# krispy-kenay/WebDGS

Hardware: AMD Instinct MI355X
Metric: training iters/sec (fwd+bwd+Adam), 1M Gaussians @1080p SH3 (higher is better)
Workload: dtype f32

## Files before the change

### bindings/napi/webdgs_napi.cc

```cpp
#include <node_api.h>

#include <cstdint>
#include <cstring>
#include <string>

#include "../../include/webdgs.h"

#define NAPI_OK(call)                                                         \
    do {                                                                      \
        if ((call) != napi_ok) {                                              \
            napi_throw_error(env, nullptr, "N-API call failed: " #call);      \
            return nullptr;                                                   \
        }                                                                     \
    } while (0)

static napi_value throw_wdgs(napi_env env, int code) {
    std::string msg = "[wdgs " + std::to_string(code) + "] " + wdgs_last_error();
    napi_throw_error(env, code == WDGS_E_CAPACITY ? "WDGS_E_CAPACITY" : (code == WDGS_E_STATE ? "WDGS_E_STATE" : "WDGS_E"), msg.c_str());
    return nullptr;
}
#define WDGS_OK_OR_THROW(expr)                      \
    do {                                            \
        int _rc = (expr);                           \
        if (_rc != WDGS_OK) return throw_wdgs(env, _rc); \
// ... 62 lines not shown

static napi_value abiVersion(napi_env env, napi_callback_info) { return make_u32(env, (uint32_t)wdgs_abi_version()); }
static napi_value deviceCreate(napi_env env, napi_callback_info info) {
    ARGS(1);
    wdgs_device* d = nullptr;
    WDGS_OK_OR_THROW(wdgs_device_create((int)get_u32(env, argv[0]), nullptr, &d));
    return make_ptr(env, d);
}
static napi_value deviceDestroy(napi_env env, napi_callback_info info) { ARGS(1); wdgs_device_destroy((wdgs_device*)get_ptr(env, argv[0])); return js_undefined(env); }
static napi_value deviceSynchronize(napi_env env, napi_callback_info info) {
    ARGS(1);
    WDGS_OK_OR_THROW(wdgs_device_synchronize((wdgs_device*)get_ptr(env, argv[0])));
    return js_undefined(env);
}
static napi_value deviceMemoryInfo(napi_env env, napi_callback_info info) {
    ARGS(1);
    size_t f = 0, t = 0, c = 0;
    WDGS_OK_OR_THROW(wdgs_device_memory_info((wdgs_device*)get_ptr(env, argv[0]), &f, &t, &c));
    napi_value o, v; napi_create_object(env, &o);
    napi_create_double(env, (double)f, &v); set_prop(env, o, "free", v);
    napi_create_double(env, (double)t, &v); set_prop(env, o, "total", v);
    napi_create_double(env, (double)c, &v); set_prop(env, o, "cached", v);
    return o;
}
static napi_value bufferCreate(napi_env env, napi_callback_info info) {
    ARGS(2);
    wdgs_buffer* b = nullptr;
    WDGS_OK_OR_THROW(wdgs_buffer_create((wdgs_device*)get_ptr(env, argv[0]), (size_t)get_f64(env, argv[1]), &b));
    napi_value o; napi_create_object(env, &o);
    set_prop(env, o, "handle", make_ptr(env, b));
    set_prop(env, o, "ptr", make_ptr(env, wdgs_buffer_ptr(b)));
    napi_value sz; napi_create_double(env, (double)wdgs_buffer_size(b), &sz);
    set_prop(env, o, "size", sz);
    return o;
}
static napi_value bufferDestroy(napi_env env, napi_callback_info info) { ARGS(1); wdgs_buffer_destroy((wdgs_buffer*)get_ptr(env, argv[0])); return js_undefined(env); }
static napi_value copyToDevice(napi_env env, napi_callback_info info) {
    ARGS(3);
    void* data = nullptr; size_t len = 0; napi_typedarray_type tt; napi_value ab; size_t off;
    bool is_ta = false; napi_is_typedarray(env, argv[2], &is_ta);
    if (is_ta) { NAPI_OK(napi_get_typedarray_info(env, argv[2], &tt, &len, &data, &ab, &off)); size_t es[] = {1,1,1,2,2,4,4,4,8,8,8}; len *= es[tt]; }
    else NAPI_OK(napi_get_arraybuffer_info(env, argv[2], &data, &len));
    WDGS_OK_OR_THROW(wdgs_copy_to_device((wdgs_device*)get_ptr(env, argv[0]), get_ptr(env, argv[1]), data, len));
    return js_undefined(env);
}
static napi_value copyToHost(napi_env env, napi_callback_info info) {
    ARGS(3);
    size_t len = (size_t)get_f64(env, argv[2]);
    void* data = nullptr; napi_value ab;
    NAPI_OK(napi_create_arraybuffer(env, len, &data, &ab));
    WDGS_OK_OR_THROW(wdgs_copy_to_host((wdgs_device*)get_ptr(env, argv[0]), data, get_ptr(env, argv[1]), len));
    return ab;
}
static napi_value tiledForwardCreate(napi_env env, napi_callback_info info) {
    ARGS(2);
    wdgs_tiled_forward_config c; std::memset(&c, 0, sizeof(c));
    c.num_points = (uint32_t)prop_f64(env, argv[1], "numPoints", 0);
    c.sh_deg = (uint32_t)prop_f64(env, argv[1], "shDeg", 0);
    c.viewport_width = (uint32_t)prop_f64(env, argv[1], "viewportWidth", 1);
    c.viewport_height = (uint32_t)prop_f64(env, argv[1], "viewportHeight", 1);
    c.gaussian_scale = (float)prop_f64(env, argv[1], "gaussianScale", 1.0);
    c.point_size_px = (float)prop_f64(env, argv[1], "pointSizePx", 3.0);
    c.max_splat_radius_px = (float)prop_f64(env, argv[1], "maxSplatRadiusPx", 128.0);
    c.render_mode = (uint32_t)prop_f64(env, argv[1], "renderMode", 1);
    c.max_tile_entries = (uint32_t)prop_f64(env, argv[1], "maxTileEntries", 0);
    c.compat_caps = (uint32_t)prop_f64(env, argv[1], "compatCaps", 0);
    wdgs_tiled_forward* op = nullptr;
    WDGS_OK_OR_THROW(wdgs_tiled_forward_create((wdgs_device*)get_ptr(env, argv[0]), &c, &op));
    return make_ptr(env, op);
}
static napi_value tiledForwardEncode(napi_env env, napi_callback_info info) {
    ARGS(5);
    WDGS_OK_OR_THROW(wdgs_tiled_forward_encode((wdgs_tiled_forward*)get_ptr(env, argv[0]), get_ptr(env, argv[1]), get_ptr(env, argv[2]), get_ptr(env, argv[3]),
                                               (int)get_u32(env, argv[4])));
    return js_undefined(env);
}
static napi_value tiledForwardSetViewport(napi_env env, napi_callback_info info) {
    ARGS(3);
    WDGS_OK_OR_THROW(wdgs_tiled_forward_set_viewport((wdgs_tiled_forward*)get_ptr(env, argv[0]), get_u32(env, argv[1]), get_u32(env, argv[2])));
    return js_undefined(env);
}
static napi_value tiledForwardGetResources(napi_env env, napi_callback_info info) {
    ARGS(1);
    wdgs_tiled_forward_resources r;
    WDGS_OK_OR_THROW(wdgs_tiled_forward_get_resources((wdgs_tiled_forward*)get_ptr(env, argv[0]), &r));
    napi_value o; napi_create_object(env, &o);
    set_prop(env, o, "splatBuffer", make_ptr(env, r.splat_buffer));
    set_prop(env, o, "tileKeysBuffer", make_ptr(env, r.tile_keys_buffer));
    set_prop(env, o, "tileIndicesBuffer", make_ptr(env, r.tile_indices_buffer));
    set_prop(env, o, "tileOffsetsBuffer", make_ptr(env, r.tile_offsets_buffer));
    set_prop(env, o, "tileCountsBuffer", make_ptr(env, r.tile_counts_buffer));
    set_prop(env, o, "statsBuffer", make_ptr(env, r.stats_buffer));
    set_prop(env, o, "numTilesX", make_u32(env, r.num_tiles_x));
    set_prop(env, o, "numTilesY", make_u32(env, r.num_tiles_y));
    set_prop(env, o, "totalTiles", make_u32(env, r.total_tiles));
    set_prop(env, o, "maxTileEntries", make_u32(env, r.max_tile_entries));
    return o;
}
static napi_value tiledForwardDestroy(napi_env env, napi_callback_info info) { ARGS(1); wdgs_tiled_forward_destroy((wdgs_tiled_forward*)get_ptr(env, argv[0])); return js_undefined(env); }
static napi_value tiledRasterizerCreate(napi_env env, napi_callback_info info) {
    ARGS(2);
    wdgs_tiled_rasterizer* op = nullptr;
    WDGS_OK_OR_THROW(wdgs_tiled_rasterizer_create((wdgs_device*)get_ptr(env, argv[0]), (wdgs_tiled_forward*)get_ptr(env, argv[1]), 0, &op));
    return make_ptr(env, op);
}
static napi_value tiledRasterizerEncode(napi_env env, napi_callback_info info) {
    ARGS(3);
    WDGS_OK_OR_THROW(wdgs_tiled_rasterizer_encode((wdgs_tiled_rasterizer*)get_ptr(env, argv[0]), get_u32(env, argv[1]), get_u32(env, argv[2])));
    return js_undefined(env);
}
static napi_value tiledRasterizerGet(napi_env env, napi_callback_info info) {
    ARGS(2);
    void* p = nullptr;
    wdgs_tiled_rasterizer* op = (wdgs_tiled_rasterizer*)get_ptr(env, argv[0]);
    switch (get_u32(env, argv[1])) {
        case 0: WDGS_OK_OR_THROW(wdgs_tiled_rasterizer_get_output(op, &p)); break;
        case 1: WDGS_OK_OR_THROW(wdgs_tiled_rasterizer_get_alpha(op, &p)); break;
        case 2: WDGS_OK_OR_THROW(wdgs_tiled_rasterizer_get_n_contrib(op, &p)); break;
        default: WDGS_OK_OR_THROW(wdgs_tiled_rasterizer_get_tile_offsets(op, &p)); break;
    }
    return make_ptr(env, p);
}
static napi_value tiledRasterizerDestroy(napi_env env, napi_callback_info info) { ARGS(1); wdgs_tiled_rasterizer_destroy((wdgs_tiled_rasterizer*)get_ptr(env, argv[0])); return js_undefined(env); }
static napi_value tiledBackwardCreate(napi_env env, napi_callback_info info) {
    ARGS(2);
    wdgs_tiled_backward_config c; std::memset(&c, 0, sizeof(c));
    c.num_points = (uint32_t)prop_f64(env, argv[1], "numPoints", 0);
    c.sh_deg = (uint32_t)prop_f64(env, argv[1], "shDeg", 0);
    c.viewport_width = (uint32_t)prop_f64(env, argv[1], "viewportWidth", 1);
    c.viewport_height = (uint32_t)prop_f64(env, argv[1], "viewportHeight", 1);
    c.training.lambda_l1 = (float)prop_f64(env, argv[1], "lambda_l1", 0.8);
    c.training.lambda_l2 = (float)prop_f64(env, argv[1], "lambda_l2", 0.0);
    c.training.lambda_dssim = (float)prop_f64(env, argv[1], "lambda_dssim", 0.2);
    c.training.c1 = (float)prop_f64(env, argv[1], "c1", 0.0001);
    c.training.c2 = (float)prop_f64(env, argv[1], "c2", 0.0009);
    c.max_splat_radius_px = (float)prop_f64(env, argv[1], "maxSplatRadiusPx", 128.0);
    uint32_t mode = 0;
    if (!prop_dssim_mode(env, argv[1], &mode)) return nullptr;
    wdgs_tiled_backward* op = nullptr;
    WDGS_OK_OR_THROW(wdgs_tiled_backward_create((wdgs_device*)get_ptr(env, argv[0]), &c, &op));
    const int r = wdgs_tiled_backward_set_dssim_mode(op, mode);
    if (r != WDGS_OK) { wdgs_tiled_backward_destroy(op); WDGS_OK_OR_THROW(r); }
    return make_ptr(env, op);
}
static napi_value tiledBackwardEncode(napi_env env, napi_callback_info info) {
    ARGS(5);
    wdgs_tiled_backward_resources r;
    r.splat_buffer = prop_ptr(env, argv[3], "splatBuffer");
    r.tile_offsets_buffer = prop_ptr(env, argv[3], "tileOffsetsBuffer");
    r.tile_indices_buffer = prop_ptr(env, argv[3], "tileIndicesBuffer");
    r.camera_buffer = prop_ptr(env, argv[3], "cameraBuffer");
    r.alpha_texture = prop_ptr(env, argv[3], "alphaTexture");
    r.n_contrib_texture = prop_ptr(env, argv[3], "nContribTexture");
    WDGS_OK_OR_THROW(wdgs_tiled_backward_encode((wdgs_tiled_backward*)get_ptr(env, argv[0]), get_ptr(env, argv[1]), get_ptr(env, argv[2]), &r, get_ptr(env, argv[4])));
    return js_undefined(env);
}
static napi_value tiledBackwardGradients(napi_env env, napi_callback_info info) { ARGS(1); return make_ptr(env, wdgs_tiled_backward_gradients((wdgs_tiled_backward*)get_ptr(env, argv[0]))); }
static napi_value tiledBackwardDestroy(napi_env env, napi_callback_info info) { ARGS(1); wdgs_tiled_backward_destroy((wdgs_tiled_backward*)get_ptr(env, argv[0])); return js_undefined(env); }
static napi_value optimizerCreate(napi_env env, napi_callback_info info) {
    ARGS(4);
    wdgs_optimizer* op = nullptr;
    WDGS_OK_OR_THROW(wdgs_optimizer_create((wdgs_device*)get_ptr(env, argv[0]), get_u32(env, argv[1]), nullptr, get_ptr(env, argv[2]), get_ptr(env, argv[3]), nullptr, 1, 0, &op));
    return make_ptr(env, op);
}
static napi_value optimizerStep(napi_env env, napi_callback_info info) {
    ARGS(5);
    WDGS_OK_OR_THROW(wdgs_optimizer_step((wdgs_optimizer*)get_ptr(env, argv[0]), get_ptr(env, argv[1]), get_ptr(env, argv[2]), get_ptr(env, argv[3]), get_ptr(env, argv[4])));
    return js_undefined(env);
}
static napi_value optimizerGetIteration(napi_env env, napi_callback_info info) { ARGS(1); return make_u32(env, wdgs_optimizer_get_iteration((wdgs_optimizer*)get_ptr(env, argv[0]))); }
static napi_value optimizerDestroy(napi_env env, napi_callback_info info) { ARGS(1); wdgs_optimizer_destroy((wdgs_optimizer*)get_ptr(env, argv[0])); return js_undefined(env); }

static napi_value tiledForwardSet(napi_env env, napi_callback_info info) {
    ARGS(3);
    wdgs_tiled_forward* op = (wdgs_tiled_forward*)get_ptr(env, argv[0]);
    switch (get_u32(env, argv[1])) {
        case 0: WDGS_OK_OR_THROW(wdgs_tiled_forward_set_render_mode(op, get_u32(env, argv[2]))); break;
        case 1: WDGS_OK_OR_THROW(wdgs_tiled_forward_set_point_size(op, (float)get_f64(env, argv[2]))); break;
        default: WDGS_OK_OR_THROW(wdgs_tiled_forward_set_gaussian_scale(op, (float)get_f64(env, argv[2]))); break;
    }
    return js_undefined(env);
}
static napi_value tiledForwardCheck(napi_env env, napi_callback_info info) {
    ARGS(1);
    uint32_t st[4] = {0, 0, 0, 0};
    WDGS_OK_OR_THROW(wdgs_tiled_forward_check((wdgs_tiled_forward*)get_ptr(env, argv[0]), st));
    napi_value o; napi_create_object(env, &o);
    set_prop(env, o, "totalTileEntries", make_u32(env, st[0]));
    set_prop(env, o, "visibleCount", make_u32(env, st[1]));
    return o;
}
static napi_value tiledForwardSetLongLists(napi_env env, napi_callback_info info) {
    ARGS(4);
    WDGS_OK_OR_THROW(wdgs_tiled_forward_set_long_lists((wdgs_tiled_forward*)get_ptr(env, argv[0]), get_u32(env, argv[1]), get_u32(env, argv[2]), get_u32(env, argv[3])));
    return js_undefined(env);
}
static napi_value tiledForwardLongListStats(napi_env env, napi_callback_info info) {
    ARGS(1);
    uint32_t st[12] = {0};
    WDGS_OK_OR_THROW(wdgs_tiled_forward_long_list_stats((wdgs_tiled_forward*)get_ptr(env, argv[0]), st));
    static const char* const keys[12] = {"blocksWanted", "itemsWanted", "forwardQueue", "backwardQueue", "rowsUsed", "rowsWanted", "stalled", nullptr, "maxItems", "maxBlocks", "maxRows", "threshold"};
    napi_value o; napi_create_object(env, &o);
    for (int i = 0; i < 12; i++) if (keys[i]) set_prop(env, o, keys[i], make_u32(env, st[i]));
    return o;
}
static napi_value tiledRasterizerBlit(napi_env env, napi_callback_info info) {
    ARGS(4);
    WDGS_OK_OR_THROW(wdgs_tiled_rasterizer_blit((wdgs_tiled_rasterizer*)get_ptr(env, argv[0]), get_ptr(env, argv[1]), get_u32(env, argv[2]), get_u32(env, argv[3])));
    return js_undefined(env);
}
static napi_value tiledRasterizerEncodeDepth(napi_env env, napi_callback_info info) {
    ARGS(2);
    WDGS_OK_OR_THROW(wdgs_tiled_rasterizer_encode_depth((wdgs_tiled_rasterizer*)get_ptr(env, argv[0]), get_u32(env, argv[1])));
    return js_undefined(env);
}
static napi_value tiledRasterizerGetDepth(napi_env env, napi_callback_info info) {
    ARGS(2);
    void* p = nullptr;
    WDGS_OK_OR_THROW(wdgs_tiled_rasterizer_get_depth((wdgs_tiled_rasterizer*)get_ptr(env, argv[0]), get_u32(env, argv[1]), &p));
    return make_ptr(env, p);
}
static napi_value depthToRgba8(napi_env env, napi_callback_info info) {
    ARGS(7);
    WDGS_OK_OR_THROW(wdgs_depth_to_rgba8((wdgs_device*)get_ptr(env, argv[0]), get_ptr(env, argv[1]), get_u32(env, argv[2]), get_u32(env, argv[3]), (float)get_f64(env, argv[4]),
                                         (float)get_f64(env, argv[5]), get_ptr(env, argv[6])));
    return js_undefined(env);
}
static napi_value bufferClear(napi_env env, napi_callback_info info) {
    ARGS(3);
    WDGS_OK_OR_THROW(wdgs_memset((wdgs_device*)get_ptr(env, argv[0]), get_ptr(env, argv[1]), 0, (size_t)get_f64(env, argv[2])));
    return js_undefined(env);
}
static napi_value encoderBegin(napi_env env, napi_callback_info info) { ARGS(1); WDGS_OK_OR_THROW(wdgs_encoder_begin((wdgs_device*)get_ptr(env, argv[0]))); return js_undefined(env); }
static napi_value encoderFinish(napi_env env, napi_callback_info info) {
    ARGS(1);
    wdgs_command_buffer* c = nullptr;
    WDGS_OK_OR_THROW(wdgs_encoder_finish((wdgs_device*)get_ptr(env, argv[0]), &c));
    return make_ptr(env, c);
}
static napi_value queueSubmit(napi_env env, napi_callback_info info) {
    ARGS(2);
    WDGS_OK_OR_THROW(wdgs_queue_submit((wdgs_device*)get_ptr(env, argv[0]), (wdgs_command_buffer*)get_ptr(env, argv[1])));
    return js_undefined(env);
}
static napi_value commandBufferDestroy(napi_env env, napi_callback_info info) { ARGS(1); wdgs_command_buffer_destroy((wdgs_command_buffer*)get_ptr(env, argv[0])); return js_undefined(env); }

struct DoneCtx { napi_deferred deferred; napi_threadsafe_function tsfn; };
static void done_call_js(napi_env env, napi_value, void* context, void*) {
    DoneCtx* c = static_cast<DoneCtx*>(context);
    if (env) { napi_value u; napi_get_undefined(env, &u); napi_resolve_deferred(env, c->deferred, u); }
    napi_release_threadsafe_function(c->tsfn, napi_tsfn_release);
    delete c;
}
static void done_from_runtime_thread(void* user) {
    DoneCtx* c = static_cast<DoneCtx*>(user);
    napi_call_threadsafe_function(c->tsfn, nullptr, napi_tsfn_blocking);
}
static napi_value queueOnSubmittedWorkDone(napi_env env, napi_callback_info info) {
    ARGS(1);
    DoneCtx* c = new DoneCtx();
    napi_value promise, name;
    NAPI_OK(napi_create_promise(env, &c->deferred, &promise));
    napi_create_string_utf8(env, "wdgs onSubmittedWorkDone", NAPI_AUTO_LENGTH, &name);
    NAPI_OK(napi_create_threadsafe_function(env, nullptr, nullptr, name, 0, 1, nullptr, nullptr, c, done_call_js, &c->tsfn));
    int rc = wdgs_queue_on_done((wdgs_device*)get_ptr(env, argv[0]), done_from_runtime_thread, c);
    if (rc != WDGS_OK) { napi_release_threadsafe_function(c->tsfn, napi_tsfn_abort); delete c; return throw_wdgs(env, rc); }
    return promise;
}

static void read_backward_resources(napi_env env, napi_value o, wdgs_tiled_backward_resources* r) {
    r->splat_buffer = prop_ptr(env, o, "splatBuffer");
    r->tile_offsets_buffer = prop_ptr(env, o, "tileOffsetsBuffer");
    r->tile_indices_buffer = prop_ptr(env, o, "tileIndicesBuffer");
    r->camera_buffer = prop_ptr(env, o, "cameraBuffer");
    r->alpha_texture = prop_ptr(env, o, "alphaTexture");
    r->n_contrib_texture = prop_ptr(env, o, "nContribTexture");
}
static napi_value tiledBackwardMetric(napi_env env, napi_callback_info info) {
    ARGS(5);
    wdgs_tiled_backward* op = (wdgs_tiled_backward*)get_ptr(env, argv[0]);
    switch (get_u32(env, argv[1])) {
        case 0: WDGS_OK_OR_THROW(wdgs_tiled_backward_compute_loss_only(op, get_ptr(env, argv[2]), get_ptr(env, argv[3]))); break;
        case 1: WDGS_OK_OR_THROW(wdgs_tiled_backward_compute_metric_map(op, get_ptr(env, argv[2]), get_ptr(env, argv[3]), (float)get_f64(env, argv[4]))); break;
        case 2: {
            wdgs_tiled_backward_resources r;
            read_backward_resources(env, argv[2], &r);
            WDGS_OK_OR_THROW(wdgs_tiled_backward_compute_metric_counts(op, &r, get_u32(env, argv[3]), (int)get_u32(env, argv[4])));
            break;
        }
        case 3: WDGS_OK_OR_THROW(wdgs_tiled_backward_normalize_metric_counts(op, get_u32(env, argv[2]))); break;
        case 5: {
            uint32_t mode = 0;
            if (!prop_dssim_mode(env, argv[2], &mode)) return nullptr;
            wdgs_training_config t;
            t.lambda_l1 = (float)prop_f64(env, argv[2], "lambda_l1", 0.8);
            t.lambda_l2 = (float)prop_f64(env, argv[2], "lambda_l2", 0.0);
            t.lambda_dssim = (float)prop_f64(env, argv[2], "lambda_dssim", 0.2);
            t.c1 = (float)prop_f64(env, argv[2], "c1", 0.0001);
            t.c2 = (float)prop_f64(env, argv[2], "c2", 0.0009);
            WDGS_OK_OR_THROW(wdgs_tiled_backward_set_training_config(op, &t));
            WDGS_OK_OR_THROW(wdgs_tiled_backward_set_dssim_mode(op, mode));
            break;
        }
        default: WDGS_OK_OR_THROW(wdgs_tiled_backward_set_viewport(op, get_u32(env, argv[2]), get_u32(env, argv[3]))); break;
    }
    return js_undefined(env);
}
static napi_value tiledBackwardGet(napi_env env, napi_callback_info info) {
    ARGS(2);
    wdgs_tiled_backward* op = (wdgs_tiled_backward*)get_ptr(env, argv[0]);
    switch (get_u32(env, argv[1])) {
        case 0: return make_ptr(env, wdgs_tiled_backward_gradients(op));
        case 1: return make_ptr(env, wdgs_tiled_backward_metric_counts(op));
        case 2: return make_ptr(env, wdgs_tiled_backward_loss_image(op));
        default: return make_ptr(env, wdgs_tiled_backward_metric_map(op));
    }
}
static napi_value downsampleRGBA8(napi_env env, napi_callback_info info) {
    ARGS(7);
    WDGS_OK_OR_THROW(wdgs_downsample_rgba8((wdgs_device*)get_ptr(env, argv[0]), get_ptr(env, argv[1]), get_u32(env, argv[2]), get_u32(env, argv[3]),
                                           get_ptr(env, argv[4]), get_u32(env, argv[5]), get_u32(env, argv[6])));
    return js_undefined(env);
}
static napi_value imageSSE(napi_env env, napi_callback_info info) {
    ARGS(5);
    WDGS_OK_OR_THROW(wdgs_image_sse_rgb8((wdgs_device*)get_ptr(env, argv[0]), get_ptr(env, argv[1]), get_ptr(env, argv[2]), get_u32(env, argv[3]), get_ptr(env, argv[4])));
    return js_undefined(env);
}
static napi_value imageSSIM(napi_env env, napi_callback_info info) {
    ARGS(7);
    WDGS_OK_OR_THROW(wdgs_image_ssim_rgb8((wdgs_device*)get_ptr(env, argv[0]), get_ptr(env, argv[1]), get_ptr(env, argv[2]), get_u32(env, argv[3]), get_u32(env, argv[4]),
                                          get_ptr(env, argv[5]), get_ptr(env, argv[6])));
    return js_undefined(env);
}

static bool read_state(napi_env env, napi_value o, wdgs_optimizer_state* s) {
    napi_valuetype t; napi_typeof(env, o, &t);
    if (t != napi_object) return false;
    s->opt_pos = prop_ptr(env, o, "optPosBuffer"); s->opt_rot = prop_ptr(env, o, "optRotBuffer"); s->opt_scale = prop_ptr(env, o, "optScaleBuffer");
    s->opt_opacity = prop_ptr(env, o, "optOpacityBuffer"); s->param_sh = prop_ptr(env, o, "paramSH"); s->state_sh = prop_ptr(env, o, "stateSH");
    return true;
}
static napi_value make_state(napi_env env, const wdgs_optimizer_state& s) {
    napi_value o; napi_create_object(env, &o);
    set_prop(env, o, "optPosBuffer", make_ptr(env, s.opt_pos)); set_prop(env, o, "optRotBuffer", make_ptr(env, s.opt_rot));
    set_prop(env, o, "optScaleBuffer", make_ptr(env, s.opt_scale)); set_prop(env, o, "optOpacityBuffer", make_ptr(env, s.opt_opacity));
    set_prop(env, o, "paramSH", make_ptr(env, s.param_sh)); set_prop(env, o, "stateSH", make_ptr(env, s.state_sh));
    return o;
}
static napi_value optimizerStateSizes(napi_env env, napi_callback_info info) {
    ARGS(1);
    size_t sz[6];
    WDGS_OK_OR_THROW(wdgs_optimizer_state_sizes(get_u32(env, argv[0]), sz));
    napi_value arr; napi_create_array_with_length(env, 6, &arr);
    for (uint32_t i = 0; i < 6; i++) { napi_value v; napi_create_double(env, (double)sz[i], &v); napi_set_element(env, arr, i, v); }
    return arr;
}
static napi_value optimizerCreateWithState(napi_env env, napi_callback_info info) {
    ARGS(7);
    wdgs_optimizer_state st; std::memset(&st, 0, sizeof(st));
    const bool has = read_state(env, argv[4], &st);
    wdgs_optimizer* op = nullptr;
    WDGS_OK_OR_THROW(wdgs_optimizer_create((wdgs_device*)get_ptr(env, argv[0]), get_u32(env, argv[1]), nullptr, get_ptr(env, argv[2]), get_ptr(env, argv[3]),
                                           has ? &st : nullptr, (int)get_u32(env, argv[5]), get_u32(env, argv[6]), &op));
    return make_ptr(env, op);
}
static napi_value optimizerState(napi_env env, napi_callback_info info) {
    ARGS(2);
    wdgs_optimizer_state st;
    if (get_u32(env, argv[1])) WDGS_OK_OR_THROW(wdgs_optimizer_release_state((wdgs_optimizer*)get_ptr(env, argv[0]), &st));
    else WDGS_OK_OR_THROW(wdgs_optimizer_get_state((wdgs_optimizer*)get_ptr(env, argv[0]), &st));
    return make_state(env, st);
}
static napi_value optimizerHyperparameters(napi_env env, napi_callback_info info) {
    ARGS(2);
    wdgs_optimizer* op = (wdgs_optimizer*)get_ptr(env, argv[0]);
    wdgs_adam_hyperparameters h;
    WDGS_OK_OR_THROW(wdgs_optimizer_get_hyperparameters(op, &h));
    napi_valuetype t; napi_typeof(env, argv[1], &t);
    if (t == napi_object) {
        h.lr_pos = (float)prop_f64(env, argv[1], "lr_pos", h.lr_pos); h.lr_color = (float)prop_f64(env, argv[1], "lr_color", h.lr_color);
        h.lr_opacity = (float)prop_f64(env, argv[1], "lr_opacity", h.lr_opacity); h.lr_scale = (float)prop_f64(env, argv[1], "lr_scale", h.lr_scale);
        h.lr_rot = (float)prop_f64(env, argv[1], "lr_rot", h.lr_rot); h.beta1 = (float)prop_f64(env, argv[1], "beta1", h.beta1);
        h.beta2 = (float)prop_f64(env, argv[1], "beta2", h.beta2); h.epsilon = (float)prop_f64(env, argv[1], "epsilon", h.epsilon);
        WDGS_OK_OR_THROW(wdgs_optimizer_set_hyperparameters(op, &h));
    }
    napi_value o; napi_create_object(env, &o);
    const char* names[8] = {"lr_pos", "lr_color", "lr_opacity", "lr_scale", "lr_rot", "beta1", "beta2", "epsilon"};
    const float vals[8] = {h.lr_pos, h.lr_color, h.lr_opacity, h.lr_scale, h.lr_rot, h.beta1, h.beta2, h.epsilon};
    for (int i = 0; i < 8; i++) { napi_value v; napi_create_double(env, vals[i], &v); set_prop(env, o, names[i], v); }
    return o;
}
static napi_value optimizerAdvanceIteration(napi_env env, napi_callback_info info) {
    ARGS(2);
    WDGS_OK_OR_THROW(wdgs_optimizer_advance_iteration((wdgs_optimizer*)get_ptr(env, argv[0]), get_u32(env, argv[1])));
    return js_undefined(env);
}
static napi_value optimizerStepF32(napi_env env, napi_callback_info info) {
    ARGS(5);
    WDGS_OK_OR_THROW(wdgs_optimizer_step_f32((wdgs_optimizer*)get_ptr(env, argv[0]), get_ptr(env, argv[1]), get_ptr(env, argv[2]), get_ptr(env, argv[3]), get_ptr(env, argv[4])));
    return js_undefined(env);
}
static napi_value accumulateGradients(napi_env env, napi_callback_info info) {
    ARGS(6);
    WDGS_OK_OR_THROW(wdgs_accumulate_gradients((wdgs_device*)get_ptr(env, argv[0]), get_u32(env, argv[1]), get_ptr(env, argv[2]), get_ptr(env, argv[3]),
                                               get_ptr(env, argv[4]), get_ptr(env, argv[5])));
    return js_undefined(env);
}

static void read_densify_config(napi_env env, napi_value o, wdgs_densify_config* c) {
    c->num_views = (uint32_t)prop_f64(env, o, "numViews", 1);
    c->clone_threshold = (uint32_t)prop_f64(env, o, "cloneThreshold", 0);
    c->split_threshold = (float)prop_f64(env, o, "splitThreshold", 1e9);
    c->prune_threshold = (float)prop_f64(env, o, "pruneThreshold", 0.0);
    c->max_new_points_per_step = (uint32_t)prop_f64(env, o, "maxNewPointsPerStep", 0);
    c->max_buffer_bytes = (uint64_t)prop_f64(env, o, "maxBufferBytes", 128.0 * 1024 * 1024);
}
static napi_value densifyCreate(napi_env env, napi_callback_info info) {
    ARGS(2);
    wdgs_densify_config c; read_densify_config(env, argv[1], &c);
    wdgs_densify_prune* op = nullptr;
    WDGS_OK_OR_THROW(wdgs_densify_prune_create((wdgs_device*)get_ptr(env, argv[0]), &c, &op));
    return make_ptr(env, op);
}
static napi_value densifySetConfig(napi_env env, napi_callback_info info) {
    ARGS(2);
    wdgs_densify_config c; read_densify_config(env, argv[1], &c);
    WDGS_OK_OR_THROW(wdgs_densify_prune_set_config((wdgs_densify_prune*)get_ptr(env, argv[0]), &c));
    return js_undefined(env);
// ... 370 lines not shown
```

### include/webdgs.h

```cpp
#ifndef WEBDGS_H
#define WEBDGS_H

#include <stddef.h>
#include <stdint.h>

#ifdef __cplusplus
extern "C" {
#endif

#define WDGS_OK 0
#define WDGS_E_INVALID (-1)
#define WDGS_E_HIP (-2)
#define WDGS_E_CAPACITY (-3)
#define WDGS_E_STATE (-4)

typedef struct wdgs_device wdgs_device;
typedef struct wdgs_buffer wdgs_buffer;
typedef struct wdgs_prefix_scanner wdgs_prefix_scanner;
typedef struct wdgs_sorter wdgs_sorter;
typedef struct wdgs_tiled_forward wdgs_tiled_forward;
typedef struct wdgs_tiled_rasterizer wdgs_tiled_rasterizer;
typedef struct wdgs_tiled_backward wdgs_tiled_backward;
typedef struct wdgs_optimizer wdgs_optimizer;
typedef struct wdgs_densify_prune wdgs_densify_prune;
typedef struct wdgs_command_buffer wdgs_command_buffer;

const char* wdgs_last_error(void);
int wdgs_abi_version(void);

int wdgs_device_create(int hip_ordinal, void* external_hip_stream, wdgs_device** out);
int wdgs_device_destroy(wdgs_device* dev);
int wdgs_device_synchronize(wdgs_device* dev);
int wdgs_device_memory_info(wdgs_device* dev, size_t* free_bytes, size_t* total_bytes, size_t* cached_bytes);
int wdgs_device_set_profiling(wdgs_device* dev, int enabled);
typedef struct wdgs_kernel_time {
    char name[48];
    uint32_t launches;
    float total_ms;
} wdgs_kernel_time;
int wdgs_device_get_kernel_times(wdgs_device* dev, wdgs_kernel_time* out, uint32_t cap, uint32_t* count);
int wdgs_device_reset_kernel_times(wdgs_device* dev);
#define WDGS_MAX_LANES 4
#define WDGS_MAX_BATCH_VIEWS 16
int wdgs_device_select_lane(wdgs_device* dev, int lane);
int wdgs_device_lane_order(wdgs_device* dev, int waiter_lane, int signal_lane);
int wdgs_device_lane_mark(wdgs_device* dev, int lane, int mark);
int wdgs_device_lane_wait_mark(wdgs_device* dev, int lane, int mark);

int wdgs_encoder_begin(wdgs_device* dev);
int wdgs_encoder_finish(wdgs_device* dev, wdgs_command_buffer** out);
int wdgs_encoder_abort(wdgs_device* dev);
int wdgs_queue_submit(wdgs_device* dev, wdgs_command_buffer* cmd);
int wdgs_command_buffer_destroy(wdgs_command_buffer* cmd);
typedef void (*wdgs_done_callback)(void* user);
int wdgs_queue_on_done(wdgs_device* dev, wdgs_done_callback fn, void* user);
#define WDGS_TICKET_RING 8
int wdgs_queue_mark(wdgs_device* dev, uint64_t* ticket);
int wdgs_queue_wait(wdgs_device* dev, uint64_t ticket);

int wdgs_copy_to_host(wdgs_device* dev, void* dst_host, const void* src_dev, size_t bytes);
int wdgs_copy_to_device(wdgs_device* dev, void* dst_dev, const void* src_host, size_t bytes);
int wdgs_memset(wdgs_device* dev, void* dst_dev, int value, size_t bytes);
int wdgs_copy_buffer_to_buffer(wdgs_device* dev, void* dst_dev, const void* src_dev, size_t bytes);

int wdgs_buffer_create(wdgs_device* dev, size_t bytes, wdgs_buffer** out);
int wdgs_buffer_destroy(wdgs_buffer* buf);
void* wdgs_buffer_ptr(const wdgs_buffer* buf);
size_t wdgs_buffer_size(const wdgs_buffer* buf);
int wdgs_buffer_write(wdgs_device* dev, wdgs_buffer* buf, size_t offset, const void* src_host, size_t bytes);
int wdgs_buffer_read(wdgs_device* dev, const wdgs_buffer* buf, size_t offset, void* dst_host, size_t bytes);
int wdgs_buffer_read_async(wdgs_device* dev, const wdgs_buffer* buf, size_t offset, void* dst_host, size_t bytes);
int wdgs_host_alloc(size_t bytes, void** out_host);
int wdgs_host_free(void* host);

int wdgs_prefix_scanner_create(wdgs_device* dev, uint32_t max_elements, wdgs_prefix_scanner** out);
int wdgs_prefix_scanner_destroy(wdgs_prefix_scanner* s);
void* wdgs_prefix_scanner_input(wdgs_prefix_scanner* s);
void* wdgs_prefix_scanner_output(wdgs_prefix_scanner* s);
int wdgs_prefix_scanner_set_count(wdgs_prefix_scanner* s, uint32_t count);
int wdgs_prefix_scanner_scan(wdgs_prefix_scanner* s);
int wdgs_prefix_scanner_scan_ptr(wdgs_prefix_scanner* s, const void* in_dev, void* out_dev, uint32_t count);

int wdgs_sorter_create(wdgs_device* dev, uint32_t max_capacity, const void* stats_dev, wdgs_sorter** out);
int wdgs_sorter_destroy(wdgs_sorter* s);
void* wdgs_sorter_keys(wdgs_sorter* s, int ping_pong_index);
void* wdgs_sorter_values(wdgs_sorter* s, int ping_pong_index);
int wdgs_sorter_sort(wdgs_sorter* s, uint32_t key_bits);
int wdgs_sorter_final_out_index(wdgs_sorter* s);
uint32_t wdgs_sorter_capacity(wdgs_sorter* s);

typedef struct wdgs_tiled_forward_config {
    uint32_t num_points;
    uint32_t sh_deg;
    uint32_t viewport_width;
    uint32_t viewport_height;
    float gaussian_scale;
    float point_size_px;
    float max_splat_radius_px;
    uint32_t render_mode;
    uint32_t max_tile_entries;
    uint32_t compat_caps;
} wdgs_tiled_forward_config;

typedef struct wdgs_tiled_forward_resources {
    void* splat_buffer;
    void* depths_buffer;
    void* tile_keys_buffer;
    void* tile_indices_buffer;
    void* tile_offsets_buffer;
    void* tile_counts_buffer;
    void* stats_buffer;
    uint32_t num_tiles_x, num_tiles_y, total_tiles, max_tile_entries;
    float settings[7];
} wdgs_tiled_forward_resources;

int wdgs_tiled_forward_create(wdgs_device* dev, const wdgs_tiled_forward_config* cfg, wdgs_tiled_forward** out);
int wdgs_tiled_forward_destroy(wdgs_tiled_forward* op);
int wdgs_tiled_forward_resize(wdgs_tiled_forward* op, uint32_t num_points);
int wdgs_tiled_forward_encode(wdgs_tiled_forward* op, const void* gaussians_dev, const void* sh_dev, const void* camera_dev, int skip_sort);
int wdgs_tiled_forward_set_viewport(wdgs_tiled_forward* op, uint32_t width, uint32_t height);
int wdgs_tiled_forward_set_render_mode(wdgs_tiled_forward* op, uint32_t render_mode);
int wdgs_tiled_forward_set_point_size(wdgs_tiled_forward* op, float point_size_px);
int wdgs_tiled_forward_set_gaussian_scale(wdgs_tiled_forward* op, float scale);
int wdgs_tiled_forward_get_resources(wdgs_tiled_forward* op, wdgs_tiled_forward_resources* out);
int wdgs_tiled_forward_check(wdgs_tiled_forward* op, uint32_t* stats_out);
int wdgs_tiled_forward_set_long_lists(wdgs_tiled_forward* op, uint32_t threshold, uint32_t max_items, uint32_t max_rows);
int wdgs_tiled_forward_long_list_stats(wdgs_tiled_forward* op, uint32_t stats_out[12]);

int wdgs_tiled_rasterizer_create(wdgs_device* dev, wdgs_tiled_forward* forward, uint32_t compat_caps, wdgs_tiled_rasterizer** out);
int wdgs_tiled_rasterizer_destroy(wdgs_tiled_rasterizer* op);
int wdgs_tiled_rasterizer_encode(wdgs_tiled_rasterizer* op, uint32_t width, uint32_t height);
int wdgs_tiled_rasterizer_get_output(wdgs_tiled_rasterizer* op, void** rgba8_dev);
int wdgs_tiled_rasterizer_get_alpha(wdgs_tiled_rasterizer* op, void** final_t_dev);
int wdgs_tiled_rasterizer_get_n_contrib(wdgs_tiled_rasterizer* op, void** n_contrib_dev);
int wdgs_tiled_rasterizer_get_tile_offsets(wdgs_tiled_rasterizer* op, void** ranges_dev);
int wdgs_tiled_rasterizer_blit(wdgs_tiled_rasterizer* op, void* target_rgba8_dev, uint32_t target_width, uint32_t target_height);

#define WDGS_DEPTH_EXPECTED   1u
#define WDGS_DEPTH_MEDIAN     2u
#define WDGS_DEPTH_WEIGHT_SUM 4u
int wdgs_tiled_rasterizer_encode_depth(wdgs_tiled_rasterizer* op, uint32_t kinds);
int wdgs_tiled_rasterizer_get_depth(wdgs_tiled_rasterizer* op, uint32_t kind, void** f32_dev);
int wdgs_depth_to_rgba8(wdgs_device* dev, const void* depth_f32_dev, uint32_t width, uint32_t height, float near_z, float far_z, void* rgba8_dev);

typedef struct wdgs_training_config {
    float lambda_l1, lambda_l2, lambda_dssim, c1, c2;
} wdgs_training_config;
typedef struct wdgs_tiled_backward_config {
    uint32_t num_points;
    uint32_t sh_deg;
    uint32_t viewport_width, viewport_height;
    wdgs_training_config training;
    float gaussian_scale, point_size_px, max_splat_radius_px;
} wdgs_tiled_backward_config;
typedef struct wdgs_tiled_backward_resources {
    const void* splat_buffer;
    const void* tile_offsets_buffer;
    const void* tile_indices_buffer;
    const void* camera_buffer;
    const void* alpha_texture;
    const void* n_contrib_texture;
} wdgs_tiled_backward_resources;

int wdgs_tiled_backward_create(wdgs_device* dev, const wdgs_tiled_backward_config* cfg, wdgs_tiled_backward** out);
int wdgs_tiled_backward_resize(wdgs_tiled_backward* op, uint32_t num_points);
int wdgs_tiled_backward_destroy(wdgs_tiled_backward* op);
int wdgs_tiled_backward_encode(wdgs_tiled_backward* op, const void* predicted_rgba8_dev, const void* target_rgba8_dev,
                               const wdgs_tiled_backward_resources* res, const void* gaussians_dev);
typedef struct wdgs_view_accumulate {
    void* sums;
    void* visible;
    const void* tile_counts;
    void* guard;
    const void* overflow_word;
    int first;
} wdgs_view_accumulate;
int wdgs_tiled_backward_encode_raster(wdgs_tiled_backward* op, const void* predicted_rgba8_dev, const void* target_rgba8_dev,
                                      const wdgs_tiled_backward_resources* res);
int wdgs_tiled_backward_encode_geometry(wdgs_tiled_backward* op, const void* camera_dev, const void* gaussians_dev, const wdgs_view_accumulate* into);
int wdgs_tiled_backward_compute_loss_only(wdgs_tiled_backward* op, const void* predicted_rgba8_dev, const void* target_rgba8_dev);
int wdgs_tiled_backward_compute_metric_map(wdgs_tiled_backward* op, const void* predicted_rgba8_dev, const void* target_rgba8_dev, float threshold);
int wdgs_tiled_backward_compute_metric_counts(wdgs_tiled_backward* op, const wdgs_tiled_backward_resources* res, uint32_t num_instances, int clear);
int wdgs_tiled_backward_normalize_metric_counts(wdgs_tiled_backward* op, uint32_t divisor);
int wdgs_tiled_backward_set_viewport(wdgs_tiled_backward* op, uint32_t width, uint32_t height);
int wdgs_tiled_backward_set_training_config(wdgs_tiled_backward* op, const wdgs_training_config* cfg);
#define WDGS_DSSIM_REFERENCE 0
#define WDGS_DSSIM_GAUSSIAN 1
int wdgs_tiled_backward_set_dssim_mode(wdgs_tiled_backward* op, uint32_t mode);
int wdgs_tiled_backward_get_dssim_mode(const wdgs_tiled_backward* op, uint32_t* out);
void* wdgs_tiled_backward_gradients(wdgs_tiled_backward* op);
void* wdgs_tiled_backward_metric_counts(wdgs_tiled_backward* op);
int wdgs_tiled_backward_set_metric_counts_target(wdgs_tiled_backward* op, void* counts_dev);
void* wdgs_tiled_backward_loss_image(wdgs_tiled_backward* op);
void* wdgs_tiled_backward_metric_map(wdgs_tiled_backward* op);
int wdgs_tiled_backward_set_gradient_output(wdgs_tiled_backward* op, int enabled);
void* wdgs_tiled_backward_accumulators(wdgs_tiled_backward* op);
void* wdgs_tiled_backward_metric_minmax(wdgs_tiled_backward* op);
int wdgs_downsample_rgba8(wdgs_device* dev, const void* src_dev, uint32_t src_w, uint32_t src_h, void* dst_dev, uint32_t dst_w, uint32_t dst_h);

int wdgs_image_sse_rgb8(wdgs_device* dev, const void* a_rgba8_dev, const void* b_rgba8_dev, uint32_t num_pixels, void* out_u64_dev);

int wdgs_image_ssim_rgb8(wdgs_device* dev, const void* a_rgba8_dev, const void* b_rgba8_dev, uint32_t width, uint32_t height, void* out_f64_dev,
                         void* map_f32_dev);

int wdgs_debug_eval_math(wdgs_device* dev, uint32_t which, uint32_t count, const void* in_u32_dev, void* out_u32_dev);

typedef struct wdgs_adam_hyperparameters {
    float lr_pos, lr_color, lr_opacity, lr_scale, lr_rot, beta1, beta2, epsilon;
} wdgs_adam_hyperparameters;
typedef struct wdgs_optimizer_state {
    void* opt_pos;
    void* opt_rot;
    void* opt_scale;
    void* opt_opacity;
    void* param_sh;
    void* state_sh;
} wdgs_optimizer_state;
int wdgs_optimizer_state_sizes(uint32_t num_points, size_t sizes_out[6]);
int wdgs_optimizer_create(wdgs_device* dev, uint32_t num_points, const wdgs_adam_hyperparameters* params,
                          const void* gaussians_dev, const void* sh_dev,
                          const wdgs_optimizer_state* initial_state, int owns_state, uint32_t initial_iteration, wdgs_optimizer** out);
int wdgs_optimizer_destroy(wdgs_optimizer* op);
int wdgs_optimizer_init_from_point_cloud(wdgs_optimizer* op, const void* gaussians_dev, const void* sh_dev);
int wdgs_optimizer_step(wdgs_optimizer* op, void* gaussians_dev, void* sh_dev, const void* gradients_dev, const void* tile_counts_dev);
int wdgs_optimizer_step_with_geometry(wdgs_optimizer* op, wdgs_tiled_backward* bwd, const void* camera_dev, void* gaussians_dev, void* sh_dev,
                                      const void* tile_counts_dev);
int wdgs_optimizer_step_f32(wdgs_optimizer* op, void* gaussians_dev, void* sh_dev, const void* grad_f32_dev, const void* visible_counts_dev);
int wdgs_accumulate_gradients(wdgs_device* dev, uint32_t num_points, const void* gradients_dev, const void* tile_counts_dev,
                              void* acc_f32_dev, void* visible_counts_dev);
int wdgs_store_gradients(wdgs_device* dev, uint32_t num_points, const void* gradients_dev, const void* tile_counts_dev,
                         void* acc_f32_dev, void* visible_counts_dev);
int wdgs_optimizer_step_f32_range(wdgs_optimizer* op, void* gaussians_dev, void* sh_dev, const void* grad_f32_dev, const void* visible_counts_dev,
                                  uint32_t first, uint32_t count, void* rows_out_dev);
int wdgs_apply_repacked_rows(wdgs_device* dev, uint32_t num_points, const void* rows_dev, uint32_t skip_first, uint32_t skip_count,
                             const void* guard_dev, void* gaussians_dev, void* sh_dev);
int wdgs_optimizer_set_guard(wdgs_optimizer* op, const void* flag_u32_dev);
int wdgs_optimizer_set_deferred_sh(wdgs_optimizer* op, void* sh_dev, int enabled);
void* wdgs_optimizer_dc_words(wdgs_optimizer* op);
int wdgs_optimizer_flush_sh(wdgs_optimizer* op, void* sh_dev);
int wdgs_optimizer_apply_repacked_rows(wdgs_optimizer* op, const void* rows_dev, uint32_t skip_first, uint32_t skip_count, const void* guard_u32_dev,
                                       void* gaussians_dev, void* sh_dev);
int wdgs_tiled_forward_set_dc_source(wdgs_tiled_forward* op, const void* dc_words_dev);

int wdgs_tiled_forward_project_views(wdgs_tiled_forward* const* ops, const void* const* cameras_dev, uint32_t count, const void* gaussians_dev, const void* sh_dev);
int wdgs_tiled_forward_encode_projected(wdgs_tiled_forward* op);
int wdgs_tiled_forward_is_projected(const wdgs_tiled_forward* op);
int wdgs_tiled_backward_encode_geometry_views(wdgs_tiled_backward* const* ops, const void* const* cameras_dev, const void* const* tile_counts_dev,
                                              const void* const* overflow_words_dev, uint32_t count, const void* gaussians_dev, void* sums_f32_dev,
                                              void* visible_dev, void* guard_u32_dev, int write_gradients, int continues);
int wdgs_guard_accumulate(wdgs_device* dev, void* flag_u32_dev, const void* src_u32_dev, int overwrite);
int wdgs_optimizer_state_changed(wdgs_optimizer* op);
uint32_t wdgs_optimizer_get_iteration(const wdgs_optimizer* op);
int wdgs_optimizer_advance_iteration(wdgs_optimizer* op, uint32_t count);
int wdgs_optimizer_get_hyperparameters(const wdgs_optimizer* op, wdgs_adam_hyperparameters* out);
int wdgs_optimizer_set_hyperparameters(wdgs_optimizer* op, const wdgs_adam_hyperparameters* params);
int wdgs_optimizer_get_state(wdgs_optimizer* op, wdgs_optimizer_state* out);
int wdgs_optimizer_release_state(wdgs_optimizer* op, wdgs_optimizer_state* out);

typedef struct wdgs_densify_config {
    uint32_t num_views;
    uint32_t clone_threshold;
    float split_threshold;
    float prune_threshold;
    uint32_t max_new_points_per_step;
    uint64_t max_buffer_bytes;
} wdgs_densify_config;
typedef struct wdgs_densify_prepared {
    void* action_buffer;
    void* out_count_buffer;
    void* out_offset_buffer;
    void* out_total_buffer;
    uint32_t max_out_points;
} wdgs_densify_prepared;

int wdgs_densify_prune_create(wdgs_device* dev, const wdgs_densify_config* cfg, wdgs_densify_prune** out);
int wdgs_densify_prune_destroy(wdgs_densify_prune* op);
int wdgs_densify_prune_set_config(wdgs_densify_prune* op, const wdgs_densify_config* cfg);
int wdgs_densify_prune_ensure_size(wdgs_densify_prune* op, uint32_t num_points);
int wdgs_densify_prune_encode_prepare(wdgs_densify_prune* op, uint32_t num_points, const void* gaussians_dev,
                                      const void* metric_counts_dev, wdgs_densify_prepared* out);
int wdgs_densify_prune_encode_decision(wdgs_densify_prune* op, uint32_t num_points, const void* gaussians_dev, const void* metric_counts_dev);
int wdgs_densify_prune_encode_prefix_sum(wdgs_densify_prune* op, uint32_t num_points);
int wdgs_densify_prune_encode_cap_to_max(wdgs_densify_prune* op, uint32_t num_points, uint32_t max_out_points);
int wdgs_densify_prune_encode_total_out(wdgs_densify_prune* op, uint32_t num_points);
int wdgs_densify_prune_compute_max_out_points(wdgs_densify_prune* op, uint32_t num_points, uint32_t* max_out_points);
int wdgs_densify_prune_get_buffers(wdgs_densify_prune* op, wdgs_densify_prepared* out);
int wdgs_densify_prune_read_total(wdgs_densify_prune* op, uint32_t* total_out);
int wdgs_densify_prune_encode_scatter(wdgs_densify_prune* op, uint32_t in_points, const void* in_gaussians_dev, const void* in_sh_dev,
                                      const wdgs_optimizer_state* in_state, uint32_t out_num_points, int reset_new_optimizer_state,
                                      void* out_gaussians_dev, void* out_sh_dev, const wdgs_optimizer_state* out_state);

#define WDGS_COMM_ID_BYTES 128
typedef struct wdgs_comm wdgs_comm;
int wdgs_comm_get_unique_id(uint8_t id_out[WDGS_COMM_ID_BYTES]);
int wdgs_comm_create(wdgs_device* dev, const uint8_t id[WDGS_COMM_ID_BYTES], int world_size, int rank, wdgs_comm** out);
int wdgs_comm_destroy(wdgs_comm* comm);
int wdgs_comm_world_size(const wdgs_comm* comm);
int wdgs_comm_rank(const wdgs_comm* comm);
int wdgs_comm_allreduce_gradients(wdgs_comm* comm, void* grad_f32_dev, void* visible_counts_dev, uint32_t num_points);
int wdgs_comm_allreduce_counts(wdgs_comm* comm, void* counts_u32_dev, uint32_t count);
int wdgs_comm_exchange_gradients(wdgs_comm* comm, void* grad_f32_dev, void* visible_counts_dev, void* flag_u32_dev, uint32_t slice_points);
int wdgs_comm_allgather_rows(wdgs_comm* comm, void* rows_dev, uint32_t slice_points);
int wdgs_comm_broadcast(wdgs_comm* comm, void* ptr_dev, size_t bytes, int root);
int wdgs_comm_group_start(void);
int wdgs_comm_group_end(void);

#ifdef __cplusplus
}
#endif
#endif
```

### webdgs_amd/_lib.py

```python
from __future__ import annotations

import ctypes as C
import os

_HERE = os.path.dirname(os.path.abspath(__file__))
LIB_PATH = os.environ.get("WDGS_LIB_PATH") or os.path.join(_HERE, "lib", "libwebdgs_hip.so")

WDGS_OK, WDGS_E_INVALID, WDGS_E_HIP, WDGS_E_CAPACITY, WDGS_E_STATE = 0, -1, -2, -3, -4


class WdgsError(RuntimeError):

    def __init__(self, code: int, message: str):
        super().__init__(f"[wdgs {code}] {message}")
        self.code = code


class CapacityError(WdgsError):
    pass


class StateError(WdgsError):
    pass


class KernelTime(C.Structure):
    _fields_ = [("name", C.c_char * 48), ("launches", C.c_uint32), ("total_ms", C.c_float)]


class TiledForwardConfig(C.Structure):
    _fields_ = [("num_points", C.c_uint32), ("sh_deg", C.c_uint32), ("viewport_width", C.c_uint32), ("viewport_height", C.c_uint32),
                ("gaussian_scale", C.c_float), ("point_size_px", C.c_float), ("max_splat_radius_px", C.c_float), ("render_mode", C.c_uint32),
                ("max_tile_entries", C.c_uint32), ("compat_caps", C.c_uint32)]


class TiledForwardResources(C.Structure):
    _fields_ = [("splat_buffer", C.c_void_p), ("depths_buffer", C.c_void_p), ("tile_keys_buffer", C.c_void_p), ("tile_indices_buffer", C.c_void_p),
                ("tile_offsets_buffer", C.c_void_p), ("tile_counts_buffer", C.c_void_p), ("stats_buffer", C.c_void_p),
                ("num_tiles_x", C.c_uint32), ("num_tiles_y", C.c_uint32), ("total_tiles", C.c_uint32), ("max_tile_entries", C.c_uint32),
                ("settings", C.c_float * 7)]


class TrainingConfig(C.Structure):
    _fields_ = [("lambda_l1", C.c_float), ("lambda_l2", C.c_float), ("lambda_dssim", C.c_float), ("c1", C.c_float), ("c2", C.c_float)]


class TiledBackwardConfig(C.Structure):
    _fields_ = [("num_points", C.c_uint32), ("sh_deg", C.c_uint32), ("viewport_width", C.c_uint32), ("viewport_height", C.c_uint32),
                ("training", TrainingConfig), ("gaussian_scale", C.c_float), ("point_size_px", C.c_float), ("max_splat_radius_px", C.c_float)]


class TiledBackwardResources(C.Structure):
    _fields_ = [("splat_buffer", C.c_void_p), ("tile_offsets_buffer", C.c_void_p), ("tile_indices_buffer", C.c_void_p), ("camera_buffer", C.c_void_p),
                ("alpha_texture", C.c_void_p), ("n_contrib_texture", C.c_void_p)]


class ViewAccumulate(C.Structure):
    _fields_ = [("sums", C.c_void_p), ("visible", C.c_void_p), ("tile_counts", C.c_void_p), ("guard", C.c_void_p), ("overflow_word", C.c_void_p),
                ("first", C.c_int)]


class AdamHyperparameters(C.Structure):
    _fields_ = [("lr_pos", C.c_float), ("lr_color", C.c_float), ("lr_opacity", C.c_float), ("lr_scale", C.c_float), ("lr_rot", C.c_float),
                ("beta1", C.c_float), ("beta2", C.c_float), ("epsilon", C.c_float)]


class OptimizerState(C.Structure):
    _fields_ = [("opt_pos", C.c_void_p), ("opt_rot", C.c_void_p), ("opt_scale", C.c_void_p), ("opt_opacity", C.c_void_p), ("param_sh", C.c_void_p),
                ("state_sh", C.c_void_p)]


class DensifyConfig(C.Structure):
    _fields_ = [("num_views", C.c_uint32), ("clone_threshold", C.c_uint32), ("split_threshold", C.c_float), ("prune_threshold", C.c_float),
                ("max_new_points_per_step", C.c_uint32), ("max_buffer_bytes", C.c_uint64)]


class DensifyPrepared(C.Structure):
    _fields_ = [("action_buffer", C.c_void_p), ("out_count_buffer", C.c_void_p), ("out_offset_buffer", C.c_void_p), ("out_total_buffer", C.c_void_p),
                ("max_out_points", C.c_uint32)]


_P = C.c_void_p
_U = C.c_uint32
_I = C.c_int
_F = C.c_float
_Z = C.c_size_t
DoneCallback = C.CFUNCTYPE(None, C.c_void_p)

SIGNATURES = {
    "wdgs_last_error": (C.c_char_p, []),
    "wdgs_abi_version": (_I, []),
    "wdgs_device_create": (_I, [_I, _P, C.POINTER(_P)]),
    "wdgs_device_destroy": (_I, [_P]),
    "wdgs_device_synchronize": (_I, [_P]),
    "wdgs_device_memory_info": (_I, [_P, C.POINTER(C.c_size_t), C.POINTER(C.c_size_t), C.POINTER(C.c_size_t)]),
    "wdgs_device_set_profiling": (_I, [_P, _I]),
    "wdgs_device_get_kernel_times": (_I, [_P, C.POINTER(KernelTime), _U, C.POINTER(_U)]),
    "wdgs_device_reset_kernel_times": (_I, [_P]),
    "wdgs_queue_mark": (_I, [_P, C.POINTER(C.c_uint64)]),
    "wdgs_queue_wait": (_I, [_P, C.c_uint64]),
    "wdgs_device_select_lane": (_I, [_P, _I]),
    "wdgs_device_lane_order": (_I, [_P, _I, _I]),
    "wdgs_device_lane_mark": (_I, [_P, _I, _I]),
    "wdgs_device_lane_wait_mark": (_I, [_P, _I, _I]),
    "wdgs_encoder_begin": (_I, [_P]),
    "wdgs_encoder_finish": (_I, [_P, C.POINTER(_P)]),
    "wdgs_encoder_abort": (_I, [_P]),
    "wdgs_queue_submit": (_I, [_P, _P]),
    "wdgs_command_buffer_destroy": (_I, [_P]),
    "wdgs_queue_on_done": (_I, [_P, DoneCallback, _P]),
    "wdgs_buffer_read_async": (_I, [_P, _P, _Z, _P, _Z]),
    "wdgs_host_alloc": (_I, [_Z, C.POINTER(_P)]),
    "wdgs_host_free": (_I, [_P]),
    "wdgs_tiled_rasterizer_blit": (_I, [_P, _P, _U, _U]),
    "wdgs_densify_prune_encode_decision": (_I, [_P, _U, _P, _P]),
    "wdgs_densify_prune_encode_prefix_sum": (_I, [_P, _U]),
    "wdgs_densify_prune_encode_cap_to_max": (_I, [_P, _U, _U]),
    "wdgs_densify_prune_encode_total_out": (_I, [_P, _U]),
    "wdgs_densify_prune_compute_max_out_points": (_I, [_P, _U, C.POINTER(_U)]),
    "wdgs_densify_prune_get_buffers": (_I, [_P, C.POINTER(DensifyPrepared)]),
    "wdgs_debug_eval_math": (_I, [_P, _U, _U, _P, _P]),
    "wdgs_comm_get_unique_id": (_I, [C.POINTER(C.c_uint8)]),
    "wdgs_comm_create": (_I, [_P, C.POINTER(C.c_uint8), _I, _I, C.POINTER(_P)]),
    "wdgs_comm_destroy": (_I, [_P]),
    "wdgs_comm_world_size": (_I, [_P]),
    "wdgs_comm_rank": (_I, [_P]),
    "wdgs_comm_allreduce_gradients": (_I, [_P, _P, _P, _U]),
    "wdgs_comm_allreduce_counts": (_I, [_P, _P, _U]),
    "wdgs_comm_exchange_gradients": (_I, [_P, _P, _P, _P, _U]),
    "wdgs_comm_allgather_rows": (_I, [_P, _P, _U]),
    "wdgs_comm_broadcast": (_I, [_P, _P, _Z, _I]),
    "wdgs_comm_group_start": (_I, []),
    "wdgs_comm_group_end": (_I, []),
    "wdgs_optimizer_step_f32_range": (_I, [_P, _P, _P, _P, _P, _U, _U, _P]),
    "wdgs_apply_repacked_rows": (_I, [_P, _U, _P, _U, _U, _P, _P, _P]),
    "wdgs_optimizer_set_guard": (_I, [_P, _P]),
    "wdgs_optimizer_set_deferred_sh": (_I, [_P, _P, _I]),
    "wdgs_optimizer_dc_words": (_P, [_P]),
    "wdgs_optimizer_flush_sh": (_I, [_P, _P]),
    "wdgs_optimizer_apply_repacked_rows": (_I, [_P, _P, _U, _U, _P, _P, _P]),
    "wdgs_tiled_forward_set_dc_source": (_I, [_P, _P]),
    "wdgs_tiled_forward_project_views": (_I, [_P, _P, _U, _P, _P]),
    "wdgs_tiled_forward_encode_projected": (_I, [_P]),
    "wdgs_tiled_forward_is_projected": (_I, [_P]),
    "wdgs_tiled_backward_encode_geometry_views": (_I, [_P, _P, _P, _P, _U, _P, _P, _P, _P, _I, _I]),
    "wdgs_guard_accumulate": (_I, [_P, _P, _P, _I]),
    "wdgs_optimizer_state_changed": (_I, [_P]),
    "wdgs_copy_to_host": (_I, [_P, _P, _P, _Z]),
    "wdgs_copy_to_device": (_I, [_P, _P, _P, _Z]),
    "wdgs_memset": (_I, [_P, _P, _I, _Z]),
    "wdgs_copy_buffer_to_buffer": (_I, [_P, _P, _P, _Z]),
    "wdgs_buffer_create": (_I, [_P, _Z, C.POINTER(_P)]),
    "wdgs_buffer_destroy": (_I, [_P]),
    "wdgs_buffer_ptr": (_P, [_P]),
    "wdgs_buffer_size": (_Z, [_P]),
    "wdgs_buffer_write": (_I, [_P, _P, _Z, _P, _Z]),
    "wdgs_buffer_read": (_I, [_P, _P, _Z, _P, _Z]),
    "wdgs_prefix_scanner_create": (_I, [_P, _U, C.POINTER(_P)]),
    "wdgs_prefix_scanner_destroy": (_I, [_P]),
    "wdgs_prefix_scanner_input": (_P, [_P]),
    "wdgs_prefix_scanner_output": (_P, [_P]),
    "wdgs_prefix_scanner_set_count": (_I, [_P, _U]),
    "wdgs_prefix_scanner_scan": (_I, [_P]),
    "wdgs_prefix_scanner_scan_ptr": (_I, [_P, _P, _P, _U]),
    "wdgs_sorter_create": (_I, [_P, _U, _P, C.POINTER(_P)]),
    "wdgs_sorter_destroy": (_I, [_P]),
    "wdgs_sorter_keys": (_P, [_P, _I]),
    "wdgs_sorter_values": (_P, [_P, _I]),
    "wdgs_sorter_sort": (_I, [_P, _U]),
    "wdgs_sorter_final_out_index": (_I, [_P]),
    "wdgs_sorter_capacity": (_U, [_P]),
    "wdgs_tiled_forward_create": (_I, [_P, C.POINTER(TiledForwardConfig), C.POINTER(_P)]),
    "wdgs_tiled_forward_destroy": (_I, [_P]),
    "wdgs_tiled_forward_resize": (_I, [_P, _U]),
    "wdgs_tiled_forward_encode": (_I, [_P, _P, _P, _P, _I]),
    "wdgs_tiled_forward_set_viewport": (_I, [_P, _U, _U]),
    "wdgs_tiled_forward_set_render_mode": (_I, [_P, _U]),
    "wdgs_tiled_forward_set_point_size": (_I, [_P, _F]),
    "wdgs_tiled_forward_set_gaussian_scale": (_I, [_P, _F]),
    "wdgs_tiled_forward_get_resources": (_I, [_P, C.POINTER(TiledForwardResources)]),
    "wdgs_tiled_forward_check": (_I, [_P, C.POINTER(_U)]),
    "wdgs_tiled_forward_set_long_lists": (_I, [_P, _U, _U, _U]),
    "wdgs_tiled_forward_long_list_stats": (_I, [_P, C.POINTER(_U)]),
    "wdgs_tiled_rasterizer_create": (_I, [_P, _P, _U, C.POINTER(_P)]),
    "wdgs_tiled_rasterizer_destroy": (_I, [_P]),
    "wdgs_tiled_rasterizer_encode": (_I, [_P, _U, _U]),
    "wdgs_tiled_rasterizer_get_output": (_I, [_P, C.POINTER(_P)]),
    "wdgs_tiled_rasterizer_get_alpha": (_I, [_P, C.POINTER(_P)]),
    "wdgs_tiled_rasterizer_get_n_contrib": (_I, [_P, C.POINTER(_P)]),
    "wdgs_tiled_rasterizer_get_tile_offsets": (_I, [_P, C.POINTER(_P)]),
    "wdgs_tiled_rasterizer_encode_depth": (_I, [_P, _U]),
    "wdgs_tiled_rasterizer_get_depth": (_I, [_P, _U, C.POINTER(_P)]),
    "wdgs_depth_to_rgba8": (_I, [_P, _P, _U, _U, _F, _F, _P]),
    "wdgs_tiled_backward_create": (_I, [_P, C.POINTER(TiledBackwardConfig), C.POINTER(_P)]),
    "wdgs_tiled_backward_resize": (_I, [_P, _U]),
    "wdgs_tiled_backward_destroy": (_I, [_P]),
    "wdgs_tiled_backward_encode": (_I, [_P, _P, _P, C.POINTER(TiledBackwardResources), _P]),
    "wdgs_tiled_backward_encode_raster": (_I, [_P, _P, _P, C.POINTER(TiledBackwardResources)]),
    "wdgs_tiled_backward_encode_geometry": (_I, [_P, _P, _P, C.POINTER(ViewAccumulate)]),
    "wdgs_tiled_backward_compute_loss_only": (_I, [_P, _P, _P]),
    "wdgs_tiled_backward_compute_metric_map": (_I, [_P, _P, _P, _F]),
    "wdgs_tiled_backward_compute_metric_counts": (_I, [_P, C.POINTER(TiledBackwardResources), _U, _I]),
    "wdgs_tiled_backward_normalize_metric_counts": (_I, [_P, _U]),
    "wdgs_tiled_backward_set_viewport": (_I, [_P, _U, _U]),
    "wdgs_tiled_backward_set_training_config": (_I, [_P, C.POINTER(TrainingConfig)]),
    "wdgs_tiled_backward_set_dssim_mode": (_I, [_P, _U]),
    "wdgs_tiled_backward_get_dssim_mode": (_I, [_P, C.POINTER(_U)]),
    "wdgs_tiled_backward_gradients": (_P, [_P]),
    "wdgs_tiled_backward_metric_counts": (_P, [_P]),
    "wdgs_tiled_backward_set_metric_counts_target": (_I, [_P, _P]),
    "wdgs_tiled_backward_loss_image": (_P, [_P]),
    "wdgs_tiled_backward_metric_map": (_P, [_P]),
    "wdgs_tiled_backward_accumulators": (_P, [_P]),
    "wdgs_tiled_backward_set_gradient_output": (_I, [_P, _I]),
    "wdgs_tiled_backward_metric_minmax": (_P, [_P]),
    "wdgs_downsample_rgba8": (_I, [_P, _P, _U, _U, _P, _U, _U]),
    "wdgs_image_sse_rgb8": (_I, [_P, _P, _P, _U, _P]),
    "wdgs_image_ssim_rgb8": (_I, [_P, _P, _P, _U, _U, _P, _P]),
    "wdgs_optimizer_state_sizes": (_I, [_U, C.POINTER(_Z * 6)]),
    "wdgs_optimizer_create": (_I, [_P, _U, C.POINTER(AdamHyperparameters), _P, _P, C.POINTER(OptimizerState), _I, _U, C.POINTER(_P)]),
    "wdgs_optimizer_destroy": (_I, [_P]),
    "wdgs_optimizer_init_from_point_cloud": (_I, [_P, _P, _P]),
    "wdgs_optimizer_step": (_I, [_P, _P, _P, _P, _P]),
    "wdgs_optimizer_step_with_geometry": (_I, [_P, _P, _P, _P, _P, _P]),
    "wdgs_optimizer_step_f32": (_I, [_P, _P, _P, _P, _P]),
    "wdgs_accumulate_gradients": (_I, [_P, _U, _P, _P, _P, _P]),
    "wdgs_store_gradients": (_I, [_P, _U, _P, _P, _P, _P]),
    "wdgs_optimizer_get_iteration": (_U, [_P]),
    "wdgs_optimizer_advance_iteration": (_I, [_P, _U]),
    "wdgs_optimizer_get_hyperparameters": (_I, [_P, C.POINTER(AdamHyperparameters)]),
    "wdgs_optimizer_set_hyperparameters": (_I, [_P, C.POINTER(AdamHyperparameters)]),
    "wdgs_optimizer_get_state": (_I, [_P, C.POINTER(OptimizerState)]),
    "wdgs_optimizer_release_state": (_I, [_P, C.POINTER(OptimizerState)]),
    "wdgs_densify_prune_create": (_I, [_P, C.POINTER(DensifyConfig), C.POINTER(_P)]),
    "wdgs_densify_prune_destroy": (_I, [_P]),
    "wdgs_densify_prune_set_config": (_I, [_P, C.POINTER(DensifyConfig)]),
    "wdgs_densify_prune_ensure_size": (_I, [_P, _U]),
    "wdgs_densify_prune_encode_prepare": (_I, [_P, _U, _P, _P, C.POINTER(DensifyPrepared)]),
    "wdgs_densify_prune_read_total": (_I, [_P, C.POINTER(_U)]),
    "wdgs_densify_prune_encode_scatter": (_I, [_P, _U, _P, _P, C.POINTER(OptimizerState), _U, _I, _P, _P, C.POINTER(OptimizerState)]),
}

_lib = None


def load() -> C.CDLL:
    global _lib
    if _lib is not None:
        return _lib
    if not os.path.exists(LIB_PATH):
        raise ImportError(f"{LIB_PATH} is missing: build it with `python -c 'import __graft_entry__ as g; g.build()'` "
                          "or `make -C webdgs_amd/csrc` (hipcc --offload-arch=gfx950). There is no CPU fallback.")
    lib = C.CDLL(LIB_PATH)
    for name, (res, args) in SIGNATURES.items():
        fn = getattr(lib, name)
        fn.restype = res
        fn.argtypes = args
    _lib = lib
    return lib


def check(code: int) -> None:
    if code == WDGS_OK:
        return
    msg = load().wdgs_last_error().decode("utf-8", "replace")
    if code == WDGS_E_CAPACITY:
        raise CapacityError(code, msg)
    if code == WDGS_E_STATE:
        raise StateError(code, msg)
    raise WdgsError(code, msg)
```

### webdgs_amd/csrc/api.hip

```cpp
#include <cstdarg>
#include <cstdio>
#include <cstdlib>
#include <cstring>
#include <algorithm>
#include <mutex>
#include <map>
#include <set>
#include <unordered_map>
#include <vector>

#include "common.h"
#include "alloc_cache.h"
#include "longlist.h"

int launch_project_count(wdgs_device*, u32, const void*, const void*, const void*, const RenderSettings&, const TileInfo&, void*, void*, void*, void*, void*, void*,
                         const void*, void*, const void*);
int launch_emit_scatter(wdgs_device*, u32, const void*, const void*, const void*, void*, const void*, const RenderSettings&, const TileInfo&, const void*, const void*, void*, void*, u32);
int sorter_sort_rows(wdgs_sorter* s, u32 num_tiles_x, u32 num_tiles_y, u32* ranges, const LongWork* lw);
extern "C" void sorter_set_final_out_index(wdgs_sorter* s, int i);
int launch_update_stats(wdgs_device*, u32, const void*, const void*, u32, void*, void*, void*);
int launch_emit(wdgs_device*, u32, const void*, const void*, const void*, void*, const void*, const RenderSettings&, const TileInfo&, void*, void*, u32);
int launch_tile_ranges(wdgs_device*, const void*, const void*, u32, void*);
int launch_depth_composite(wdgs_device*, const RenderSettings&, const TileInfo&, const void*, u32, const void*, const void*, const void*, const void*, const void*, u32,
                           void*, void*, void*, const void*, const void*);
int launch_rasterize(wdgs_device*, const RenderSettings&, const TileInfo&, const void*, u32, const void*, const void*, const void*, const void*, u32, void*,
                     void*, void*, const void*, const void*, const LongWork*);
int launch_loss_grad(wdgs_device*, u32, u32, const void*, const void*, const wdgs_training_config&, void*, void*, u32, const void*);
int launch_dssim_grad(wdgs_device*, u32, u32, const void*, const void*, const wdgs_training_config&, void*, void*, u32, const void*);
int launch_backward_rasterize(wdgs_device*, const RenderSettings&, u32, u32, const void*, const void*, const void*, const void*, const void*, const void*,
                              void*, void*, const LongWork*);
int launch_acc_clear_if_dirty(wdgs_device*, void*, u32, void*);
int launch_geometry_backward_views(wdgs_device*, u32, u32, const void* const*, const RenderSettings&, const void*, void* const*, void* const*, const void* const*,
                                   const void* const*, void* const*, void*, void*, void*, u32);
int launch_project_count_views(wdgs_device*, u32, u32, const void*, const void*, const void* const*, const RenderSettings&, const TileInfo&, void* const*, void* const*,
                               void* const*, void* const*, void* const*, void* const*, const void*, void* const*, const void* const*);
int launch_geometry_backward(wdgs_device*, u32, const void*, const RenderSettings&, const void*, void*, void*);
int launch_geometry_backward_adam(wdgs_device*, u32, const void*, const RenderSettings&, void*, void*, void*, void*, const wdgs_adam_hyperparameters&, const void*,
                                  const wdgs_optimizer_state&, const CsView&, void*, const void*, void*);
int launch_geometry_backward_accumulate(wdgs_device*, u32, const void*, const RenderSettings&, const void*, void*, void*, void*, void*, void*, const void*, void*,
                                        const void*, u32);
int launch_adam_repack(wdgs_device*, u32, const wdgs_adam_hyperparameters&, const void*, const void*, const wdgs_optimizer_state&, const CsView&, void*, void*,
                       const void*, void*);
int launch_adam_repack_f32(wdgs_device*, u32, u32, const wdgs_adam_hyperparameters&, const void*, const void*, const wdgs_optimizer_state&, const CsView&, void*,
                           void*, const void*, void*, void*, void*);
int launch_apply_rows(wdgs_device*, u32, const void*, u32, u32, const void*, void*, void*, void*, void*);
int launch_dc_words_load(wdgs_device*, u32, const void*, void*);
int launch_dc_words_flush(wdgs_device*, u32, const void*, void*);
int launch_guard_accumulate(wdgs_device*, void*, const void*, u32);
int launch_cs_load(wdgs_device*, u32, const wdgs_optimizer_state&, const CsView&);
int launch_cs_flush(wdgs_device*, u32, const CsView&, const wdgs_optimizer_state&);
int launch_accumulate_gradients(wdgs_device*, u32, const void*, const void*, void*, void*);
int launch_store_gradients(wdgs_device*, u32, const void*, const void*, void*, void*);
int launch_unpack(wdgs_device*, u32, const void*, const void*, const wdgs_optimizer_state&);
int launch_metric_map(wdgs_device*, u32, u32, const void*, const void*, float, float, void*, void*, void*, void*);
int launch_metric_count(wdgs_device*, const RenderSettings&, u32, u32, const void*, const void*, u32, const void*, u32, const void*, const void*, void*, u32);
int launch_metric_normalize(wdgs_device*, u32, u32, void*);
int launch_downsample(wdgs_device*, const void*, u32, u32, void*, u32, u32);

int sorter_sort_segmented(wdgs_sorter* s, u32 segment_bits, u32 num_segments, u32* ranges, const LongWork* lw);
extern "C" int wdgs_sorter_final_out_index(wdgs_sorter* s);
extern "C" uint32_t wdgs_sorter_capacity(wdgs_sorter* s);

static thread_local char g_last_error[512] = "";

static std::mutex g_live_mutex;
static std::set<const wdgs_device*> g_live_devices;
bool wdgs_device_alive(const wdgs_device* d) {
    std::lock_guard<std::mutex> lock(g_live_mutex);
    return d && g_live_devices.count(d) != 0;
}
static void sync_if_alive(wdgs_device* d) {
    if (wdgs_device_alive(d) && !d->capturing) (void)wdgs_sync_lanes(d);
}

void wdgs_set_error(const char* fmt, ...) {
    va_list ap;
    va_start(ap, fmt);
    vsnprintf(g_last_error, sizeof(g_last_error), fmt, ap);
    va_end(ap);
}

namespace {
struct HipBackend {
    void* malloc(int device, size_t bytes) {
        int cur = 0;
        if (hipGetDevice(&cur) != hipSuccess) return nullptr;
        if (cur != device && hipSetDevice(device) != hipSuccess) return nullptr;
        void* p = nullptr;
        const hipError_t e = hipMalloc(&p, bytes);
        if (cur != device) (void)hipSetDevice(cur);
        if (e != hipSuccess) { (void)hipGetLastError(); return nullptr; }
        return p;
    }
    void free(void* p) { (void)hipFree(p); }
    bool sync(int device) {
        int cur = 0;
        if (hipGetDevice(&cur) != hipSuccess) return false;
        if (cur != device && hipSetDevice(device) != hipSuccess) return false;
        const hipError_t e = hipDeviceSynchronize();
        if (cur != device) (void)hipSetDevice(cur);
        return e == hipSuccess;
    }
};
wdgs::AllocCache<HipBackend> g_alloc_cache;
size_t g_cache_limit = 0;
std::mutex g_cache_limit_mutex;
bool alloc_cache_enabled() {
    static const bool on = !(std::getenv("WDGS_ALLOC_CACHE") && std::getenv("WDGS_ALLOC_CACHE")[0] == '0');
    return on;
}
}

int wdgs_alloc(void** p, size_t bytes, bool zero, hipStream_t stream) {
    *p = nullptr;
    if (bytes == 0) bytes = 16;
    if (!alloc_cache_enabled()) {
        WDGS_CHECK_HIP(hipMalloc(p, bytes));
    } else {
        int device = 0;
        WDGS_CHECK_HIP(hipGetDevice(&device));
        hipStreamCaptureStatus capture = hipStreamCaptureStatusNone;
        const bool recording = stream && hipStreamIsCapturing(stream, &capture) == hipSuccess && capture != hipStreamCaptureStatusNone;
        *p = g_alloc_cache.alloc(device, bytes, !recording);
        WDGS_REQUIRE(*p, WDGS_E_HIP, "device allocation of %zu bytes failed (device %d)", bytes, device);
    }
    if (zero) WDGS_CHECK_HIP(hipMemsetAsync(*p, 0, bytes, stream));
    return WDGS_OK;
}

void wdgs_free(void* p) {
    if (!p) return;
    if (alloc_cache_enabled()) {
        size_t limit;
        {
            std::lock_guard<std::mutex> lock(g_cache_limit_mutex);
            if (g_cache_limit == 0) {
                size_t free_b = 0, total_b = 0;
                g_cache_limit = (hipMemGetInfo(&free_b, &total_b) == hipSuccess && total_b) ? total_b / 4 : ((size_t)8 << 30);
            }
            limit = g_cache_limit;
        }
        if (g_alloc_cache.free(p, limit)) return;
    }
    (void)hipFree(p);
}
static void free_dev(void* p) { wdgs_free(p); }

struct wdgs_buffer {
    void* ptr;
    size_t size;
};

struct wdgs_prefix_scanner {
    wdgs_device* dev;
    u32 max_elements, count;
    u32 *input, *output;
    ScanScratch scratch;
};

struct wdgs_tiled_forward {
    wdgs_device* dev;
    wdgs_tiled_forward_config cfg;
    RenderSettings settings;
    TileInfo tile_info;
    u32* stats;
    u32* nf_stamp;
    u32 nf_capacity;
    LongWork long_lists;
    u32 long_flags_capacity;
    u32* host_stats;
    u32* splats;
    u32* depths;
    u32* block_counts;
    u32* column_counts;
    u32* column_totals;
    const void* dc_source;
    u32 points_capacity;
    wdgs_prefix_scanner* scanner;
    wdgs_sorter* sorter;
    u32* ranges;
// ... 929 lines not shown
            WDGS_TRY(wdgs_alloc((void**)&op->ranges, sizeof(u32) * (size_t)(ti.total_tiles + 1), true, d->stream));
            op->ranges_capacity = ti.total_tiles + 1;
        }
        WDGS_TRY(launch_tile_ranges(d, keys, f->stats, ti.total_tiles, op->ranges));
        op->ranges_used = op->ranges;
    }
    WDGS_TRY(launch_rasterize(d, f->settings, ti, f->splats, f->cfg.num_points, op->ranges_used, keys, vals, f->stats, op->compat_caps ? 32u : 0u, op->rgba8,
                              op->alpha, op->n_contrib, f->nf_stamp, f->stats + FRAME_WORD,
                              (f->ranges_valid && f->long_lists.hdr && !op->compat_caps) ? &f->long_lists : nullptr));
    op->encoded = true;
    return WDGS_OK;
}

int wdgs_tiled_rasterizer_encode_depth(wdgs_tiled_rasterizer* op, uint32_t kinds) {
    WDGS_REQUIRE(op, WDGS_E_INVALID, "wdgs_tiled_rasterizer_encode_depth: null op");
    constexpr uint32_t all = WDGS_DEPTH_EXPECTED | WDGS_DEPTH_MEDIAN | WDGS_DEPTH_WEIGHT_SUM;
    WDGS_REQUIRE(kinds != 0u && (kinds & ~all) == 0u, WDGS_E_INVALID, "wdgs_tiled_rasterizer_encode_depth: kinds 0x%x is not a non-empty set of WDGS_DEPTH_* bits", kinds);
    wdgs_tiled_forward* f = op->fwd;
    WDGS_REQUIRE(op->encoded && f->encoded && op->ranges_used, WDGS_E_STATE, "TiledRasterizer.encodeDepth before encode: depth is composited from the frame encode rasterized");
    WDGS_REQUIRE(op->width == f->cfg.viewport_width && op->height == f->cfg.viewport_height, WDGS_E_STATE,
                 "TiledRasterizer.encodeDepth: the forward pass viewport changed to %ux%u since the last encode (%ux%u)", f->cfg.viewport_width, f->cfg.viewport_height,
                 op->width, op->height);
    WDGS_REQUIRE(f->settings.gaussian_mode >= 0.5f, WDGS_E_STATE, "TiledRasterizer.encodeDepth: the forward pass is in point-cloud render mode, which has no weights");
    wdgs_device* d = op->dev;
    if (op->depth_width != op->width || op->depth_height != op->height) {
        bool any = false;
        for (float* img : op->depth) any = any || img != nullptr;
        if (any) {
            WDGS_REQUIRE(!d->capturing, WDGS_E_STATE, "TiledRasterizer.encodeDepth re-allocates its images after a size change: run one eager encodeDepth before recording");
            (void)wdgs_sync_lanes(d);
            for (float*& img : op->depth) { free_dev(img); img = nullptr; }
        }
        op->depth_width = op->width;
        op->depth_height = op->height;
    }
    for (u32 k = 0; k < 3u; k++) {
        if (!((kinds >> k) & 1u) || op->depth[k]) continue;
        WDGS_REQUIRE(!d->capturing, WDGS_E_STATE, "TiledRasterizer.encodeDepth allocates a depth image on first use of its kind: run one eager encodeDepth before recording");
        WDGS_TRY(wdgs_alloc((void**)&op->depth[k], (size_t)op->width * op->height * 4, true, d->stream));
    }
    const int fo = wdgs_sorter_final_out_index(f->sorter);
    WDGS_TRY(launch_depth_composite(d, f->settings, f->tile_info, f->splats, f->cfg.num_points, f->depths, op->ranges_used, wdgs_sorter_keys(f->sorter, fo),
                                    wdgs_sorter_values(f->sorter, fo), f->stats, op->compat_caps ? 32u : 0u, (kinds & WDGS_DEPTH_WEIGHT_SUM) ? op->depth[2] : nullptr,
                                    (kinds & WDGS_DEPTH_EXPECTED) ? op->depth[0] : nullptr, (kinds & WDGS_DEPTH_MEDIAN) ? op->depth[1] : nullptr, f->nf_stamp,
                                    f->stats + FRAME_WORD));
    op->depth_encoded = kinds;
    return WDGS_OK;
}
int wdgs_tiled_rasterizer_get_depth(wdgs_tiled_rasterizer* op, uint32_t kind, void** out) {
    WDGS_REQUIRE(op && out, WDGS_E_INVALID, "wdgs_tiled_rasterizer_get_depth: null argument");
    WDGS_REQUIRE(kind == WDGS_DEPTH_EXPECTED || kind == WDGS_DEPTH_MEDIAN || kind == WDGS_DEPTH_WEIGHT_SUM, WDGS_E_INVALID,
                 "wdgs_tiled_rasterizer_get_depth: kind 0x%x is not one WDGS_DEPTH_* bit", kind);
    const u32 k = kind == WDGS_DEPTH_EXPECTED ? 0u : kind == WDGS_DEPTH_MEDIAN ? 1u : 2u;
    WDGS_REQUIRE((op->depth_encoded & kind) && op->depth[k], WDGS_E_STATE, "TiledRasterizer: depth image of this kind not encoded yet (call encodeDepth with it first)");
    *out = op->depth[k];
    return WDGS_OK;
}
#define RASTER_GETTER(fn, field, what)                                                                            \
    int fn(wdgs_tiled_rasterizer* op, void** out) {                                                               \
        WDGS_REQUIRE(op && out, WDGS_E_INVALID, #fn ": null argument");                                           \
        WDGS_REQUIRE(op->encoded && op->field, WDGS_E_STATE, "TiledRasterizer: " what " not created yet (call encode first)"); \
        *out = op->field;                                                                                         \
        return WDGS_OK;                                                                                           \
    }
RASTER_GETTER(wdgs_tiled_rasterizer_get_output, rgba8, "output texture")
RASTER_GETTER(wdgs_tiled_rasterizer_get_alpha, alpha, "alpha texture")
RASTER_GETTER(wdgs_tiled_rasterizer_get_n_contrib, n_contrib, "n_contrib texture")
RASTER_GETTER(wdgs_tiled_rasterizer_get_tile_offsets, ranges_used, "tile offsets")
#undef RASTER_GETTER

int wdgs_tiled_rasterizer_blit(wdgs_tiled_rasterizer* op, void* target, uint32_t tw, uint32_t th) {
    WDGS_REQUIRE(op && target, WDGS_E_INVALID, "wdgs_tiled_rasterizer_blit: null argument");
    WDGS_REQUIRE(op->encoded && op->rgba8, WDGS_E_STATE, "TiledRasterizer: no output texture to blit from. Call encode() first.");
    WDGS_REQUIRE(tw > 0 && th > 0, WDGS_E_INVALID, "wdgs_tiled_rasterizer_blit: empty target %ux%u", tw, th);
    return launch_downsample(op->dev, op->rgba8, op->width, op->height, target, tw, th);
}

static int backward_alloc_images(wdgs_tiled_backward* op, u32 w, u32 h) {
    const u32 px = w * h;
    if (px <= op->img_capacity) return WDGS_OK;
    (void)wdgs_sync_lanes(op->dev);
    free_dev(op->loss_image); free_dev(op->metric_err); free_dev(op->metric_flags);
    op->loss_image = nullptr; op->metric_err = nullptr; op->metric_flags = nullptr;
    WDGS_TRY(wdgs_alloc((void**)&op->loss_image, (size_t)px * 16, true, op->dev->stream));
    WDGS_TRY(wdgs_alloc((void**)&op->metric_err, (size_t)px * 4, true, op->dev->stream));
    WDGS_TRY(wdgs_alloc((void**)&op->metric_flags, (size_t)px * 4, true, op->dev->stream));
    op->img_capacity = px;
    return WDGS_OK;
}

static int backward_alloc_per_point(wdgs_tiled_backward* op, u32 capacity) {
    wdgs_device* d = op->dev;
    int r = wdgs_alloc((void**)&op->acc, (size_t)capacity * 48 + 16, true, d->stream);
    if (r == WDGS_OK) op->acc_dirty = reinterpret_cast<u32*>(reinterpret_cast<char*>(op->acc) + (size_t)capacity * 48);
    if (r == WDGS_OK) r = wdgs_alloc((void**)&op->gradients, (size_t)capacity * 32, true, d->stream);
    if (r == WDGS_OK) r = wdgs_alloc((void**)&op->metric_counts, (size_t)capacity * 4, true, d->stream);
    if (r == WDGS_OK) op->points_capacity = capacity;
    return r;
}
int wdgs_tiled_backward_resize(wdgs_tiled_backward* op, uint32_t n) {
    WDGS_REQUIRE(op, WDGS_E_INVALID, "wdgs_tiled_backward_resize: null op");
    wdgs_device* d = op->dev;
    WDGS_REQUIRE(!d->capturing, WDGS_E_STATE, "wdgs_tiled_backward_resize while recording a command buffer");
    WDGS_CHECK_HIP(hipSetDevice(d->ordinal));
    WDGS_CHECK_HIP(wdgs_sync_lanes(d));
    const u32 need = std::max(n, 1u);
    if (need > op->points_capacity) {
        free_dev(op->acc); free_dev(op->gradients); free_dev(op->metric_counts);
        op->acc = nullptr; op->gradients = nullptr; op->metric_counts = nullptr;
        op->points_capacity = 0;
        WDGS_TRY(backward_alloc_per_point(op, (u32)std::min<uint64_t>((uint64_t)need + need / 4, 0xFFFFFFFFull)));
    } else {
        WDGS_CHECK_HIP(hipMemsetAsync(op->acc, 0, (size_t)need * 48, d->stream));
        WDGS_CHECK_HIP(hipMemsetAsync(op->acc_dirty, 0, 16, d->stream));
        WDGS_CHECK_HIP(hipMemsetAsync(op->gradients, 0, (size_t)need * 32, d->stream));
        WDGS_CHECK_HIP(hipMemsetAsync(op->metric_counts, 0, (size_t)need * 4, d->stream));
    }
    op->cfg.num_points = n;
    return WDGS_OK;
}
int wdgs_tiled_backward_create(wdgs_device* d, const wdgs_tiled_backward_config* cfg, wdgs_tiled_backward** out) {
    WDGS_REQUIRE(d && cfg && out, WDGS_E_INVALID, "wdgs_tiled_backward_create: null argument");
    WDGS_REQUIRE(cfg->viewport_width > 0 && cfg->viewport_height > 0, WDGS_E_INVALID, "viewport must be non-empty");
    wdgs_tiled_backward* op = new wdgs_tiled_backward();
    std::memset(op, 0, sizeof(*op));
    op->dev = d;
    op->cfg = *cfg;
    op->gradient_output = true;
    if (op->cfg.training.c1 == 0.f) op->cfg.training.c1 = 0.01f * 0.01f;
    if (op->cfg.training.c2 == 0.f) op->cfg.training.c2 = 0.03f * 0.03f;
    op->settings = RenderSettings{cfg->gaussian_scale != 0.f ? cfg->gaussian_scale : 1.0f, (float)cfg->sh_deg, (float)cfg->viewport_width,
                                  (float)cfg->viewport_height, cfg->point_size_px != 0.f ? cfg->point_size_px : 3.0f, 0.0f,
                                  cfg->max_splat_radius_px != 0.f ? cfg->max_splat_radius_px : 128.0f};
    int r = backward_alloc_per_point(op, std::max(cfg->num_points, 1u));
    if (r == WDGS_OK) r = wdgs_alloc((void**)&op->metric_minmax, 4096, true, d->stream);
    if (r == WDGS_OK) r = backward_alloc_images(op, cfg->viewport_width, cfg->viewport_height);
    if (r != WDGS_OK) { wdgs_tiled_backward_destroy(op); return r; }
    *out = op;
    return WDGS_OK;
}
int wdgs_tiled_backward_destroy(wdgs_tiled_backward* op) {
    if (!op) return WDGS_OK;
    sync_if_alive(op->dev);
    free_dev(op->acc); free_dev(op->gradients); free_dev(op->loss_image); free_dev(op->metric_counts);
    free_dev(op->metric_err); free_dev(op->metric_flags); free_dev(op->metric_minmax);
    delete op;
    return WDGS_OK;
}
int wdgs_tiled_backward_set_gradient_output(wdgs_tiled_backward* op, int enabled) {
    WDGS_REQUIRE(op, WDGS_E_INVALID, "wdgs_tiled_backward_set_gradient_output: null op");
    op->gradient_output = enabled != 0;
    return WDGS_OK;
}
static int backward_loss(wdgs_tiled_backward* op, const void* pred, const void* targ, void* acc, u32 acc_rows, const void* acc_dirty) {
    const u32 w = op->cfg.viewport_width, h = op->cfg.viewport_height;
    if (op->dssim_mode == WDGS_DSSIM_GAUSSIAN) return launch_dssim_grad(op->dev, w, h, pred, targ, op->cfg.training, op->loss_image, acc, acc_rows, acc_dirty);
    return launch_loss_grad(op->dev, w, h, pred, targ, op->cfg.training, op->loss_image, acc, acc_rows, acc_dirty);
}
int wdgs_tiled_backward_compute_loss_only(wdgs_tiled_backward* op, const void* pred, const void* targ) {
    WDGS_REQUIRE(op && pred && targ, WDGS_E_INVALID, "wdgs_tiled_backward_compute_loss_only: null argument");
    return backward_loss(op, pred, targ, nullptr, 0u, nullptr);
}
static int backward_encode_raster(wdgs_tiled_backward* op, const void* pred, const void* targ, const wdgs_tiled_backward_resources* res) {
    wdgs_device* d = op->dev;
    const u32 w = op->cfg.viewport_width, h = op->cfg.viewport_height, n = op->cfg.num_points;
    if (w > 0 && h > 0) WDGS_TRY(backward_loss(op, pred, targ, op->acc, std::max(n, 1u), op->acc_dirty));
    else WDGS_TRY(launch_acc_clear_if_dirty(d, op->acc, n, op->acc_dirty));
    const LongWork* lw = nullptr;
    auto owner = d->range_tables.find(res->tile_offsets_buffer);
    if (owner != d->range_tables.end() && owner->second->ranges_valid && owner->second->long_lists.hdr) lw = &owner->second->long_lists;
    return launch_backward_rasterize(d, op->settings, ceil_div(w, 16), ceil_div(h, 16), res->tile_offsets_buffer, res->tile_indices_buffer, res->splat_buffer,
                                     res->alpha_texture, res->n_contrib_texture, op->loss_image, op->acc, op->acc_dirty, lw);
}
int wdgs_tiled_backward_encode(wdgs_tiled_backward* op, const void* pred, const void* targ, const wdgs_tiled_backward_resources* res,
                               const void* gaussians) {
    WDGS_REQUIRE(op && pred && targ && res && gaussians, WDGS_E_INVALID, "wdgs_tiled_backward_encode: null argument");
    WDGS_REQUIRE(res->splat_buffer && res->tile_offsets_buffer && res->tile_indices_buffer && res->camera_buffer && res->alpha_texture && res->n_contrib_texture,
                 WDGS_E_INVALID, "wdgs_tiled_backward_encode: incomplete resources");
    WDGS_TRY(backward_encode_raster(op, pred, targ, res));
    return launch_geometry_backward(op->dev, op->cfg.num_points, res->camera_buffer, op->settings, gaussians, op->acc, op->gradients);
}
int wdgs_tiled_backward_encode_raster(wdgs_tiled_backward* op, const void* pred, const void* targ, const wdgs_tiled_backward_resources* res) {
    WDGS_REQUIRE(op && pred && targ && res, WDGS_E_INVALID, "wdgs_tiled_backward_encode_raster: null argument");
    WDGS_REQUIRE(res->splat_buffer && res->tile_offsets_buffer && res->tile_indices_buffer && res->alpha_texture && res->n_contrib_texture, WDGS_E_INVALID,
                 "wdgs_tiled_backward_encode_raster: incomplete resources");
    return backward_encode_raster(op, pred, targ, res);
}
int wdgs_tiled_backward_encode_geometry(wdgs_tiled_backward* op, const void* camera, const void* gaussians, const wdgs_view_accumulate* into) {
    WDGS_REQUIRE(op && camera && gaussians, WDGS_E_INVALID, "wdgs_tiled_backward_encode_geometry: null argument");
    if (!into) return launch_geometry_backward(op->dev, op->cfg.num_points, camera, op->settings, gaussians, op->acc, op->gradients);
    WDGS_REQUIRE(into->sums && into->visible && into->tile_counts && into->guard && into->overflow_word, WDGS_E_INVALID,
                 "wdgs_tiled_backward_encode_geometry: incomplete accumulate target");
    return launch_geometry_backward_accumulate(op->dev, op->cfg.num_points, camera, op->settings, gaussians, op->acc, op->acc_dirty, op->gradients, into->sums, into->visible,
                                               into->tile_counts, into->guard, into->overflow_word, into->first ? 1u : 2u);
}
int wdgs_tiled_backward_encode_geometry_views(wdgs_tiled_backward* const* ops, const void* const* cameras, const void* const* tile_counts, const void* const* overflow_words,
                                              uint32_t count, const void* gaussians, void* sums, void* visible, void* guard, int write_gradients, int continues) {
    WDGS_REQUIRE(ops && cameras && tile_counts && overflow_words && gaussians && sums && visible && guard && count > 0 && count <= WDGS_MAX_BATCH_VIEWS, WDGS_E_INVALID,
                 "wdgs_tiled_backward_encode_geometry_views: invalid argument");
    wdgs_tiled_backward* b0 = ops[0];
    WDGS_REQUIRE(b0, WDGS_E_INVALID, "wdgs_tiled_backward_encode_geometry_views: null pass");
    void *accs[WDGS_MAX_BATCH_VIEWS], *dirty[WDGS_MAX_BATCH_VIEWS], *grads[WDGS_MAX_BATCH_VIEWS];
    for (u32 v = 0; v < count; v++) {
        wdgs_tiled_backward* b = ops[v];
        WDGS_REQUIRE(b && cameras[v] && tile_counts[v] && overflow_words[v], WDGS_E_INVALID, "wdgs_tiled_backward_encode_geometry_views: null argument for view %u", v);
        for (u32 u = 0; u < v; u++) WDGS_REQUIRE(ops[u] != b, WDGS_E_INVALID, "wdgs_tiled_backward_encode_geometry_views: pass %u is given twice (every view has accumulators of its own)", v);
        WDGS_REQUIRE(b->dev == b0->dev && b->cfg.num_points == b0->cfg.num_points && std::memcmp(&b->settings, &b0->settings, sizeof(RenderSettings)) == 0, WDGS_E_STATE,
                     "wdgs_tiled_backward_encode_geometry_views: pass %u differs from pass 0 (cloud size, viewport or settings)", v);
        accs[v] = b->acc; dirty[v] = b->acc_dirty; grads[v] = b->gradients;
    }
    return launch_geometry_backward_views(b0->dev, b0->cfg.num_points, count, cameras, b0->settings, gaussians, accs, dirty, tile_counts, overflow_words,
                                          write_gradients ? grads : nullptr, sums, visible, guard, continues ? 1u : 0u);
}
int wdgs_tiled_backward_compute_metric_map(wdgs_tiled_backward* op, const void* pred, const void* targ, float threshold) {
    WDGS_REQUIRE(op && pred && targ, WDGS_E_INVALID, "wdgs_tiled_backward_compute_metric_map: null argument");
    return launch_metric_map(op->dev, op->cfg.viewport_width, op->cfg.viewport_height, pred, targ, 1000000.0f, threshold, op->metric_err, op->metric_minmax,
                             op->metric_minmax + 2, op->metric_flags);
}
int wdgs_tiled_backward_compute_metric_counts(wdgs_tiled_backward* op, const wdgs_tiled_backward_resources* res, uint32_t num_instances, int clear) {
    WDGS_REQUIRE(op && res && res->splat_buffer && res->tile_offsets_buffer && res->tile_indices_buffer && res->n_contrib_texture, WDGS_E_INVALID,
                 "wdgs_tiled_backward_compute_metric_counts: incomplete resources");
    const u32 n = op->cfg.num_points;
    u32* const counts = op->metric_counts_into ? op->metric_counts_into : op->metric_counts;
    if (clear) WDGS_CHECK_HIP(hipMemsetAsync(counts, 0, (size_t)std::max(n, 1u) * 4, op->dev->stream));
    return launch_metric_count(op->dev, op->settings, ceil_div(op->cfg.viewport_width, 16), ceil_div(op->cfg.viewport_height, 16), res->tile_offsets_buffer,
                               res->tile_indices_buffer, num_instances, res->splat_buffer, n, op->metric_flags, res->n_contrib_texture, counts, n);
}
int wdgs_tiled_backward_normalize_metric_counts(wdgs_tiled_backward* op, uint32_t divisor) {
    WDGS_REQUIRE(op, WDGS_E_INVALID, "null op");
    return launch_metric_normalize(op->dev, op->cfg.num_points, divisor, op->metric_counts);
}
int wdgs_tiled_backward_set_viewport(wdgs_tiled_backward* op, uint32_t w, uint32_t h) {
    WDGS_REQUIRE(op && w > 0 && h > 0, WDGS_E_INVALID, "wdgs_tiled_backward_set_viewport: invalid argument");
    op->cfg.viewport_width = w;
    op->cfg.viewport_height = h;
    op->settings.viewport_x = (float)w;
    op->settings.viewport_y = (float)h;
    return backward_alloc_images(op, w, h);
}
int wdgs_tiled_backward_set_training_config(wdgs_tiled_backward* op, const wdgs_training_config* cfg) {
    WDGS_REQUIRE(op && cfg, WDGS_E_INVALID, "null argument");
    op->cfg.training = *cfg;
    if (op->cfg.training.c1 == 0.f) op->cfg.training.c1 = 0.01f * 0.01f;
    if (op->cfg.training.c2 == 0.f) op->cfg.training.c2 = 0.03f * 0.03f;
    return WDGS_OK;
}
int wdgs_tiled_backward_set_dssim_mode(wdgs_tiled_backward* op, uint32_t mode) {
    WDGS_REQUIRE(op, WDGS_E_INVALID, "wdgs_tiled_backward_set_dssim_mode: null op");
    WDGS_REQUIRE(mode == WDGS_DSSIM_REFERENCE || mode == WDGS_DSSIM_GAUSSIAN, WDGS_E_INVALID, "wdgs_tiled_backward_set_dssim_mode: unknown mode %u", mode);
    op->dssim_mode = mode;
    return WDGS_OK;
}
int wdgs_tiled_backward_get_dssim_mode(const wdgs_tiled_backward* op, uint32_t* out) {
    WDGS_REQUIRE(op && out, WDGS_E_INVALID, "wdgs_tiled_backward_get_dssim_mode: null argument");
    *out = op->dssim_mode;
    return WDGS_OK;
}
void* wdgs_tiled_backward_gradients(wdgs_tiled_backward* op) { return op ? op->gradients : nullptr; }
void* wdgs_tiled_backward_metric_counts(wdgs_tiled_backward* op) { return op ? op->metric_counts : nullptr; }
int wdgs_tiled_backward_set_metric_counts_target(wdgs_tiled_backward* op, void* counts_dev) {
    WDGS_REQUIRE(op, WDGS_E_INVALID, "wdgs_tiled_backward_set_metric_counts_target: null op");
    op->metric_counts_into = (u32*)counts_dev;
    return WDGS_OK;
}
void* wdgs_tiled_backward_loss_image(wdgs_tiled_backward* op) { return op ? op->loss_image : nullptr; }
void* wdgs_tiled_backward_metric_map(wdgs_tiled_backward* op) { return op ? op->metric_flags : nullptr; }
void* wdgs_tiled_backward_accumulators(wdgs_tiled_backward* op) { return op ? op->acc : nullptr; }
void* wdgs_tiled_backward_metric_minmax(wdgs_tiled_backward* op) { return op ? op->metric_minmax : nullptr; }

int wdgs_downsample_rgba8(wdgs_device* d, const void* src, uint32_t sw, uint32_t sh, void* dst, uint32_t dw, uint32_t dh) {
    WDGS_REQUIRE(d && src && dst && sw && sh && dw && dh, WDGS_E_INVALID, "wdgs_downsample_rgba8: invalid argument");
    return launch_downsample(d, src, sw, sh, dst, dw, dh);
}

int wdgs_optimizer_state_sizes(uint32_t n, size_t sizes[6]) {
    WDGS_REQUIRE(sizes, WDGS_E_INVALID, "null argument");
    const size_t N = std::max(n, 1u);
    sizes[0] = sizes[1] = sizes[2] = N * 48;
    sizes[3] = N * 12;
    sizes[4] = N * 48 * 4;
    sizes[5] = N * 48 * 2 * 4;
    return WDGS_OK;
}

static void optimizer_free_state(wdgs_optimizer* op) {
    free_dev(op->state.opt_pos); free_dev(op->state.opt_rot); free_dev(op->state.opt_scale);
    free_dev(op->state.opt_opacity); free_dev(op->state.param_sh); free_dev(op->state.state_sh);
    std::memset(&op->state, 0, sizeof(op->state));
}

int wdgs_optimizer_create(wdgs_device* d, uint32_t n, const wdgs_adam_hyperparameters* params, const void* gaussians, const void* sh,
                          const wdgs_optimizer_state* initial, int owns_state, uint32_t initial_iteration, wdgs_optimizer** out) {
    WDGS_REQUIRE(d && out, WDGS_E_INVALID, "wdgs_optimizer_create: null argument");
    wdgs_optimizer* op = new wdgs_optimizer();
    std::memset(op, 0, sizeof(*op));
    op->dev = d;
    op->num_points = n;
    const wdgs_adam_hyperparameters defaults = {0.00016f, 0.0025f, 0.05f, 0.005f, 0.001f, 0.9f, 0.999f, 1e-8f};
    op->params = params ? *params : defaults;
    if (initial) {
        WDGS_REQUIRE(initial->opt_pos && initial->opt_rot && initial->opt_scale && initial->opt_opacity && initial->param_sh && initial->state_sh,
                     WDGS_E_INVALID, "wdgs_optimizer_create: incomplete initial state");
        op->state = *initial;
        op->owns_state = owns_state != 0;
        op->iteration = initial_iteration;
    } else {
        if (!(gaussians && sh)) { delete op; wdgs_set_error("wdgs_optimizer_create: point cloud required when no initial state is given"); return WDGS_E_INVALID; }
        size_t sz[6];
        wdgs_optimizer_state_sizes(n, sz);
        void** fields[6] = {&op->state.opt_pos, &op->state.opt_rot, &op->state.opt_scale, &op->state.opt_opacity, &op->state.param_sh, &op->state.state_sh};
        op->owns_state = true;
        for (int i = 0; i < 6; i++) {
            int r = wdgs_alloc(fields[i], sz[i], true, d->stream);
            if (r != WDGS_OK) { optimizer_free_state(op); delete op; return r; }
        }
        int r = launch_unpack(d, n, gaussians, sh, op->state);
        if (r != WDGS_OK) { optimizer_free_state(op); delete op; return r; }
        op->iteration = 0;
    }
// ... 155 lines not shown
```

### webdgs_amd/csrc/dssim.hip

```cpp
#include "common.h"
#include "dmath.h"

namespace {

WD_DEV float sgn(float v) { return v > 0.0f ? 1.0f : (v < 0.0f ? -1.0f : 0.0f); }

constexpr u32 DT = 32;
constexpr u32 DR = 5;
constexpr u32 DK = SSIM_TAPS;
constexpr u32 ME = DT + 2u * DR;
constexpr u32 IE = ME + 2u * DR;
constexpr u32 IN_WORDS = IE * IE;
constexpr u32 IN_PER_THREAD = (IN_WORDS + 255u) / 256u;
constexpr u32 MP = ME + 1u;
constexpr u32 NP = DT + 1u;
constexpr u32 P_FLOATS = 3u * ME * MP > 2u * IN_WORDS ? 3u * ME * MP : 2u * IN_WORDS;
constexpr u32 H_FLOATS = 5u * IE * ME;
static_assert(3u * ME * NP <= H_FLOATS, "dssim LDS layout");

constexpr u32 H1_OUT = 3;
constexpr u32 H1_SEGS = ME / H1_OUT;
constexpr u32 V1_OUT = 7;
constexpr u32 V1_ITEMS = ME * (ME / V1_OUT);
constexpr u32 H2_OUT = 4;
// ... 41 lines not shown
        const bool in = t < IN_WORDS && gx >= 0 && gx < (int)W && gy >= 0 && gy < (int)H;
        const size_t p = in ? (size_t)gy * W + (size_t)gx : 0;
        ra[i] = in ? pred[p] : 0u;
        rb[i] = in ? targ[p] : 0u;
    }
    const u32 lx = threadIdx.x & (DT - 1u), ly0 = (threadIdx.x / DT) * V2_OUT;
    const u32 ox = (u32)bx + lx;
    u32 pa[V2_OUT], pb[V2_OUT];
#pragma unroll
    for (u32 k = 0; k < V2_OUT; k++) {
        const u32 oy = (u32)by + ly0 + k;
        const bool in = ox < W && oy < H;
        const size_t p = in ? (size_t)oy * W + ox : 0;
        pa[k] = in ? pred[p] : 0u;
        pb[k] = in ? targ[p] : 0u;
    }
    const u32 cx = min((u32)bx + DT / 2u, W - 1u), cy = min((u32)by + DT / 2u, H - 1u);
    const u32 a0 = pred[(size_t)cy * W + cx], b0 = targ[(size_t)cy * W + cx];
    float g[3][V2_OUT];
    __syncthreads();

#pragma unroll 1
    for (u32 c = 0; c < 3u; c++) {
        const u32 sh = 8u * c;
        const float s = (s_lut[(a0 >> sh) & 0xFFu] + s_lut[(b0 >> sh) & 0xFFu]) * 0.5f;
#pragma unroll
        for (u32 i = 0; i < IN_PER_THREAD; i++) {
            const u32 t = threadIdx.x + 256u * i;
            if (t < IN_WORDS) {
                s_x[t] = s_lut[(ra[i] >> sh) & 0xFFu] - s;
                s_y[t] = s_lut[(rb[i] >> sh) & 0xFFu] - s;
            }
        }
        __syncthreads();
        for (u32 it = threadIdx.x; it < IE * H1_SEGS; it += 256u) {
            const u32 r = it / H1_SEGS, c0 = (it % H1_SEGS) * H1_OUT;
            float xs[H1_OUT + DK - 1u], ys[H1_OUT + DK - 1u];
#pragma unroll
            for (u32 j = 0; j < H1_OUT + DK - 1u; j++) { xs[j] = s_x[r * IE + c0 + j]; ys[j] = s_y[r * IE + c0 + j]; }
#pragma unroll
            for (u32 o = 0; o < H1_OUT; o++) {
                float mx = 0.f, my = 0.f, xx = 0.f, yy = 0.f, xy = 0.f;
#pragma unroll
                for (u32 k = 0; k < DK; k++) {
                    const float x = xs[o + k], y = ys[o + k], w = win.g[k];
                    mx = __builtin_fmaf(w, x, mx);
                    my = __builtin_fmaf(w, y, my);
                    xx = __builtin_fmaf(w, x * x, xx);
                    yy = __builtin_fmaf(w, y * y, yy);
                    xy = __builtin_fmaf(w, x * y, xy);
                }
                const u32 h = r * ME + c0 + o;
                s_h[0u * IE * ME + h] = mx; s_h[1u * IE * ME + h] = my; s_h[2u * IE * ME + h] = xx; s_h[3u * IE * ME + h] = yy; s_h[4u * IE * ME + h] = xy;
            }
        }
        __syncthreads();
        if (threadIdx.x < V1_ITEMS) {
            const u32 col = threadIdx.x % ME, r0 = (threadIdx.x / ME) * V1_OUT;
            float v[V1_OUT][5];
#pragma unroll
            for (u32 o = 0; o < V1_OUT; o++)
#pragma unroll
                for (u32 q = 0; q < 5u; q++) v[o][q] = 0.f;
#pragma unroll
            for (u32 j = 0; j < V1_OUT + DK - 1u; j++) {
                float hq[5];
#pragma unroll
                for (u32 q = 0; q < 5u; q++) hq[q] = s_h[q * IE * ME + (r0 + j) * ME + col];
#pragma unroll
                for (u32 o = 0; o < V1_OUT; o++)
                    if (j >= o && j - o < DK) {
#pragma unroll
                        for (u32 q = 0; q < 5u; q++) v[o][q] = __builtin_fmaf(win.g[j - o], hq[q], v[o][q]);
                    }
            }
            const int gx = bx - (int)DR + (int)col;
#pragma unroll
            for (u32 o = 0; o < V1_OUT; o++) {
                const int gy = by - (int)DR + (int)(r0 + o);
                float ma = 0.f, md = 0.f, mg = 0.f;
                if (gx >= 0 && gx < (int)W && gy >= 0 && gy < (int)H) dssim_maps(v[o], s, cfg.c1, cfg.c2, ma, md, mg);
                const u32 m = (r0 + o) * MP + col;
                s_p[0u * ME * MP + m] = ma; s_p[1u * ME * MP + m] = md; s_p[2u * ME * MP + m] = mg;
            }
        }
        __syncthreads();
        for (u32 it = threadIdx.x; it < ME * (DT / H2_OUT); it += 256u) {
            const u32 r = it % ME, c0 = (it / ME) * H2_OUT;
            float n[3][H2_OUT];
#pragma unroll
            for (u32 m = 0; m < 3u; m++)
#pragma unroll
                for (u32 o = 0; o < H2_OUT; o++) n[m][o] = 0.f;
#pragma unroll
            for (u32 j = 0; j < H2_OUT + DK - 1u; j++) {
                float t[3];
#pragma unroll
                for (u32 m = 0; m < 3u; m++) t[m] = s_p[m * ME * MP + r * MP + c0 + j];
#pragma unroll
                for (u32 o = 0; o < H2_OUT; o++)
                    if (j >= o && j - o < DK) {
#pragma unroll
                        for (u32 m = 0; m < 3u; m++) n[m][o] = __builtin_fmaf(win.g[j - o], t[m], n[m][o]);
                    }
            }
#pragma unroll
            for (u32 m = 0; m < 3u; m++)
#pragma unroll
                for (u32 o = 0; o < H2_OUT; o++) s_h[m * ME * NP + r * NP + c0 + o] = n[m][o];
        }
        __syncthreads();
        {
            float n[3][V2_OUT];
#pragma unroll
            for (u32 m = 0; m < 3u; m++)
#pragma unroll
                for (u32 o = 0; o < V2_OUT; o++) n[m][o] = 0.f;
#pragma unroll
            for (u32 j = 0; j < V2_OUT + DK - 1u; j++) {
                float t[3];
#pragma unroll
                for (u32 m = 0; m < 3u; m++) t[m] = s_h[m * ME * NP + (ly0 + j) * NP + lx];
#pragma unroll
                for (u32 o = 0; o < V2_OUT; o++)
                    if (j >= o && j - o < DK) {
#pragma unroll
                        for (u32 m = 0; m < 3u; m++) n[m][o] = __builtin_fmaf(win.g[j - o], t[m], n[m][o]);
                    }
            }
#pragma unroll
            for (u32 o = 0; o < V2_OUT; o++) {
                const float xp = s_lut[(pa[o] >> sh) & 0xFFu] - s, yp = s_lut[(pb[o] >> sh) & 0xFFu] - s;
                g[c][o] = (n[0][o] + xp * n[1][o]) + (yp - xp) * n[2][o];
            }
        }
    }
#pragma unroll
    for (u32 o = 0; o < V2_OUT; o++) {
        const u32 oy = (u32)by + ly0 + o;
        if (ox >= W || oy >= H) continue;
        const float d[3] = {s_lut[pa[o] & 0xFFu] - s_lut[pb[o] & 0xFFu], s_lut[(pa[o] >> 8) & 0xFFu] - s_lut[(pb[o] >> 8) & 0xFFu],
                            s_lut[(pa[o] >> 16) & 0xFFu] - s_lut[(pb[o] >> 16) & 0xFFu]};
        float4 r;
        r.x = cfg.lambda_l1 * sgn(d[0]) + cfg.lambda_l2 * d[0] - cfg.lambda_dssim * g[0][o];
        r.y = cfg.lambda_l1 * sgn(d[1]) + cfg.lambda_l2 * d[1] - cfg.lambda_dssim * g[1][o];
        r.z = cfg.lambda_l1 * sgn(d[2]) + cfg.lambda_l2 * d[2] - cfg.lambda_dssim * g[2][o];
        r.w = 1.0f;
        out[(size_t)oy * W + ox] = r;
    }
}

}

int launch_loss_grad(wdgs_device*, u32, u32, const void*, const void*, const wdgs_training_config&, void*, void*, u32, const void*);

int launch_dssim_grad(wdgs_device* dev, u32 W, u32 H, const void* pred, const void* targ, const wdgs_training_config& cfg, void* out, void* acc, u32 acc_rows,
                      const void* acc_dirty) {
    if (W == 0 || H == 0) return WDGS_OK;
    if (cfg.lambda_dssim == 0.0f) return launch_loss_grad(dev, W, H, pred, targ, cfg, out, acc, acc_rows, acc_dirty);
    WDGS_LAUNCH(dev, "dssim_grad", dssim_grad_kernel, dim3(ceil_div(W, DT), ceil_div(H, DT)), dim3(256), 0, W, H, (const u32*)pred, (const u32*)targ, cfg,
                ssim_window(), (float4*)out, (int4*)acc, acc_rows * 3u , (const u32*)acc_dirty);
    WDGS_CHECK_HIP(hipGetLastError());
    return WDGS_OK;
}
```

### webdgs_amd/csrc/loss.hip

```cpp
#include "common.h"
#include "dmath.h"

namespace {

typedef wd_pair f2;

WD_DEV float sgn(float v) { return v > 0.0f ? 1.0f : (v < 0.0f ? -1.0f : 0.0f); }

constexpr u32 LT = 32;
constexpr u32 LH = LT + 4;

template <u32 PPT>
__global__ __launch_bounds__(256) void loss_grad_kernel(u32 W, u32 H, const u32* __restrict__ pred, const u32* __restrict__ targ,
                                                         wdgs_training_config cfg, float4* __restrict__ out, int4* __restrict__ acc, u32 acc_quads,
                                                         const u32* __restrict__ acc_dirty) {
    if (acc && *acc_dirty != 0u) {
        const int4 z = make_int4(0, 0, 0, 0);
        const u32 nblk = gridDim.x * gridDim.y, blk = blockIdx.y * gridDim.x + blockIdx.x;
        for (u32 i = blk * 256u + threadIdx.x; i < acc_quads; i += nblk * 256u) acc[i] = z;
    }
    __shared__ float s_lut[256];
    constexpr u32 TH = 8u * PPT, HH = TH + 4u;
    __shared__ float4 sp[HH][LH];
    __shared__ float2 st[HH][LH];
    s_lut[threadIdx.x] = wd_div((float)threadIdx.x, 255.0f);
    __syncthreads();
    const int bx = blockIdx.x * LT, by = blockIdx.y * TH;
    for (u32 t = threadIdx.x; t < HH * LH; t += 256u) {
        const int hy = (int)(t / LH), hx = (int)(t % LH);
        int gx = bx + hx - 2, gy = by + hy - 2;
        gx = gx < 0 ? 0 : (gx > (int)W - 1 ? (int)W - 1 : gx);
        gy = gy < 0 ? 0 : (gy > (int)H - 1 ? (int)H - 1 : gy);
        const u32 a = pred[(size_t)gy * W + gx], b = targ[(size_t)gy * W + gx];
        sp[hy][hx] = make_float4(s_lut[a & 0xFFu], s_lut[(a >> 8) & 0xFFu], s_lut[(a >> 16) & 0xFFu], s_lut[b & 0xFFu]);
        st[hy][hx] = make_float2(s_lut[(b >> 8) & 0xFFu], s_lut[(b >> 16) & 0xFFu]);
    }
    __syncthreads();
    const u32 lx = threadIdx.x & (LT - 1u), ly0 = (threadIdx.x / LT) * PPT;
    const u32 x = bx + lx, y0 = by + ly0;
    if (x >= W || y0 >= H) return;

    const bool dssim = cfg.lambda_dssim > 0.0f;
    const float n = 25.0f;
    float mx[PPT][3], my[PPT][3], sx2[PPT][3], sy2[PPT][3], sxy[PPT][3];
    if (dssim) {
        f2 mxa[PPT], mxb[PPT], mya[PPT], myb[PPT];
#pragma unroll
        for (u32 k = 0; k < PPT; k++) mxa[k] = mxb[k] = mya[k] = myb[k] = f2{0.f, 0.f};
#pragma unroll
        for (u32 r = 0; r < PPT + 4u; r++) {
#pragma unroll
            for (u32 c = 0; c < 5u; c++) {
                const float4 a = sp[ly0 + r][lx + c];
                const float2 b = st[ly0 + r][lx + c];
#pragma unroll
                for (u32 k = 0; k < PPT; k++)
                    if (r >= k && r <= k + 4u) {
                        mxa[k] += f2{a.x, a.y}; mxb[k].x += a.z;
                        mya[k] += f2{a.w, b.x}; myb[k].x += b.y;
                    }
            }
#pragma unroll
            for (u32 k = 0; k < PPT; k++)
                asm volatile("" : "+v"(mxa[k].x), "+v"(mxa[k].y), "+v"(mxb[k].x), "+v"(mya[k].x), "+v"(mya[k].y), "+v"(myb[k].x));
        }
        f2 sx2a[PPT], sx2b[PPT], sy2a[PPT], sy2b[PPT], sxya[PPT], sxyb[PPT], ma[PPT], mb[PPT], na[PPT], nb[PPT];
#pragma unroll
        for (u32 k = 0; k < PPT; k++) {
            mx[k][0] = wd_div_inrange(mxa[k].x, n); mx[k][1] = wd_div_inrange(mxa[k].y, n); mx[k][2] = wd_div_inrange(mxb[k].x, n);
            my[k][0] = wd_div_inrange(mya[k].x, n); my[k][1] = wd_div_inrange(mya[k].y, n); my[k][2] = wd_div_inrange(myb[k].x, n);
            ma[k] = f2{mx[k][0], mx[k][1]}; mb[k] = f2{mx[k][2], 0.f};
            na[k] = f2{my[k][0], my[k][1]}; nb[k] = f2{my[k][2], 0.f};
            sx2a[k] = sx2b[k] = sy2a[k] = sy2b[k] = sxya[k] = sxyb[k] = f2{0.f, 0.f};
        }
#pragma unroll
        for (u32 r = 0; r < PPT + 4u; r++) {
#pragma unroll
            for (u32 c = 0; c < 5u; c++) {
                const float4 a = sp[ly0 + r][lx + c];
                const float2 b = st[ly0 + r][lx + c];
#pragma unroll
                for (u32 k = 0; k < PPT; k++)
                    if (r >= k && r <= k + 4u) {
                        const f2 daa = f2{a.x, a.y} - ma[k];
                        const float dab = a.z - mb[k].x;
                        const f2 dba = f2{a.w, b.x} - na[k];
                        const float dbb = b.y - nb[k].x;
                        sx2a[k].x = __builtin_fmaf(daa.x, daa.x, sx2a[k].x); sx2a[k].y = __builtin_fmaf(daa.y, daa.y, sx2a[k].y);
                        sx2b[k].x = __builtin_fmaf(dab, dab, sx2b[k].x);
                        sy2a[k].x = __builtin_fmaf(dba.x, dba.x, sy2a[k].x); sy2a[k].y = __builtin_fmaf(dba.y, dba.y, sy2a[k].y);
                        sy2b[k].x = __builtin_fmaf(dbb, dbb, sy2b[k].x);
                        sxya[k].x = __builtin_fmaf(daa.x, dba.x, sxya[k].x); sxya[k].y = __builtin_fmaf(daa.y, dba.y, sxya[k].y);
                        sxyb[k].x = __builtin_fmaf(dab, dbb, sxyb[k].x);
                    }
            }
#pragma unroll
            for (u32 k = 0; k < PPT; k++)
                asm volatile("" : "+v"(sx2a[k].x), "+v"(sx2a[k].y), "+v"(sx2b[k].x), "+v"(sy2a[k].x), "+v"(sy2a[k].y), "+v"(sy2b[k].x), "+v"(sxya[k].x),
                             "+v"(sxya[k].y), "+v"(sxyb[k].x));
        }
#pragma unroll
        for (u32 k = 0; k < PPT; k++) {
            sx2[k][0] = sx2a[k].x; sx2[k][1] = sx2a[k].y; sx2[k][2] = sx2b[k].x;
            sy2[k][0] = sy2a[k].x; sy2[k][1] = sy2a[k].y; sy2[k][2] = sy2b[k].x;
            sxy[k][0] = sxya[k].x; sxy[k][1] = sxya[k].y; sxy[k][2] = sxyb[k].x;
        }
    }
#pragma unroll
    for (u32 k = 0; k < PPT; k++) {
        const u32 y = y0 + k;
        if (y >= H) break;
        const float4 p = sp[ly0 + k + 2u][lx + 2u];
        const float2 t = st[ly0 + k + 2u][lx + 2u];
        const float d[3] = {p.x - p.w, p.y - t.x, p.z - t.y};
        float g[3] = {0.0f, 0.0f, 0.0f};
        if (dssim) {
#pragma unroll
            for (int c = 0; c < 3; c++) {
                const float vx = wd_div_inrange(sx2[k][c], n), vy = wd_div_inrange(sy2[k][c], n), vxy = wd_div_inrange(sxy[k][c], n);
                const float num1 = 2.0f * mx[k][c] * my[k][c] + cfg.c1;
                const float num2 = 2.0f * vxy + cfg.c2;
                const float den1 = mx[k][c] * mx[k][c] + my[k][c] * my[k][c] + cfg.c1;
                const float den2 = vx + vy + cfg.c2;
                const float den = den1 * den2;
                const float ssim = (cfg.c1 > 0.0f && cfg.c2 > 0.0f) ? wd_div_inrange(num1 * num2, den) : wd_div(num1 * num2, den);
                g[c] = ((1.0f - ssim) * 0.5f) * d[c];
            }
        }
        float4 o;
        o.x = cfg.lambda_l1 * sgn(d[0]) + cfg.lambda_l2 * d[0] + cfg.lambda_dssim * g[0];
        o.y = cfg.lambda_l1 * sgn(d[1]) + cfg.lambda_l2 * d[1] + cfg.lambda_dssim * g[1];
        o.z = cfg.lambda_l1 * sgn(d[2]) + cfg.lambda_l2 * d[2] + cfg.lambda_dssim * g[2];
        o.w = 1.0f;
        out[(size_t)y * W + x] = o;
    }
}

}

int launch_loss_grad(wdgs_device* dev, u32 W, u32 H, const void* pred, const void* targ, const wdgs_training_config& cfg, void* out, void* acc, u32 acc_rows,
                     const void* acc_dirty) {
    if (W == 0 || H == 0) return WDGS_OK;
#define WDGS_LOSS_LAUNCH(PPT_)                                                                                                                                       \
    WDGS_LAUNCH(dev, "loss_grad", loss_grad_kernel<PPT_>, dim3(ceil_div(W, LT), ceil_div(H, 8u * PPT_)), dim3(256), 0, W, H, (const u32*)pred, (const u32*)targ, cfg, \
                (float4*)out, (int4*)acc, acc_rows * 3u , (const u32*)acc_dirty)
    if ((size_t)W * H <= 640u * 480u) { WDGS_LOSS_LAUNCH(1u); } else { WDGS_LOSS_LAUNCH(2u); }
#undef WDGS_LOSS_LAUNCH
    WDGS_CHECK_HIP(hipGetLastError());
    return WDGS_OK;
}
```

### webdgs_amd/ops.py

```python
from __future__ import annotations

import ctypes as C
import dataclasses
import re
from typing import Optional

import numpy as np
import torch

from . import _lib
from ._lib import CapacityError, StateError, WdgsError, check


MAX_LANES = 4
MAX_BATCH_VIEWS = 16


class HipBuffer:

    def __init__(self, device: "HipDevice", ptr: int, size: int, owner: Optional[torch.Tensor] = None, label: str = ""):
        self.device, self.ptr, self.size, self._owner, self.label = device, int(ptr or 0), int(size), owner, label
        self.destroyed = False
        self.before_read = None

# ... 359 lines not shown
        check(self.device.lib.wdgs_tiled_forward_get_resources(self.handle, C.byref(r)))
        return r

    def getResources(self) -> dict:
        r, d, n = self._res(), self.device, max(1, self.pointCloud.num_points)
        return dict(splatBuffer=d.view(r.splat_buffer, 24 * n), depthsBuffer=d.view(r.depths_buffer, 4 * n),
                    tileKeysBuffer=d.view(r.tile_keys_buffer, 4 * r.max_tile_entries), tileIndicesBuffer=d.view(r.tile_indices_buffer, 4 * r.max_tile_entries),
                    tileOffsetsBuffer=d.view(r.tile_offsets_buffer, 4 * n), tileCountsBuffer=d.view(r.tile_counts_buffer, 4 * n),
                    statsBuffer=d.view(r.stats_buffer, 16), numTilesX=r.num_tiles_x, numTilesY=r.num_tiles_y, totalTiles=r.total_tiles,
                    maxTileEntries=r.max_tile_entries, settings=np.array(list(r.settings), np.float32))

    def getSortedIndicesBuffer(self) -> HipBuffer:
        return self.getResources()["tileIndicesBuffer"]

    def getSortedKeysBuffer(self) -> HipBuffer:
        return self.getResources()["tileKeysBuffer"]

    def getTileOffsetsBuffer(self) -> HipBuffer:
        return self.getResources()["tileOffsetsBuffer"]

    def getStatsBuffer(self) -> HipBuffer:
        return self.getResources()["statsBuffer"]

    def check(self) -> np.ndarray:
        st = (C.c_uint32 * 4)()
        check(self.device.lib.wdgs_tiled_forward_check(self.handle, st))
        return np.array(list(st), np.uint32)

    def setLongLists(self, threshold: int, maxItems: int = 0, maxRows: int = 0) -> None:
        check(self.device.lib.wdgs_tiled_forward_set_long_lists(self.handle, int(threshold), int(maxItems), int(maxRows)))

    def longListStats(self) -> dict:
        st = (C.c_uint32 * 12)()
        check(self.device.lib.wdgs_tiled_forward_long_list_stats(self.handle, st))
        keys = ("blocksWanted", "itemsWanted", "forwardQueue", "backwardQueue", "rowsUsed", "rowsWanted", "stalled", "_", "maxItems", "maxBlocks", "maxRows", "threshold")
        return {k: int(v) for k, v in zip(keys, st) if k != "_"}

    def destroy(self) -> None:
        if self.destroyed:
            return
        self.destroyed = True
        self.device.lib.wdgs_tiled_forward_destroy(self.handle)
        self.handle = None


DEPTH_KINDS = {"expected": 1, "median": 2, "weight_sum": 4}


def _depth_mask(kinds) -> int:
    mask = 0
    for k in ((kinds,) if isinstance(kinds, str) else kinds):
        if k not in DEPTH_KINDS:
            raise ValueError(f"unknown depth kind {k!r}: one of {sorted(DEPTH_KINDS)}")
        mask |= DEPTH_KINDS[k]
    return mask


class TiledRasterizer:

    def __init__(self, config: dict):
        self.device: HipDevice = config["device"]
        self.forwardPass: TiledForwardPass = config["forwardPass"]
        self.destroyed = False
        self.width = self.height = 0
        h = C.c_void_p()
        check(self.device.lib.wdgs_tiled_rasterizer_create(self.device.handle, self.forwardPass.handle, 1 if config.get("compatCaps") else 0, C.byref(h)))
        self.handle = h

    def encode(self, encoder: Optional[HipEncoder], width: int, height: int) -> None:
        check(self.device.lib.wdgs_tiled_rasterizer_encode(self.handle, int(width), int(height)))
        self.width, self.height = int(width), int(height)

    def _get(self, fn, nbytes: int) -> HipBuffer:
        p = C.c_void_p()
        check(fn(self.handle, C.byref(p)))
        return self.device.view(p.value, nbytes)

    def getOutputTextureView(self) -> HipBuffer:
        return self._get(self.device.lib.wdgs_tiled_rasterizer_get_output, 4 * self.width * self.height)

    def getAlphaTextureView(self) -> HipBuffer:
        return self._get(self.device.lib.wdgs_tiled_rasterizer_get_alpha, 4 * self.width * self.height)

    def getNContribTextureView(self) -> HipBuffer:
        return self._get(self.device.lib.wdgs_tiled_rasterizer_get_n_contrib, 4 * self.width * self.height)

    def getTileOffsetsBuffer(self) -> HipBuffer:
        tiles = ((self.width + 15) // 16) * ((self.height + 15) // 16)
        return self._get(self.device.lib.wdgs_tiled_rasterizer_get_tile_offsets, 4 * (tiles + 1))

    def encodeDepth(self, encoder: Optional[HipEncoder], kinds=("expected",)) -> None:
        mask = int(kinds) if isinstance(kinds, (int, np.integer)) else _depth_mask(kinds)
        check(self.device.lib.wdgs_tiled_rasterizer_encode_depth(self.handle, mask))

    def getDepthTextureView(self, kind: str = "expected") -> HipBuffer:
        p = C.c_void_p()
        check(self.device.lib.wdgs_tiled_rasterizer_get_depth(self.handle, _depth_mask((kind,)), C.byref(p)))
        return self.device.view(p.value, 4 * self.width * self.height)

    def blitToTexture(self, encoder: Optional[HipEncoder], target: HipBuffer, width: Optional[int] = None, height: Optional[int] = None) -> None:
        w, h = int(width or self.width), int(height or self.height)
        if self.handle is not None and w * h * 4 > target.size:
            raise _lib.WdgsError(_lib.WDGS_E_INVALID, f"blitToTexture: target of {target.size} bytes is smaller than {w}x{h} rgba8")
        check(self.device.lib.wdgs_tiled_rasterizer_blit(self.handle, target.ptr, max(w, 0), max(h, 0)))

    def destroy(self) -> None:
        if self.destroyed:
            return
        self.destroyed = True
        self.device.lib.wdgs_tiled_rasterizer_destroy(self.handle)
        self.handle = None


def _training_config(tc: Optional[dict]) -> _lib.TrainingConfig:
    tc = tc or {}
    return _lib.TrainingConfig(float(tc.get("lambda_l1", 0.8)), float(tc.get("lambda_l2", 0.0)), float(tc.get("lambda_dssim", 0.2)),
                               float(tc.get("c1", 0.01 * 0.01)), float(tc.get("c2", 0.03 * 0.03)))


DSSIM_MODES = {"reference": 0, "gaussian": 1}


def dssim_mode(tc: Optional[dict]) -> int:
    mode = (tc or {}).get("dssim_mode")
    mode = "reference" if mode is None else mode
    if not isinstance(mode, str) or mode not in DSSIM_MODES:
        raise ValueError(f"dssim_mode must be one of {sorted(DSSIM_MODES)}, not {mode!r}")
    return DSSIM_MODES[mode]


class TiledBackwardPass:

    def __init__(self, device: HipDevice, pointCloud: PointCloud, config: dict):
        mode = dssim_mode(config.get("trainingConfig"))
        self.device, self.pointCloud = device, pointCloud
        self.destroyed = False
        self.viewportWidth, self.viewportHeight = int(config["viewportWidth"]), int(config["viewportHeight"])
        self.trainingConfig = dict(config.get("trainingConfig") or {})
        cfg = _lib.TiledBackwardConfig(pointCloud.num_points, pointCloud.sh_deg, self.viewportWidth, self.viewportHeight, _training_config(self.trainingConfig),
                                       float(config.get("gaussianScale", 1.0)), float(config.get("pointSizePx", 3.0)),
                                       float(config.get("maxSplatRadiusPx", 128.0)))
        h = C.c_void_p()
        check(device.lib.wdgs_tiled_backward_create(device.handle, C.byref(cfg), C.byref(h)))
        self.handle = h
        if mode:
            check(device.lib.wdgs_tiled_backward_set_dssim_mode(h, mode))

    @staticmethod
    def _resources(res: dict) -> _lib.TiledBackwardResources:
        def p(k):
            b = res.get(k)
            return b.ptr if b is not None else None
        return _lib.TiledBackwardResources(p("splatBuffer"), p("tileOffsetsBuffer"), p("tileIndicesBuffer"), p("cameraBuffer"), p("alphaTexture"),
                                           p("nContribTexture"))

    def setPointCloud(self, pointCloud: PointCloud) -> bool:
        if pointCloud.sh_deg != self.pointCloud.sh_deg:
            return False
        check(self.device.lib.wdgs_tiled_backward_resize(self.handle, pointCloud.num_points))
        self.pointCloud = pointCloud
        return True

    def encode(self, encoder: Optional[HipEncoder], predictedTexture: HipBuffer, targetTexture: HipBuffer, forwardResources: dict, options=None) -> None:
        r = self._resources(forwardResources)
        check(self.device.lib.wdgs_tiled_backward_encode(self.handle, predictedTexture.ptr, targetTexture.ptr, C.byref(r), self.pointCloud.gaussian_3d_buffer.ptr))

    def encodeRaster(self, encoder: Optional[HipEncoder], predictedTexture: HipBuffer, targetTexture: HipBuffer, forwardResources: dict) -> None:
        r = self._resources(forwardResources)
        check(self.device.lib.wdgs_tiled_backward_encode_raster(self.handle, predictedTexture.ptr, targetTexture.ptr, C.byref(r)))

    def encodeGeometry(self, encoder: Optional[HipEncoder], cameraBuffer: HipBuffer, accumulate: Optional[dict] = None) -> None:
        into = None
        if accumulate is not None:
            a = accumulate
            into = C.byref(_lib.ViewAccumulate(a["sums"].ptr, a["visible"].ptr, a["tileCounts"].ptr, a["guard"].ptr, a["stats"].ptr + 8, 1 if a["first"] else 0))
        check(self.device.lib.wdgs_tiled_backward_encode_geometry(self.handle, cameraBuffer.ptr, self.pointCloud.gaussian_3d_buffer.ptr, into))

    def computeLossOnly(self, encoder, predictedTexture: HipBuffer, targetTexture: HipBuffer) -> None:
        check(self.device.lib.wdgs_tiled_backward_compute_loss_only(self.handle, predictedTexture.ptr, targetTexture.ptr))

    def computeMetricMap(self, encoder, predictedTexture: HipBuffer, targetTexture: HipBuffer, options: Optional[dict] = None) -> None:
        thr = float((options or {}).get("threshold", 0.5))
        check(self.device.lib.wdgs_tiled_backward_compute_metric_map(self.handle, predictedTexture.ptr, targetTexture.ptr, thr))

    def computeMetricCounts(self, encoder, resources: dict, options: Optional[dict] = None) -> None:
        r = self._resources(resources)
        clear = 1 if (options or {}).get("clear", True) else 0
        n_inst = resources["tileIndicesBuffer"].size // 4
        check(self.device.lib.wdgs_tiled_backward_compute_metric_counts(self.handle, C.byref(r), n_inst, clear))

    def normalizeMetricCounts(self, encoder, options: dict) -> None:
        check(self.device.lib.wdgs_tiled_backward_normalize_metric_counts(self.handle, max(1, int(options["divisor"]))))

    def setViewport(self, width: int, height: int) -> None:
        check(self.device.lib.wdgs_tiled_backward_set_viewport(self.handle, int(width), int(height)))
        self.viewportWidth, self.viewportHeight = int(width), int(height)

    def setTrainingConfig(self, next_cfg: dict) -> None:
        merged = dict(self.trainingConfig, **{k: v for k, v in next_cfg.items() if v is not None})
        mode = dssim_mode(merged)
        self.trainingConfig = merged
        tc = _training_config(self.trainingConfig)
        check(self.device.lib.wdgs_tiled_backward_set_training_config(self.handle, C.byref(tc)))
        check(self.device.lib.wdgs_tiled_backward_set_dssim_mode(self.handle, mode))

    def setGradientOutput(self, enabled: bool) -> None:
        check(self.device.lib.wdgs_tiled_backward_set_gradient_output(self.handle, 1 if enabled else 0))

    def getGradientsBuffer(self) -> HipBuffer:
        return self.device.view(self.device.lib.wdgs_tiled_backward_gradients(self.handle), 32 * max(1, self.pointCloud.num_points))

    def setMetricCountsTarget(self, counts: Optional[HipBuffer]) -> None:
        self._metric_target = counts
        check(self.device.lib.wdgs_tiled_backward_set_metric_counts_target(self.handle, counts.ptr if counts is not None else None))

    def getMetricCountsBuffer(self) -> HipBuffer:
        return self.device.view(self.device.lib.wdgs_tiled_backward_metric_counts(self.handle), 4 * max(1, self.pointCloud.num_points))

    def getLossTextureView(self) -> HipBuffer:
        return self.device.view(self.device.lib.wdgs_tiled_backward_loss_image(self.handle), 16 * self.viewportWidth * self.viewportHeight)

    def getMetricMapTextureView(self) -> HipBuffer:
        return self.device.view(self.device.lib.wdgs_tiled_backward_metric_map(self.handle), 4 * self.viewportWidth * self.viewportHeight)

    def getMetricMapTexture(self) -> HipBuffer:
        return self.getMetricMapTextureView()

    def getAccumulatorsBuffer(self) -> HipBuffer:
        return self.device.view(self.device.lib.wdgs_tiled_backward_accumulators(self.handle), 48 * max(1, self.pointCloud.num_points))

    def getMetricMinMaxBuffer(self) -> HipBuffer:
        return self.device.view(self.device.lib.wdgs_tiled_backward_metric_minmax(self.handle), 8)

    def destroy(self) -> None:
        if self.destroyed:
            return
        self.destroyed = True
        self.device.lib.wdgs_tiled_backward_destroy(self.handle)
        self.handle = None


def downsampleRGBA8(device: HipDevice, src: HipBuffer, src_w: int, src_h: int, dst: HipBuffer, dst_w: int, dst_h: int) -> None:
    check(device.lib.wdgs_downsample_rgba8(device.handle, src.ptr, src_w, src_h, dst.ptr, dst_w, dst_h))


def depthToRGBA8(device: HipDevice, depth: HipBuffer, width: int, height: int, near: float, far: float, target: HipBuffer) -> None:
    n = int(width) * int(height)
    if depth.size < 4 * n or target.size < 4 * n:
        raise ValueError(f"depthToRGBA8: buffers too small for {width}x{height}")
    check(device.lib.wdgs_depth_to_rgba8(device.handle, depth.ptr, int(width), int(height), float(near), float(far), target.ptr))


def encodeImageSSE(device: HipDevice, a: HipBuffer, b: HipBuffer, num_pixels: int, out: HipBuffer) -> None:
    check(device.lib.wdgs_image_sse_rgb8(device.handle, a.ptr, b.ptr, int(num_pixels), out.ptr))


def imageSSE(device: HipDevice, a: HipBuffer, b: HipBuffer, num_pixels: int) -> int:
    out = device.createBuffer(8, "sse")
    check(device.lib.wdgs_image_sse_rgb8(device.handle, a.ptr, b.ptr, int(num_pixels), out.ptr))
    return int(out.read(np.uint64, count=1)[0])


def imagePSNR(device: HipDevice, a: HipBuffer, b: HipBuffer, num_pixels: int) -> float:
    sse = imageSSE(device, a, b, num_pixels)
    return float("inf") if sse == 0 else 10.0 * float(np.log10(255.0 * 255.0 * 3.0 * num_pixels / sse))


def psnrFromSSE(sse: int, num_pixels: int) -> float:
    return float("inf") if int(sse) == 0 else 10.0 * float(np.log10(255.0 * 255.0 * 3.0 * num_pixels / int(sse)))


def encodeImageSSIM(device: HipDevice, a: HipBuffer, b: HipBuffer, width: int, height: int, out: HipBuffer, map: Optional[HipBuffer] = None) -> None:
    n = int(width) * int(height)
    if a.size < 4 * n or b.size < 4 * n or out.size < 8 or (map is not None and map.size < 12 * n):
        raise ValueError(f"encodeImageSSIM: buffers too small for {width}x{height}")
    check(device.lib.wdgs_image_ssim_rgb8(device.handle, a.ptr, b.ptr, int(width), int(height), out.ptr, map.ptr if map is not None else None))


def imageSSIM(device: HipDevice, a: HipBuffer, b: HipBuffer, width: int, height: int, map: Optional[HipBuffer] = None) -> float:
    out = device.createBuffer(8, "ssim")
    encodeImageSSIM(device, a, b, width, height, out, map)
    return float(out.read(np.float64, count=1)[0])


DEFAULT_ADAM_HYPERPARAMETERS = dict(lr_pos=0.00016, lr_color=0.0025, lr_opacity=0.05, lr_scale=0.005, lr_rot=0.001, beta1=0.9, beta2=0.999, epsilon=1e-8)
_STATE_FIELDS = ("optPosBuffer", "optRotBuffer", "optScaleBuffer", "optOpacityBuffer", "paramSH", "stateSH")


def allocateOptimizerStateBuffers(device: HipDevice, numPoints: int) -> dict:
    sizes = (C.c_size_t * 6)()
    check(device.lib.wdgs_optimizer_state_sizes(int(numPoints), C.byref(sizes)))
    return {k: device.createBuffer(sizes[i], k) for i, k in enumerate(_STATE_FIELDS)}


def _state_struct(buffers: dict) -> _lib.OptimizerState:
    return _lib.OptimizerState(*[buffers[k].ptr for k in _STATE_FIELDS])


class Optimizer:

    def __init__(self, device: HipDevice, pointCloud: PointCloud, params: Optional[dict] = None, initialState: Optional[dict] = None):
        self.device, self.numPoints = device, pointCloud.num_points
        self.params = {**DEFAULT_ADAM_HYPERPARAMETERS, **(params or {})}
        self.destroyed = False
        hp = _lib.AdamHyperparameters(*[float(self.params[k]) for k in DEFAULT_ADAM_HYPERPARAMETERS])
        if initialState and initialState.get("buffers"):
            self.buffers = initialState["buffers"]
            it = int(initialState.get("iteration") or 0)
            fresh = False
        else:
            self.buffers = allocateOptimizerStateBuffers(device, self.numPoints)
            it, fresh = 0, True
        st = _state_struct(self.buffers)
        h = C.c_void_p()
        check(device.lib.wdgs_optimizer_create(device.handle, self.numPoints, C.byref(hp), None, None, C.byref(st), 0, it, C.byref(h)))
        self.handle = h
        self._deferred_cloud: Optional[PointCloud] = None
        if fresh:
            check(device.lib.wdgs_optimizer_init_from_point_cloud(h, pointCloud.gaussian_3d_buffer.ptr, pointCloud.sh_buffer.ptr))

    def getIteration(self) -> int:
        return int(self.device.lib.wdgs_optimizer_get_iteration(self.handle))

    def getHyperparameters(self) -> dict:
        return dict(self.params)

    def setHyperparameters(self, next_params: dict) -> None:
        self.params.update(next_params)
        hp = _lib.AdamHyperparameters(*[float(self.params[k]) for k in DEFAULT_ADAM_HYPERPARAMETERS])
        check(self.device.lib.wdgs_optimizer_set_hyperparameters(self.handle, C.byref(hp)))

    def getStateBuffers(self) -> dict:
        st = _lib.OptimizerState()
        check(self.device.lib.wdgs_optimizer_get_state(self.handle, C.byref(st)))
        for b in self.buffers.values():
            if b.before_read is None:
                b.before_read = self._flush_state
        return self.buffers

    def _flush_state(self) -> None:
        if not self.destroyed and self.handle:
            st = _lib.OptimizerState()
            check(self.device.lib.wdgs_optimizer_get_state(self.handle, C.byref(st)))

    def setDeferredSH(self, pointCloud: PointCloud, enabled: bool = True) -> Optional[HipBuffer]:
        check(self.device.lib.wdgs_optimizer_set_deferred_sh(self.handle, pointCloud.sh_buffer.ptr, 1 if enabled else 0))
        self._deferred_cloud = pointCloud if enabled else None
        pointCloud.sh_buffer.before_read = (lambda: self.flushSH(pointCloud)) if enabled else None
        ptr = self.device.lib.wdgs_optimizer_dc_words(self.handle)
        words = self.device.view(ptr, 8 * max(1, self.numPoints), "sh-dc words") if (enabled and ptr) else None
        pointCloud.dc_words = words
        return words

    def flushSH(self, pointCloud: PointCloud) -> None:
        if not self.destroyed and self.handle:
            check(self.device.lib.wdgs_optimizer_flush_sh(self.handle, pointCloud.sh_buffer.ptr))

    def applyRepackedRows(self, rows: HipBuffer, skipFirst: int, skipCount: int, guard: Optional[HipBuffer], pointCloud: PointCloud) -> None:
        check(self.device.lib.wdgs_optimizer_apply_repacked_rows(self.handle, rows.ptr, int(skipFirst), int(skipCount), guard.ptr if guard is not None else None,
                                                                 pointCloud.gaussian_3d_buffer.ptr, pointCloud.sh_buffer.ptr))

    def advanceIteration(self, count: int = 1) -> None:
        check(self.device.lib.wdgs_optimizer_advance_iteration(self.handle, int(count)))

    def step(self, encoder, coefficients: PointCloud, gradientsBuffer: HipBuffer, tileCountsBuffer: HipBuffer) -> None:
        check(self.device.lib.wdgs_optimizer_step(self.handle, coefficients.gaussian_3d_buffer.ptr, coefficients.sh_buffer.ptr, gradientsBuffer.ptr, tileCountsBuffer.ptr))

    def stepWithGeometry(self, encoder, coefficients: PointCloud, backwardPass: "TiledBackwardPass", cameraBuffer: HipBuffer, tileCountsBuffer: HipBuffer) -> None:
        check(self.device.lib.wdgs_optimizer_step_with_geometry(self.handle, backwardPass.handle, cameraBuffer.ptr, coefficients.gaussian_3d_buffer.ptr,
                                                                coefficients.sh_buffer.ptr, tileCountsBuffer.ptr))

    def stepF32(self, encoder, coefficients: PointCloud, gradF32: HipBuffer, visibleCounts: HipBuffer) -> None:
        check(self.device.lib.wdgs_optimizer_step_f32(self.handle, coefficients.gaussian_3d_buffer.ptr, coefficients.sh_buffer.ptr, gradF32.ptr, visibleCounts.ptr))

    def stepF32Range(self, encoder, coefficients: PointCloud, gradF32: HipBuffer, visibleCounts: HipBuffer, first: int, count: int,
                     rowsOut: Optional[HipBuffer] = None) -> None:
        check(self.device.lib.wdgs_optimizer_step_f32_range(self.handle, coefficients.gaussian_3d_buffer.ptr, coefficients.sh_buffer.ptr, gradF32.ptr,
                                                            visibleCounts.ptr, int(first), int(count), rowsOut.ptr if rowsOut is not None else None))

    def setGuard(self, flagBuffer: Optional[HipBuffer], offset: int = 0) -> None:
        check(self.device.lib.wdgs_optimizer_set_guard(self.handle, (flagBuffer.ptr + offset) if flagBuffer is not None else None))

    def stateChanged(self) -> None:
        check(self.device.lib.wdgs_optimizer_state_changed(self.handle))

    def destroy(self) -> None:
        if self.destroyed:
            return
        pc = self._deferred_cloud
        if pc is not None and self.device.handle and not pc.sh_buffer.destroyed:
            try:
                self.setDeferredSH(pc, False)
            except _lib.WdgsError:
                pc.sh_buffer.before_read = None
        self.destroyed = True
        self.device.lib.wdgs_optimizer_destroy(self.handle)
# ... 151 lines not shown
```

### webdgs_amd/trainer.py

```python
from __future__ import annotations

import math
import os
import random
import time
from typing import Optional

import numpy as np
import torch

from . import loaders, ops, parallel


class Trainer:
    def __init__(self, device: ops.HipDevice, trainingConfig: Optional[dict] = None, seed: int = 0, world_size: int = 1, rank: int = 0,
                 views_per_rank: int = 1, maxTileEntries: int = 0, use_command_buffers: bool = True, exchange: Optional[parallel.Exchange] = None,
                 overlap_views: Optional[bool] = None, pipeline_depth: int = 1, batch_views: Optional[bool] = None):
        ops.dssim_mode(trainingConfig)
        self.device = device
        self.trainingConfig = dict(trainingConfig or dict(lambda_l1=0.8, lambda_l2=0.0, lambda_dssim=0.2))
        self.optimizerHyperparameters = dict(ops.DEFAULT_ADAM_HYPERPARAMETERS)
        self.world_size, self.rank, self.views_per_rank = int(world_size), int(rank), max(1, int(views_per_rank))
        self.maxTileEntries = int(maxTileEntries)
        self._grown_tile_entries = 0
        self._foreign_overflow_warned = False
        self.exchange = exchange if exchange is not None else (parallel.default_exchange(device, self.world_size) if self.world_size > 1 else parallel.Exchange())
        self._sliced = self.world_size > 1 or bool(getattr(self.exchange, "force", False))
        if self.world_size > 1 and (self.exchange.world_size, self.exchange.rank) != (self.world_size, self.rank):
            raise ValueError(f"exchange is rank {self.exchange.rank} of {self.exchange.world_size}, trainer is rank {self.rank} of {self.world_size}")
        self.use_command_buffers = bool(use_command_buffers)
        self._cmd_cache: dict = {}
        self._eager_steps = 0
        if overlap_views is None:
            overlap_views = int(os.environ.get("WDGS_LANES", self.DEFAULT_LANES))
        elif isinstance(overlap_views, bool):
            overlap_views = self.DEFAULT_LANES if overlap_views else 1
        self._lanes = max(1, min(int(overlap_views), self.views_per_rank, ops.MAX_LANES))
        self.batch_views = self.views_per_rank > 1 and (os.environ.get("WDGS_BATCH_VIEWS", "1") != "0" if batch_views is None else bool(batch_views))
        self._op_sets = min(self.views_per_rank, ops.MAX_BATCH_VIEWS) if self.batch_views else self._lanes
        self.view_group = int(os.environ.get("WDGS_VIEW_GROUP", "0"))
        self._camera_buffers: list = []
        self._rng = random.Random(seed)

        self.forwardPass = self.rasterizer = self.backwardPass = self.optimizer = None
        self.pipeline_depth = max(1, min(int(pipeline_depth), 4))
        self.reuse_passes = True
        self.fuse_geometry_adam = True
        self.keep_gradients = os.environ.get("WDGS_KEEP_GRADIENTS", "0") == "1"
        self.deferred_sh = os.environ.get("WDGS_DEFERRED_SH", "1") != "0"
        self._dc_words: Optional[ops.HipBuffer] = None
        self._gradient_output_applied: Optional[bool] = None
        self._tickets: list = []
        self._more_op_sets: list = []
        self.metricsForwardPass = self.metricsRasterizer = self.metricsPass = None
        self.metricsViewportWidth = self.metricsViewportHeight = 0
        self.metricsTarget: Optional[ops.HipBuffer] = None
        self.metric_lanes = max(1, min(int(os.environ.get("WDGS_METRIC_LANES", self.DEFAULT_LANES)), ops.MAX_LANES))
        self._more_metric_sets: list = []
        self.pointCloud: Optional[ops.PointCloud] = None
        self.cameraBuffer = device.createBuffer(272, "camera uniform")
        self.metricsCameraBuffer = device.createBuffer(272, "metrics camera uniform")

        self.isTraining = False
        self.iteration = 0
        self.maxIterations = 10_000
        self.stepItersPerSec = 0.0
        self.stepMs = 0.0
        self.lastDensifyPruneIteration: Optional[int] = None
        self.lastViewportWidth = self.lastViewportHeight = 1
        self.pendingPointCloudSwap: Optional[dict] = None
        self.trainCameras: list = []
        self.images: list = []
        self.evalCameras: list = []
        self.evalImages: list = []
        self._eval_camera_buffers: list = []
        self._eval_sets: dict = {}
        self.evalMaxTileEntries = 0
        self._eval_tile_entries = 0
        self._eval_long_lists: Optional[dict] = None

        self.densifyPruneConfig = dict(
            schedule=dict(enabled=True, warmupIterations=500, interval=100, stopIterations=15_000),
            metricViews=10, metricDownscale=2, metricThreshold=0.5, maxBufferBytes=128 * 1024 * 1024, maxNewPointsPerStep=5000,
            pruneOpacity=0.01, cloneThresholdCount=500, splitScaleThreshold=1.0)
        self.densifyPrune = ops.DensifyPrunePass(device, self._densify_op_config())
        self._dp_grad: Optional[ops.HipBuffer] = None
        self._dp_visible: Optional[ops.HipBuffer] = None
        self._dp_rows: Optional[ops.HipBuffer] = None
        self._dp_flag: Optional[ops.HipBuffer] = None
        self._agree_word: Optional[ops.HipBuffer] = None
        self.longLists: Optional[dict] = None
        self._state_sliced = False
        self.exchange_timing = False
        self._exchange_events: list = []

    DEFAULT_LANES = 3
    _OP_NAMES = ("forwardPass", "rasterizer", "backwardPass", "metricsForwardPass", "metricsRasterizer", "metricsPass", "optimizer")

    def _destroy_more_metric_sets(self) -> None:
        for more in self._more_metric_sets:
            for op in more[:3]:
                op.destroy()
        self._more_metric_sets = []

    def _destroy_more_op_sets(self) -> None:
        for ops_of_lane in self._more_op_sets:
            for op in ops_of_lane:
                op.destroy()
        self._more_op_sets = []

    def _densify_op_config(self) -> dict:
        c = self.densifyPruneConfig
        return dict(strategy="gpu_rebuild", numViews=c["metricViews"], maxBufferBytes=c["maxBufferBytes"], maxNewPointsPerStep=c["maxNewPointsPerStep"],
                    pruneThreshold=c["pruneOpacity"], cloneThreshold=c["cloneThresholdCount"], splitThreshold=c["splitScaleThreshold"])

    def setPointCloud(self, pointCloud: ops.PointCloud) -> None:
        self.applyPointCloudSwap(dict(pointCloud=pointCloud))

    def requestPointCloudSwap(self, pointCloud: ops.PointCloud, optimizerInitialState: Optional[dict] = None) -> None:
        self.pendingPointCloudSwap = dict(pointCloud=pointCloud, optimizerInitialState=optimizerInitialState)

    def consumePointCloudSwapRequest(self) -> Optional[dict]:
        req, self.pendingPointCloudSwap = self.pendingPointCloudSwap, None
        return req

    def requestResizeTo(self, numPoints: int) -> None:
        if self.pointCloud is None:
            return
        self.requestPointCloudSwap(ops.allocatePointCloudLike(self.device, self.pointCloud, dict(numPoints=numPoints)))

    def applyPointCloudSwap(self, request: dict) -> None:
        self.drain()
        self._synchronize()
        oldParams = self.optimizer.getHyperparameters() if self.optimizer else None
        if self.optimizer is not None:
            self.optimizer.destroy()
            self.optimizer = None
        old = self.pointCloud
        self.pointCloud = request["pointCloud"]
        self._invalidate_command_buffers()
        passes = [self.forwardPass, self.backwardPass, self.metricsForwardPass, self.metricsPass] + [op for more in self._more_op_sets + self._more_metric_sets for op in (more[0], more[2])]
        kept = self.reuse_passes and old is not None and all(p.setPointCloud(self.pointCloud) for p in passes if p is not None)
        if not kept:
            for name in self._OP_NAMES:
                op = getattr(self, name)
                if op is not None:
                    op.destroy()
                setattr(self, name, None)
            self._destroy_more_op_sets()
            self._destroy_more_metric_sets()
        self.optimizer = ops.Optimizer(self.device, self.pointCloud, oldParams or self.optimizerHyperparameters, request.get("optimizerInitialState"))
        self.optimizerHyperparameters = dict(self.optimizer.getHyperparameters())
        self._dc_words = self.optimizer.setDeferredSH(self.pointCloud, True) if self.deferred_sh else None
        for fw in self._forward_passes():
            fw.setDcSource(self._dc_words)
        if old is not None and old is not self.pointCloud:
            old.gaussian_3d_buffer.destroy()
            old.sh_buffer.destroy()
        self._dp_grad = self._dp_visible = self._dp_rows = self._dp_flag = None
        self._state_sliced = False
        self.ensurePipelines(self.lastViewportWidth, self.lastViewportHeight)

    def _forward_passes(self) -> list:
        return [p for p in [self.forwardPass, self.metricsForwardPass] + [more[0] for more in self._more_op_sets + self._more_metric_sets] if p is not None]

    def flushPointCloud(self) -> None:
        if self.optimizer is not None and self.pointCloud is not None:
            self.optimizer.flushSH(self.pointCloud)

    def _invalidate_command_buffers(self) -> None:
        deferred = None
        if self._tickets and self.device.handle:
            self._tickets = []
            try:
                self._synchronize()
            except ops.CapacityError as e:
                deferred = e
        for c in self._cmd_cache.values():
            c.destroy()
        self._cmd_cache = {}
        self._eager_steps = 0
        if deferred is not None:
            raise deferred

    def setDataset(self, cameras: list, images: list) -> None:
        self.trainCameras, self.images = self._views(cameras, images)
        self._camera_buffers = [self.device.bufferFrom(np.asarray(c["camera"], np.float32)) for c in self.trainCameras]
        self._invalidate_command_buffers()

    def _views(self, cameras: list, images: list) -> tuple:
        cameras, images = list(cameras), list(images)
        images = [im if isinstance(im, dict) else dict(name=im.name, width=im.width, height=im.height,
                                                       texture=im.texture if im.texture is not None else self.device.bufferFrom(im.bitmap))
                  for im in images]
        cameras = [c if "camera" in c else dict(c, camera=loaders.cameraUniforms(c, im["width"], im["height"])) for c, im in zip(cameras, images)]
        return cameras, images

    def getTrainingConfig(self) -> dict:
        return dict(self.trainingConfig)

    def setTrainingConfig(self, next_cfg: dict) -> None:
        ops.dssim_mode(dict(self.trainingConfig, **{k: v for k, v in next_cfg.items() if v is not None}))
        self.trainingConfig.update({k: v for k, v in next_cfg.items() if v is not None})
        self._invalidate_command_buffers()
        for p in [self.backwardPass, self.metricsPass] + [more[2] for more in self._more_op_sets + self._more_metric_sets]:
            if p is not None:
                p.setTrainingConfig(next_cfg)

    def getOptimizerHyperparameters(self) -> dict:
        return dict(self.optimizer.getHyperparameters() if self.optimizer else self.optimizerHyperparameters)

    def setOptimizerHyperparameters(self, next_params: dict) -> None:
        self.optimizerHyperparameters.update(next_params)
        self._invalidate_command_buffers()
        if self.optimizer:
            self.optimizer.setHyperparameters(next_params)

    def setDensifyPruneConfig(self, next_cfg: dict) -> None:
        sched = {**self.densifyPruneConfig["schedule"], **(next_cfg.get("schedule") or {})}
        self.densifyPruneConfig = {**self.densifyPruneConfig, **next_cfg, "schedule": sched}
        self.densifyPrune.setConfig(self._densify_op_config())

    def start(self) -> None:
        if self.pointCloud is None or not self.trainCameras:
            print("Cannot start training: Missing point cloud or dataset.")
            return
        self.isTraining = True
        self.iteration = 0
        self.stepItersPerSec = 0.0
        self.stepMs = 0.0
        self.lastDensifyPruneIteration = None
        for k in range(1, max(self._lanes, self.metric_lanes)):
            self.device.laneOrder(k, 0)
            self.device.laneOrder(0, k)

    def stop(self) -> None:
        self.isTraining = False
        if self.device.handle and self._tickets:
            self.drain()

    def getIsTraining(self) -> bool:
        return self.isTraining

    def setMaxIterations(self, n: int) -> None:
        self.maxIterations = max(1, int(n))

    def getMaxIterations(self) -> int:
        return self.maxIterations

    def getIteration(self) -> int:
        return self.iteration

    def getPointCount(self) -> int:
        return self.pointCloud.num_points if self.pointCloud else 0

    def getLastStepMs(self) -> float:
        return self.stepMs

    def getItersPerSec(self) -> float:
        return self.stepItersPerSec

    def getLastDensifyPruneIteration(self) -> Optional[int]:
        return self.lastDensifyPruneIteration

    def getNextDensifyPruneIteration(self) -> Optional[int]:
        s = self.densifyPruneConfig["schedule"]
        if not s["enabled"]:
            return None
        warmup, interval, stop, i = s["warmupIterations"], max(1, s["interval"]), s["stopIterations"], self.iteration
        if i >= stop:
            return None
        if i < warmup:
            return min(warmup, stop)
        nxt = warmup + math.ceil((i + 1 - warmup) / interval) * interval
        return nxt if nxt <= stop else None

    def _new_forward_pass(self, cameraBuffer, w: int, h: int, maxTileEntries: Optional[int] = None) -> ops.TiledForwardPass:
        entries = self._tile_entries() if maxTileEntries is None else int(maxTileEntries)
        fw = ops.TiledForwardPass(self.device, self.pointCloud, cameraBuffer, dict(viewportWidth=w, viewportHeight=h, renderMode="gaussian", maxTileEntries=entries))
        fw.setDcSource(self._dc_words)
        if self.longLists is not None:
            fw.setLongLists(int(self.longLists.get("threshold", 2048)), int(self.longLists.get("maxItems", 0)), int(self.longLists.get("maxRows", 0)))
        return fw

    def _grow_long_lists(self) -> None:
        import warnings
        cap_items, cap_rows = int((self.longLists or {}).get("maxItemsCap", 8192)), int((self.longLists or {}).get("maxRowsCap", 65536))
        have_items = have_rows = need_items = need_rows = 0
        for fw in self._forward_passes():
            st = fw.longListStats()
            if not st["threshold"]:
                continue
            if st["stalled"]:
                warnings.warn(f"a long-list task gave up waiting (code {st['stalled']:#x}): the frame's long tiles are not to be trusted", RuntimeWarning, stacklevel=3)
            have_items, have_rows = max(have_items, st["maxItems"]), max(have_rows, st["maxRows"])
            if st["itemsWanted"] <= cap_items:
                need_items, need_rows = max(need_items, st["itemsWanted"]), max(need_rows, st["rowsWanted"])
        items = max(have_items, min(int(need_items * 1.5), cap_items)) if need_items > have_items else have_items
        rows = max(have_rows, min(int(need_rows * 1.5), cap_rows)) if need_rows > have_rows else have_rows
        if (items, rows) == (have_items, have_rows):
            return
        self.longLists = dict(self.longLists or {}, maxItems=items, maxRows=rows)
        warnings.warn(f"long-list scratch enlarged to {self.longLists['maxItems']} chunk slots and {self.longLists['maxRows']} rows", RuntimeWarning, stacklevel=3)
        self._invalidate_command_buffers()
        for fw in self._forward_passes():
            fw.setLongLists(int(self.longLists.get("threshold", 2048)), self.longLists["maxItems"], self.longLists["maxRows"])

    def ensurePipelines(self, width: int, height: int) -> None:
        if (max(1, int(width)), max(1, int(height))) != (self.lastViewportWidth, self.lastViewportHeight):
            self._invalidate_command_buffers()
        self.lastViewportWidth, self.lastViewportHeight = max(1, int(width)), max(1, int(height))
        w, h = self.lastViewportWidth, self.lastViewportHeight
        if self.forwardPass is None:
            self.forwardPass = self._new_forward_pass(self.cameraBuffer, w, h)
        else:
            self.forwardPass.setViewport(w, h)
        if self.rasterizer is None:
            self.rasterizer = ops.TiledRasterizer(dict(device=self.device, forwardPass=self.forwardPass, format="rgba8unorm"))
        if self.backwardPass is None:
            self.backwardPass = ops.TiledBackwardPass(self.device, self.pointCloud, dict(viewportWidth=w, viewportHeight=h, trainingConfig=self.trainingConfig))
            self._gradient_output_applied = None
        else:
            self.backwardPass.setViewport(w, h)
        for more in self._more_op_sets:
            more[0].setViewport(w, h)
            more[2].setViewport(w, h)
        while len(self._more_op_sets) < self._op_sets - 1:
            fw = self._new_forward_pass(self.cameraBuffer, w, h)
            self._more_op_sets.append([fw, ops.TiledRasterizer(dict(device=self.device, forwardPass=fw, format="rgba8unorm")),
                                       ops.TiledBackwardPass(self.device, self.pointCloud, dict(viewportWidth=w, viewportHeight=h, trainingConfig=self.trainingConfig))])
        if self.optimizer is not None and self.world_size * self.views_per_rank == 1:
            self.optimizer.setGuard(self.forwardPass.getStatsBuffer(), 8)

    def ensureMetricsPipelines(self, baseWidth: int, baseHeight: int) -> tuple[int, int]:
        down = max(1, int(self.densifyPruneConfig["metricDownscale"]))
        w, h = max(1, baseWidth // down), max(1, baseHeight // down)
        if self.metricsForwardPass and self.metricsViewportWidth == w and self.metricsViewportHeight == h:
            return w, h
        for name in ("metricsForwardPass", "metricsRasterizer", "metricsPass"):
            op = getattr(self, name)
            if op is not None:
                op.destroy()
            setattr(self, name, None)
        self._destroy_more_metric_sets()
        self.metricsViewportWidth, self.metricsViewportHeight = w, h
        self.metricsForwardPass = self._new_forward_pass(self.metricsCameraBuffer, w, h)
        self.metricsRasterizer = ops.TiledRasterizer(dict(device=self.device, forwardPass=self.metricsForwardPass, format="rgba8unorm"))
        self.metricsPass = ops.TiledBackwardPass(self.device, self.pointCloud, dict(viewportWidth=w, viewportHeight=h, trainingConfig=self.trainingConfig))
        self.metricsTarget = self.device.createBuffer(4 * w * h, "metrics-gt-downsampled")
        return w, h

    def _metric_set(self, k: int) -> tuple:
        if k == 0:
            return self.metricsForwardPass, self.metricsRasterizer, self.metricsPass, self.metricsTarget, self.metricsCameraBuffer
        w, h = self.metricsViewportWidth, self.metricsViewportHeight
        while len(self._more_metric_sets) < k:
            cam = self.device.createBuffer(272, "metrics camera uniform")
            fw = self._new_forward_pass(cam, w, h)
            self._more_metric_sets.append([fw, ops.TiledRasterizer(dict(device=self.device, forwardPass=fw, format="rgba8unorm")),
                                           ops.TiledBackwardPass(self.device, self.pointCloud, dict(viewportWidth=w, viewportHeight=h, trainingConfig=self.trainingConfig)),
                                           self.device.createBuffer(4 * w * h, "metrics-gt-downsampled"), cam])
        return tuple(self._more_metric_sets[k - 1])

    @staticmethod
    def metrics_camera(camera: np.ndarray, width: int, height: int) -> np.ndarray:
        from . import synth
        cam = np.asarray(camera, np.float32)
        fov_y = 2.0 * math.atan(float(cam[65]) / (2.0 * float(cam[67])))
        focal = 0.5 * height / math.tan(fov_y * 0.5)
        fov_x = 2.0 * math.atan(width / (2.0 * focal))
        znear, zfar = 0.01, 100.0
        top, right = math.tan(fov_y / 2.0) * znear, math.tan(fov_x / 2.0) * znear
        out = np.zeros(68, np.float32)
        out[0:16] = cam[0:16]
        out[32], out[37] = 2.0 * znear / (2.0 * right), -2.0 * znear / (2.0 * top)
        out[42], out[43], out[46] = zfar / (zfar - znear), 1.0, -(zfar * znear) / (zfar - znear)
        out[16:32] = synth.mat4_inverse(out[0:16])
        out[48:64] = synth.mat4_inverse(out[32:48])
        out[64:68] = (width, height, focal, focal)
        return out

    def _ops_of(self, op_set: int) -> tuple:
        return tuple(self._more_op_sets[op_set - 1]) if op_set > 0 else (self.forwardPass, self.rasterizer, self.backwardPass)

    def _encode_view(self, encoder, index: int, op_set: int = 0, geometry: bool = True, projected: bool = False) -> None:
        forwardPass, rasterizer, backwardPass = self._ops_of(op_set)
        image = self.images[index]
        cam = self._camera_buffers[index]
        forwardPass.setCameraBuffer(cam)
        if projected:
            forwardPass.encodeProjected(encoder)
        else:
            forwardPass.encode(encoder)
        rasterizer.encode(encoder, image["width"], image["height"])
        res = dict(splatBuffer=forwardPass.getResources()["splatBuffer"], tileOffsetsBuffer=rasterizer.getTileOffsetsBuffer(),
                   tileIndicesBuffer=forwardPass.getSortedIndicesBuffer(), cameraBuffer=cam,
                   alphaTexture=rasterizer.getAlphaTextureView(), nContribTexture=rasterizer.getNContribTextureView())
        if geometry:
            backwardPass.encode(encoder, rasterizer.getOutputTextureView(), image["texture"], res)
        else:
            backwardPass.encodeRaster(encoder, rasterizer.getOutputTextureView(), image["texture"], res)

    def warmupCommandBuffers(self) -> int:
        if not self.use_command_buffers or not self.isTraining or self.pointCloud is None:
            return 0
        n_views, taken = self.world_size * self.views_per_rank, 0
        for v in range(len(self.trainCameras)):
            for _ in range(2 if v == 0 else 1):
                self.step([v] * n_views)
                taken += 1
        return taken

    def step(self, view_ids: Optional[list] = None) -> None:
        try:
            self._step(view_ids)
        except ops.CapacityError as e:
            if not self._grow_tile_entry_capacity(e):
                raise

    def _tile_entries(self) -> int:
        return self.maxTileEntries or self._grown_tile_entries

    def _grow_tile_entry_capacity(self, error) -> bool:
        import re
        import warnings
        if self.maxTileEntries != 0 or not self.device.handle:
            return False
        mine = self._own_overflow(error) or []
        now = max([int(fw.getResources()["maxTileEntries"]) for fw in self._forward_passes()] + [self._grown_tile_entries, 1 << 20])
        new = min(max(2 * now, int(max(mine) * 1.5) if mine else 0), 0xFFFFF000)
        if new <= now:
            return False
        warnings.warn(f"tile-entry lists grown from {now} to {new} entries after an overflow ({error}); the step that overflowed was skipped", RuntimeWarning, stacklevel=3)
        self._grown_tile_entries = new
        self._tickets = []
        try:
            self.device.synchronize()
        except ops.CapacityError:
            pass
        self._invalidate_command_buffers()
        for name in self._OP_NAMES:
            if name != "optimizer" and getattr(self, name) is not None:
                getattr(self, name).destroy()
                setattr(self, name, None)
        self._destroy_more_op_sets()
        self._destroy_more_metric_sets()
        self._gradient_output_applied = None
        self.ensurePipelines(self.lastViewportWidth, self.lastViewportHeight)
        for fw in self._forward_passes():
            fw.setDcSource(self._dc_words)
        return True

    def _step(self, view_ids: Optional[list] = None) -> None:
        if not self.isTraining or self.pointCloud is None:
            return
        stepStart = time.perf_counter()
        n_views = self.world_size * self.views_per_rank
        if view_ids is None:
            view_ids = [self._rng.randrange(len(self.trainCameras)) for _ in range(n_views)]
        mine = parallel.shard_views(view_ids, self.rank, self.world_size)
        image0 = self.images[mine[0]]
        self.ensurePipelines(image0["width"], image0["height"])

        s = self.densifyPruneConfig["schedule"]
        nextIteration = self.iteration + 1
        warmup, interval, stop = s["warmupIterations"], max(1, s["interval"]), s["stopIterations"]
        shouldDensify = s["enabled"] and warmup <= nextIteration <= stop and (nextIteration == warmup or (nextIteration - warmup) % interval == 0)

        try:
            if n_views == 1:
                self._step_single_view(mine[0])
            else:
                self._step_batched(mine)
        except BaseException as orig:
            if self.device.handle:
                self.device.lib.wdgs_encoder_abort(self.device.handle)
            try:
                self._invalidate_command_buffers()
            except ops.CapacityError as deferred:
                raise orig from deferred
            finally:
                self._tickets = []
            raise
        try:
            self._finish_step(n_views)
        except BaseException:
            self._tickets = []
            raise

        self.iteration += 1
        self.stepMs = (time.perf_counter() - stepStart) * 1000.0
        inst = 1000.0 / self.stepMs if self.stepMs > 0 else 0.0
        self.stepItersPerSec = inst if self.stepItersPerSec == 0 else self.stepItersPerSec * 0.9 + inst * 0.1
        if shouldDensify:
            self.drain()
            self._grow_long_lists()
            self.runDensifyPruneMultiView()
            req = self.consumePointCloudSwapRequest()
            if req is not None:
                self.applyPointCloudSwap(req)
        if self.iteration >= self.maxIterations:
            self.stop()
            self.drain()

    def _run(self, key: tuple, encode) -> bool:
        cmd = self._cmd_cache.get(key)
        if cmd is not None:
            self.device.queue.submit([cmd])
            return True
        record = self.use_command_buffers and self._eager_steps >= 1
        with self.device.createCommandEncoder("trainer-" + str(key[0]), record=record) as encoder:
            encode(encoder)
            cmd = encoder.finish()
        if record:
            self._cmd_cache[key] = cmd
        self.device.queue.submit([cmd])
        return False

    def _apply_gradient_output(self) -> None:
        want = bool(self.keep_gradients or not self.fuse_geometry_adam)
        if self._gradient_output_applied is want:
            return
        if self._gradient_output_applied is not None:
            self._invalidate_command_buffers()
        self.backwardPass.setGradientOutput(want)
        self._gradient_output_applied = want

    def _step_single_view(self, view: int) -> None:
        self._apply_gradient_output()
        tileCounts = self.forwardPass.getResources()["tileCountsBuffer"]

        def encode(encoder):
            if self.fuse_geometry_adam:
                self._encode_view(encoder, view, geometry=False)
                self.optimizer.stepWithGeometry(encoder, self.pointCloud, self.backwardPass, self._camera_buffers[view], tileCounts)
            else:
                self._encode_view(encoder, view)
                self.optimizer.step(encoder, self.pointCloud, self.backwardPass.getGradientsBuffer(), tileCounts)
        if self._run(("step", view), encode):
            self.optimizer.advanceIteration(1)
        elif not self.use_command_buffers or self._eager_steps < 1:
            self._eager_steps += 1

    def _step_batched(self, mine: list) -> None:
        n, w = self.pointCloud.num_points, self.world_size
        sl = parallel.slice_points(n, w)
        if self._dp_grad is None:
            self._dp_grad = self.device.createBuffer(4 * parallel.GRAD_FLOATS * w * sl, "dp-grad-f32")
            self._dp_visible = self.device.createBuffer(4 * w * sl, "dp-visible")
            self._dp_flag = self.device.createBuffer(16, "dp-guard")
# ... 46 lines not shown
                    dev.selectLane(U)
                ops.geometryViews([sets[k][2] for k in grp], [cams[k] for k in grp], [sets[k][0] for k in grp], self._dp_grad, self._dp_visible, self._dp_flag,
                                  self.pointCloud, continues=gi > 0)
        finally:
            if lanes:
                dev.lib.wdgs_encoder_abort(dev.handle)
                dev.selectLane(0)
                for s in range(1, ops.MAX_LANES if U else L):
                    dev.laneOrder(0, s)

    def _views_one_by_one(self, mine: list) -> None:
        dev = self.device
        L = min(self._lanes, self._op_sets)
        lanes = L > 1 and self.use_command_buffers and all(("view", v, k % L) in self._cmd_cache for k, v in enumerate(mine))
        try:
            for s in range(1, L if lanes else 0):
                dev.laneOrder(s, 0)
            for k, v in enumerate(mine):
                s = k % L
                forwardPass, _, backwardPass = self._ops_of(s)
                if lanes:
                    dev.selectLane(s)
                self._run(("view", v, s), lambda encoder, v=v, s=s: self._encode_view(encoder, v, s, geometry=False))
                if lanes and k > 0:
                    dev.laneOrder(s, (k - 1) % L)
                backwardPass.encodeGeometry(None, self._camera_buffers[v], dict(sums=self._dp_grad, visible=self._dp_visible, first=(k == 0),
                                                                                tileCounts=forwardPass.getResources()["tileCountsBuffer"],
                                                                                guard=self._dp_flag, stats=forwardPass.getStatsBuffer()))
        finally:
            if lanes:
                dev.lib.wdgs_encoder_abort(dev.handle)
                dev.selectLane(0)
                for s in range(1, L):
                    dev.laneOrder(0, s)

    def _timed(self, collective) -> None:
        if not self.exchange_timing:
            collective()
            return
        e0, e1 = torch.cuda.Event(enable_timing=True), torch.cuda.Event(enable_timing=True)
        e0.record(self.device.torch_stream)
        collective()
        e1.record(self.device.torch_stream)
        self._exchange_events.append((e0, e1))

    def exchangeMilliseconds(self) -> float:
        self.device.synchronize()
        ms = sum(a.elapsed_time(b) for a, b in self._exchange_events)
        self._exchange_events = []
        return float(ms)

    def _metric_overflow(self):
        found = None
        for fw in [self.metricsForwardPass] + [more[0] for more in self._more_metric_sets]:
            if fw is None:
                continue
            try:
                fw.check()
            except ops.CapacityError as e:
                found = found or e
        return found

    def _agree(self, flag: bool) -> bool:
        if self.world_size <= 1:
            return bool(flag)
        if self._agree_word is None:
            self._agree_word = self.device.createBuffer(4, "agreement word")
        self._agree_word.write(np.array([1 if flag else 0], np.uint32))
        self.exchange.allreduce_counts(self._agree_word.ptr, 1)
        return int(self._agree_word.read(np.uint32, 1)[0]) != 0

    def _own_overflow(self, error) -> Optional[list]:
        import re
        named = re.findall(r"(\d+) entries needed, max_tile_entries = \d+ \(forward pass (0x[0-9a-fA-F]+)\)", str(error))
        if not named:
            return None
        own = {int(fw.handle.value or 0) for fw in self._forward_passes()}
        return [int(n) for n, h in named if int(h, 16) in own]

    def _not_ours(self, error) -> bool:
        if self._own_overflow(error) != []:
            return False
        self.device.capacityReports.post(error)
        if not self._foreign_overflow_warned:
            import warnings
            warnings.warn(f"a forward pass that is not this trainer's overflowed its tile-entry lists ({error}); its owner has to enlarge them", RuntimeWarning, stacklevel=4)
            self._foreign_overflow_warned = True
        return True

    def _wait(self, ticket) -> None:
        try:
            self.device.queue.wait(ticket)
        except ops.CapacityError as e:
            if not self._not_ours(e):
                raise
        self._reports_left_for_us()

    def _synchronize(self) -> None:
        try:
            self.device.synchronize()
        except ops.CapacityError as e:
            if not self._not_ours(e):
                raise
        self._reports_left_for_us()

    def _reports_left_for_us(self) -> None:
        if self.device.capacityReports.pending:
            e = self.device.capacityReports.take(int(fw.handle.value or 0) for fw in self._forward_passes())
            if e is not None:
                raise e

    def _finish_step(self, n_views: int) -> None:
        self._tickets.append(self.device.queue.mark())
        while len(self._tickets) >= self.pipeline_depth:
            self._wait(self._tickets.pop(0))

    def drain(self) -> None:
        tickets, self._tickets = self._tickets, []
        for t in tickets:
            self._wait(t)

    def syncOptimizerState(self) -> None:
        if not self._state_sliced or self.world_size <= 1:
            return
        n, w = self.pointCloud.num_points, self.world_size
        bufs = self.optimizer.getStateBuffers()
        rows = dict(optPosBuffer=48, optRotBuffer=48, optScaleBuffer=48, optOpacityBuffer=12, paramSH=192, stateSH=384)
        for root in range(w):
            first, count = parallel.owned_range(n, w, root)
            for k, rb in rows.items():
                self.exchange.broadcast(bufs[k].ptr + first * rb, count * rb, root)
        self.optimizer.stateChanged()
        self._state_sliced = False

    def destroy(self) -> None:
        if self.device.handle:
            self.device.lib.wdgs_encoder_abort(self.device.handle)
            self._tickets = []
            try:
                self.device.synchronize()
            except ops.CapacityError:
                pass
        self._invalidate_command_buffers()
        for name in self._OP_NAMES + ("densifyPrune",):
            op = getattr(self, name, None)
            if op is not None:
                op.destroy()
            setattr(self, name, None)
        self._destroy_more_op_sets()
        self._destroy_more_metric_sets()
        self._destroy_eval_sets()
        self._dp_grad = self._dp_visible = self._dp_rows = self._dp_flag = self.metricsTarget = None
        self._camera_buffers = []
        self._eval_camera_buffers = []
        self.pointCloud = None
        self.isTraining = False

    def setEvaluationViews(self, cameras: list, images: list) -> None:
        cameras, images = list(cameras), list(images)
        if len(cameras) != len(images):
            raise ValueError(f"setEvaluationViews: {len(cameras)} cameras, {len(images)} images")
        self.evalCameras, self.evalImages = self._views(cameras, images)
        self._eval_camera_buffers = [self.device.bufferFrom(np.asarray(c["camera"], np.float32)) for c in self.evalCameras]

    def _destroy_eval_sets(self) -> None:
        for fw, rast in self._eval_sets.values():
            rast.destroy()
            fw.destroy()
        self._eval_sets = {}

    def _eval_set(self, width: int, height: int, cameraBuffer) -> tuple:
        key = (int(width), int(height))
        if key not in self._eval_sets:
            fw = self._new_forward_pass(cameraBuffer, key[0], key[1], self._eval_tile_entries or self.evalMaxTileEntries or None)
            self._eval_sets[key] = (fw, ops.TiledRasterizer(dict(device=self.device, forwardPass=fw, format="rgba8unorm")))
        return self._eval_sets[key]

    def _eval_follow_cloud(self) -> None:
        if self._eval_long_lists != self.longLists:
            self._destroy_eval_sets()
            self._eval_long_lists = None if self.longLists is None else dict(self.longLists)
        for fw, _ in list(self._eval_sets.values()):
            if fw.pointCloud is not self.pointCloud and not fw.setPointCloud(self.pointCloud):
                self._destroy_eval_sets()
                break
        for fw, _ in self._eval_sets.values():
            fw.setDcSource(self._dc_words)

    def _eval_overflow(self) -> Optional[int]:
        own = {int(fw.handle.value or 0) for fw, _ in self._eval_sets.values()}
        try:
            self.device.synchronize()
            err = self.device.capacityReports.take(own) if self.device.capacityReports.pending else None
        except ops.CapacityError as e:
            err = e
        if err is None:
            return None
        import re
        named = re.findall(r"(\d+) entries needed, max_tile_entries = \d+ \(forward pass (0x[0-9a-fA-F]+)\)", str(err))
        mine = [int(n) for n, h in named if int(h, 16) in own]
        if ops.CapacityReports.passes_named(err) - own:
            self.device.capacityReports.post(err)
        if not mine:
            if ops.CapacityReports.passes_named(err):
                return None
            raise err
        return max(mine)

    def evaluate(self, viewIds: Optional[list] = None, split: str = "eval") -> dict:
        import warnings
        if split not in ("eval", "train"):
            raise ValueError(f"evaluate: split must be 'eval' or 'train', not {split!r}")
        if self.pointCloud is None:
            raise RuntimeError("evaluate: no point cloud")
        cams, imgs, bufs = ((self.evalCameras, self.evalImages, self._eval_camera_buffers) if split == "eval" else
                            (self.trainCameras, self.images, self._camera_buffers))
        ids = list(range(len(cams))) if viewIds is None else [int(v) for v in viewIds]
        for v in ids:
            if not 0 <= v < len(cams):
                raise IndexError(f"evaluate: view {v} of {len(cams)} ({split})")
        t0 = time.perf_counter()
        try:
            self.drain()
        except ops.CapacityError as e:
            if not self._grow_tile_entry_capacity(e):
                raise
        n = len(ids)
        out = self.device.createBuffer(16 * max(1, n), "evaluation sse + ssim")
        sse_at, ssim_at = out.ptr, out.ptr + 8 * max(1, n)
        while n:
            self._eval_follow_cloud()
            for i, v in enumerate(ids):
                im, w, h = imgs[v], int(imgs[v]["width"]), int(imgs[v]["height"])
                fw, rast = self._eval_set(w, h, bufs[v])
                fw.setCameraBuffer(bufs[v])
                fw.encode(None)
                rast.encode(None, w, h)
                pred = rast.getOutputTextureView()
                ops.encodeImageSSE(self.device, pred, im["texture"], w * h, self.device.view(sse_at + 8 * i, 8))
                ops.encodeImageSSIM(self.device, pred, im["texture"], w, h, self.device.view(ssim_at + 8 * i, 8))
            needed = self._eval_overflow()
            if needed is None:
                break
            now = max([int(fw.getResources()["maxTileEntries"]) for fw, _ in self._eval_sets.values()] + [self._eval_tile_entries])
            new = min(max(2 * now, int(needed * 1.5)), 0xFFFFF000)
            if new <= now:
                raise RuntimeError(f"evaluate: a view needs {needed} tile entries, more than the lists can hold")
            warnings.warn(f"evaluation tile-entry lists grown from {now} to {new} entries after an overflow; the views are rendered again", RuntimeWarning, stacklevel=2)
            self._eval_tile_entries = new
            self._destroy_eval_sets()
        sse = out.read(np.uint64, count=n) if n else np.zeros(0, np.uint64)
        ssim = out.read(np.float64, count=n, offset=8 * max(1, n)) if n else np.zeros(0)
        psnr = [ops.psnrFromSSE(int(sse[i]), int(imgs[v]["width"]) * int(imgs[v]["height"])) for i, v in enumerate(ids)]
        ssim_l = [float(x) for x in ssim]
        return dict(iteration=self.iteration, views=ids, psnr=psnr, ssim=ssim_l, sse=[int(x) for x in sse],
                    mean_psnr=float(np.mean(psnr)) if n else float("nan"), mean_ssim=float(np.mean(ssim_l)) if n else float("nan"),
                    ms=(time.perf_counter() - t0) * 1e3)

    def runDensifyPruneMultiView(self) -> None:
        if self.pointCloud is None or self.optimizer is None or not self.trainCameras or not self.images:
            return
        baseW, baseH = self.lastViewportWidth, self.lastViewportHeight
        mW, mH = self.ensureMetricsPipelines(baseW, baseH)
        c = self.densifyPruneConfig
        viewsTarget = max(1, int(c["metricViews"]))
        encoder = self.device.createCommandEncoder("densify-prune multiview metrics")
        counts = self.metricsPass.getMetricCountsBuffer()
        encoder.clearBuffer(counts)
        dev, L = self.device, self.metric_lanes
        usedViews, attempts, taken = 0, 0, 0
        try:
            while attempts < viewsTarget * 4 and usedViews < viewsTarget:
                attempts += 1
                idx = self._rng.randrange(len(self.trainCameras))
                camData, image = self.trainCameras[idx], self.images[idx]
                if image["width"] != baseW or image["height"] != baseH:
                    continue
                take = (usedViews % self.world_size) == self.rank
                usedViews += 1
                if not take:
                    continue
                k = taken % L
                taken += 1
                fw, rast, mpass, target, cam = self._metric_set(k)
                if k > 0:
                    if taken <= L:
                        mpass.setMetricCountsTarget(counts)
                        dev.laneOrder(k, 0)
                    dev.selectLane(k)
                cam.write(self.metrics_camera(camData["camera"], mW, mH))
                fw.encode(encoder)
                rast.encode(encoder, mW, mH)
                ops.downsampleRGBA8(dev, image["texture"], baseW, baseH, target, mW, mH)
                mpass.computeMetricMap(encoder, rast.getOutputTextureView(), target, dict(threshold=c["metricThreshold"]))
                mpass.computeMetricCounts(encoder, dict(splatBuffer=fw.getResources()["splatBuffer"], tileOffsetsBuffer=rast.getTileOffsetsBuffer(),
                                                       tileIndicesBuffer=fw.getSortedIndicesBuffer(), nContribTexture=rast.getNContribTextureView()), dict(clear=False))
                if k > 0:
                    dev.selectLane(0)
        finally:
            dev.selectLane(0)
            for k in range(1, min(L, taken)):
                dev.laneOrder(0, k)
        if usedViews == 0:
            return
        if self.world_size > 1:
            overflow = self._metric_overflow()
# ... 24 lines not shown
```

Measured before the change: 1272.

## Precompute per-view target SSIM window statistics once and reuse in loss kernel

Adds a kernel that computes each training image's 5x5 window means and variances once per dataset and stores them in a per-view buffer, 24 bytes per pixel, under a memory budget. The loss-gradient kernel gains a mode that reads these cached target statistics instead of recomputing the target-side window sums each iteration. This removes per-iteration target arithmetic in the SSIM loss but adds extra global memory reads and per-view storage. Since the targets are fixed dataset images, the reuse is a legitimate precomputation.

After: 1215. 0.956x the previous value.

```diff
diff --git a/bindings/napi/webdgs_napi.cc b/bindings/napi/webdgs_napi.cc
--- a/bindings/napi/webdgs_napi.cc
+++ b/bindings/napi/webdgs_napi.cc
@@ -238,6 +238,7 @@
     r.camera_buffer = prop_ptr(env, argv[3], "cameraBuffer");
     r.alpha_texture = prop_ptr(env, argv[3], "alphaTexture");
     r.n_contrib_texture = prop_ptr(env, argv[3], "nContribTexture");
+    r.target_stats = nullptr;
     WDGS_OK_OR_THROW(wdgs_tiled_backward_encode((wdgs_tiled_backward*)get_ptr(env, argv[0]), get_ptr(env, argv[1]), get_ptr(env, argv[2]), &r, get_ptr(env, argv[4])));
     return js_undefined(env);
 }
@@ -361,6 +362,7 @@
     r->camera_buffer = prop_ptr(env, o, "cameraBuffer");
     r->alpha_texture = prop_ptr(env, o, "alphaTexture");
     r->n_contrib_texture = prop_ptr(env, o, "nContribTexture");
+    r->target_stats = nullptr;
 }
 static napi_value tiledBackwardMetric(napi_env env, napi_callback_info info) {
     ARGS(5);
diff --git a/include/webdgs.h b/include/webdgs.h
--- a/include/webdgs.h
+++ b/include/webdgs.h
@@ -160,6 +160,7 @@
     const void* camera_buffer;
     const void* alpha_texture;
     const void* n_contrib_texture;
+    const void* target_stats;
 } wdgs_tiled_backward_resources;
 
 int wdgs_tiled_backward_create(wdgs_device* dev, const wdgs_tiled_backward_config* cfg, wdgs_tiled_backward** out);
@@ -179,6 +180,9 @@
                                       const wdgs_tiled_backward_resources* res);
 int wdgs_tiled_backward_encode_geometry(wdgs_tiled_backward* op, const void* camera_dev, const void* gaussians_dev, const wdgs_view_accumulate* into);
 int wdgs_tiled_backward_compute_loss_only(wdgs_tiled_backward* op, const void* predicted_rgba8_dev, const void* target_rgba8_dev);
+int wdgs_loss_target_stats(wdgs_device* dev, uint32_t width, uint32_t height, const void* target_rgba8_dev, void* stats_dev);
+int wdgs_tiled_backward_compute_loss_only_with_stats(wdgs_tiled_backward* op, const void* predicted_rgba8_dev, const void* target_rgba8_dev,
+                                                     const void* target_stats_dev);
 int wdgs_tiled_backward_compute_metric_map(wdgs_tiled_backward* op, const void* predicted_rgba8_dev, const void* target_rgba8_dev, float threshold);
 int wdgs_tiled_backward_compute_metric_counts(wdgs_tiled_backward* op, const wdgs_tiled_backward_resources* res, uint32_t num_instances, int clear);
 int wdgs_tiled_backward_normalize_metric_counts(wdgs_tiled_backward* op, uint32_t divisor);
diff --git a/webdgs_amd/_lib.py b/webdgs_amd/_lib.py
--- a/webdgs_amd/_lib.py
+++ b/webdgs_amd/_lib.py
@@ -52,7 +52,7 @@
 
 class TiledBackwardResources(C.Structure):
     _fields_ = [("splat_buffer", C.c_void_p), ("tile_offsets_buffer", C.c_void_p), ("tile_indices_buffer", C.c_void_p), ("camera_buffer", C.c_void_p),
-                ("alpha_texture", C.c_void_p), ("n_contrib_texture", C.c_void_p)]
+                ("alpha_texture", C.c_void_p), ("n_contrib_texture", C.c_void_p), ("target_stats", C.c_void_p)]
 
 
 class ViewAccumulate(C.Structure):
@@ -199,6 +199,8 @@
     "wdgs_tiled_backward_encode_raster": (_I, [_P, _P, _P, C.POINTER(TiledBackwardResources)]),
     "wdgs_tiled_backward_encode_geometry": (_I, [_P, _P, _P, C.POINTER(ViewAccumulate)]),
     "wdgs_tiled_backward_compute_loss_only": (_I, [_P, _P, _P]),
+    "wdgs_tiled_backward_compute_loss_only_with_stats": (_I, [_P, _P, _P, _P]),
+    "wdgs_loss_target_stats": (_I, [_P, _U, _U, _P, _P]),
     "wdgs_tiled_backward_compute_metric_map": (_I, [_P, _P, _P, _F]),
     "wdgs_tiled_backward_compute_metric_counts": (_I, [_P, C.POINTER(TiledBackwardResources), _U, _I]),
     "wdgs_tiled_backward_normalize_metric_counts": (_I, [_P, _U]),
diff --git a/webdgs_amd/csrc/api.hip b/webdgs_amd/csrc/api.hip
--- a/webdgs_amd/csrc/api.hip
+++ b/webdgs_amd/csrc/api.hip
@@ -25,7 +25,8 @@
                            void*, void*, void*, const void*, const void*);
 int launch_rasterize(wdgs_device*, const RenderSettings&, const TileInfo&, const void*, u32, const void*, const void*, const void*, const void*, u32, void*,
                      void*, void*, const void*, const void*, const LongWork*);
-int launch_loss_grad(wdgs_device*, u32, u32, const void*, const void*, const wdgs_training_config&, void*, void*, u32, const void*);
+int launch_loss_grad(wdgs_device*, u32, u32, const void*, const void*, const wdgs_training_config&, void*, void*, u32, const void*, const void*);
+int launch_loss_target_stats(wdgs_device*, u32, u32, const void*, void*);
 int launch_dssim_grad(wdgs_device*, u32, u32, const void*, const void*, const wdgs_training_config&, void*, void*, u32, const void*);
 int launch_backward_rasterize(wdgs_device*, const RenderSettings&, u32, u32, const void*, const void*, const void*, const void*, const void*, const void*,
                               void*, void*, const LongWork*);
@@ -1261,19 +1262,30 @@
     op->gradient_output = enabled != 0;
     return WDGS_OK;
 }
-static int backward_loss(wdgs_tiled_backward* op, const void* pred, const void* targ, void* acc, u32 acc_rows, const void* acc_dirty) {
+static int backward_loss(wdgs_tiled_backward* op, const void* pred, const void* targ, void* acc, u32 acc_rows, const void* acc_dirty, const void* stats) {
     const u32 w = op->cfg.viewport_width, h = op->cfg.viewport_height;
     if (op->dssim_mode == WDGS_DSSIM_GAUSSIAN) return launch_dssim_grad(op->dev, w, h, pred, targ, op->cfg.training, op->loss_image, acc, acc_rows, acc_dirty);
-    return launch_loss_grad(op->dev, w, h, pred, targ, op->cfg.training, op->loss_image, acc, acc_rows, acc_dirty);
+    return launch_loss_grad(op->dev, w, h, pred, targ, op->cfg.training, op->loss_image, acc, acc_rows, acc_dirty, stats);
 }
 int wdgs_tiled_backward_compute_loss_only(wdgs_tiled_backward* op, const void* pred, const void* targ) {
     WDGS_REQUIRE(op && pred && targ, WDGS_E_INVALID, "wdgs_tiled_backward_compute_loss_only: null argument");
-    return backward_loss(op, pred, targ, nullptr, 0u, nullptr);
+    return backward_loss(op, pred, targ, nullptr, 0u, nullptr, nullptr);
+}
+int wdgs_tiled_backward_compute_loss_only_with_stats(wdgs_tiled_backward* op, const void* pred, const void* targ, const void* stats) {
+    WDGS_REQUIRE(op && pred && targ, WDGS_E_INVALID, "wdgs_tiled_backward_compute_loss_only_with_stats: null argument");
+    WDGS_REQUIRE(((uintptr_t)stats & 15u) == 0, WDGS_E_INVALID, "wdgs_tiled_backward_compute_loss_only_with_stats: target statistics must be 16-byte aligned");
+    return backward_loss(op, pred, targ, nullptr, 0u, nullptr, stats);
+}
+int wdgs_loss_target_stats(wdgs_device* d, uint32_t w, uint32_t h, const void* targ, void* stats) {
+    WDGS_REQUIRE(d && targ && stats && w > 0 && h > 0, WDGS_E_INVALID, "wdgs_loss_target_stats: invalid argument");
+    WDGS_REQUIRE(((uintptr_t)stats & 15u) == 0, WDGS_E_INVALID, "wdgs_loss_target_stats: the statistics buffer must be 16-byte aligned");
+    return launch_loss_target_stats(d, w, h, targ, stats);
 }
 static int backward_encode_raster(wdgs_tiled_backward* op, const void* pred, const void* targ, const wdgs_tiled_backward_resources* res) {
     wdgs_device* d = op->dev;
     const u32 w = op->cfg.viewport_width, h = op->cfg.viewport_height, n = op->cfg.num_points;
-    if (w > 0 && h > 0) WDGS_TRY(backward_loss(op, pred, targ, op->acc, std::max(n, 1u), op->acc_dirty));
+    WDGS_REQUIRE(((uintptr_t)res->target_stats & 15u) == 0, WDGS_E_INVALID, "backward encode: target statistics must be 16-byte aligned");
+    if (w > 0 && h > 0) WDGS_TRY(backward_loss(op, pred, targ, op->acc, std::max(n, 1u), op->acc_dirty, res->target_stats));
     else WDGS_TRY(launch_acc_clear_if_dirty(d, op->acc, n, op->acc_dirty));
     const LongWork* lw = nullptr;
     auto owner = d->range_tables.find(res->tile_offsets_buffer);
diff --git a/webdgs_amd/csrc/dssim.hip b/webdgs_amd/csrc/dssim.hip
--- a/webdgs_amd/csrc/dssim.hip
+++ b/webdgs_amd/csrc/dssim.hip
@@ -217,12 +217,12 @@
 
 }
 
-int launch_loss_grad(wdgs_device*, u32, u32, const void*, const void*, const wdgs_training_config&, void*, void*, u32, const void*);
+int launch_loss_grad(wdgs_device*, u32, u32, const void*, const void*, const wdgs_training_config&, void*, void*, u32, const void*, const void*);
 
 int launch_dssim_grad(wdgs_device* dev, u32 W, u32 H, const void* pred, const void* targ, const wdgs_training_config& cfg, void* out, void* acc, u32 acc_rows,
                       const void* acc_dirty) {
     if (W == 0 || H == 0) return WDGS_OK;
-    if (cfg.lambda_dssim == 0.0f) return launch_loss_grad(dev, W, H, pred, targ, cfg, out, acc, acc_rows, acc_dirty);
+    if (cfg.lambda_dssim == 0.0f) return launch_loss_grad(dev, W, H, pred, targ, cfg, out, acc, acc_rows, acc_dirty, nullptr);
     WDGS_LAUNCH(dev, "dssim_grad", dssim_grad_kernel, dim3(ceil_div(W, DT), ceil_div(H, DT)), dim3(256), 0, W, H, (const u32*)pred, (const u32*)targ, cfg,
                 ssim_window(), (float4*)out, (int4*)acc, acc_rows * 3u , (const u32*)acc_dirty);
     WDGS_CHECK_HIP(hipGetLastError());
diff --git a/webdgs_amd/csrc/loss.hip b/webdgs_amd/csrc/loss.hip
--- a/webdgs_amd/csrc/loss.hip
+++ b/webdgs_amd/csrc/loss.hip
@@ -10,10 +10,14 @@
 constexpr u32 LT = 32;
 constexpr u32 LH = LT + 4;
 
-template <u32 PPT>
-__global__ __launch_bounds__(256) void loss_grad_kernel(u32 W, u32 H, const u32* __restrict__ pred, const u32* __restrict__ targ,
-                                                         wdgs_training_config cfg, float4* __restrict__ out, int4* __restrict__ acc, u32 acc_quads,
-                                                         const u32* __restrict__ acc_dirty) {
+enum : u32 { LOSS_FULL = 0u, LOSS_WITH_STATS = 1u, LOSS_TARGET_STATS = 2u };
+
+template <u32 PPT, u32 MODE>
+WD_DEV void loss_window(u32 W, u32 H, const u32* __restrict__ pred, const u32* __restrict__ targ, const wdgs_training_config& cfg, float4* __restrict__ out,
+                        int4* __restrict__ acc, u32 acc_quads, const u32* __restrict__ acc_dirty, const float4* __restrict__ stats_a, const float2* __restrict__ stats_b,
+                        float4* __restrict__ stats_out_a, float2* __restrict__ stats_out_b) {
+    constexpr bool PRED = MODE != LOSS_TARGET_STATS;
+    constexpr bool TARG = MODE != LOSS_WITH_STATS;
     if (acc && *acc_dirty != 0u) {
         const int4 z = make_int4(0, 0, 0, 0);
         const u32 nblk = gridDim.x * gridDim.y, blk = blockIdx.y * gridDim.x + blockIdx.x;
@@ -40,10 +44,20 @@
     const u32 x = bx + lx, y0 = by + ly0;
     if (x >= W || y0 >= H) return;
 
-    const bool dssim = cfg.lambda_dssim > 0.0f;
+    const bool dssim = MODE == LOSS_TARGET_STATS || cfg.lambda_dssim > 0.0f;
     const float n = 25.0f;
-    float mx[PPT][3], my[PPT][3], sx2[PPT][3], sy2[PPT][3], sxy[PPT][3];
+    float mx[PPT][3], my[PPT][3], sx2[PPT][3], sy2[PPT][3], sxy[PPT][3], vys[PPT][3];
     if (dssim) {
+        if constexpr (MODE == LOSS_WITH_STATS) {
+#pragma unroll
+            for (u32 k = 0; k < PPT; k++) {
+                const size_t p = (size_t)(y0 + k < H ? y0 + k : H - 1u) * W + x;
+                const float4 sa = stats_a[p];
+                const float2 sb = stats_b[p];
+                my[k][0] = sa.x; my[k][1] = sa.y; my[k][2] = sa.z;
+                vys[k][0] = sa.w; vys[k][1] = sb.x; vys[k][2] = sb.y;
+            }
+        }
         f2 mxa[PPT], mxb[PPT], mya[PPT], myb[PPT];
 #pragma unroll
         for (u32 k = 0; k < PPT; k++) mxa[k] = mxb[k] = mya[k] = myb[k] = f2{0.f, 0.f};
@@ -52,23 +66,27 @@
 #pragma unroll
             for (u32 c = 0; c < 5u; c++) {
                 const float4 a = sp[ly0 + r][lx + c];
-                const float2 b = st[ly0 + r][lx + c];
+                float2 b = make_float2(0.f, 0.f);
+                if constexpr (TARG) b = st[ly0 + r][lx + c];
 #pragma unroll
                 for (u32 k = 0; k < PPT; k++)
                     if (r >= k && r <= k + 4u) {
-                        mxa[k] += f2{a.x, a.y}; mxb[k].x += a.z;
-                        mya[k] += f2{a.w, b.x}; myb[k].x += b.y;
+                        if constexpr (PRED) { mxa[k] += f2{a.x, a.y}; mxb[k].x += a.z; }
+                        if constexpr (TARG) { mya[k] += f2{a.w, b.x}; myb[k].x += b.y; }
                     }
             }
 #pragma unroll
-            for (u32 k = 0; k < PPT; k++)
-                asm volatile("" : "+v"(mxa[k].x), "+v"(mxa[k].y), "+v"(mxb[k].x), "+v"(mya[k].x), "+v"(mya[k].y), "+v"(myb[k].x));
+            for (u32 k = 0; k < PPT; k++) {
+                if constexpr (PRED) asm volatile("" : "+v"(mxa[k].x), "+v"(mxa[k].y), "+v"(mxb[k].x));
+                if constexpr (TARG) asm volatile("" : "+v"(mya[k].x), "+v"(mya[k].y), "+v"(myb[k].x));
+            }
         }
         f2 sx2a[PPT], sx2b[PPT], sy2a[PPT], sy2b[PPT], sxya[PPT], sxyb[PPT], ma[PPT], mb[PPT], na[PPT], nb[PPT];
 #pragma unroll
         for (u32 k = 0; k < PPT; k++) {
-            mx[k][0] = wd_div_inrange(mxa[k].x, n); mx[k][1] = wd_div_inrange(mxa[k].y, n); mx[k][2] = wd_div_inrange(mxb[k].x, n);
-            my[k][0] = wd_div_inrange(mya[k].x, n); my[k][1] = wd_div_inrange(mya[k].y, n); my[k][2] = wd_div_inrange(myb[k].x, n);
+            if constexpr (PRED) { mx[k][0] = wd_div_inrange(mxa[k].x, n); mx[k][1] = wd_div_inrange(mxa[k].y, n); mx[k][2] = wd_div_inrange(mxb[k].x, n); }
+            else mx[k][0] = mx[k][1] = mx[k][2] = 0.f;
+            if constexpr (TARG) { my[k][0] = wd_div_inrange(mya[k].x, n); my[k][1] = wd_div_inrange(mya[k].y, n); my[k][2] = wd_div_inrange(myb[k].x, n); }
             ma[k] = f2{mx[k][0], mx[k][1]}; mb[k] = f2{mx[k][2], 0.f};
             na[k] = f2{my[k][0], my[k][1]}; nb[k] = f2{my[k][2], 0.f};
             sx2a[k] = sx2b[k] = sy2a[k] = sy2b[k] = sxya[k] = sxyb[k] = f2{0.f, 0.f};
@@ -86,18 +104,25 @@
                         const float dab = a.z - mb[k].x;
                         const f2 dba = f2{a.w, b.x} - na[k];
                         const float dbb = b.y - nb[k].x;
-                        sx2a[k].x = __builtin_fmaf(daa.x, daa.x, sx2a[k].x); sx2a[k].y = __builtin_fmaf(daa.y, daa.y, sx2a[k].y);
-                        sx2b[k].x = __builtin_fmaf(dab, dab, sx2b[k].x);
-                        sy2a[k].x = __builtin_fmaf(dba.x, dba.x, sy2a[k].x); sy2a[k].y = __builtin_fmaf(dba.y, dba.y, sy2a[k].y);
-                        sy2b[k].x = __builtin_fmaf(dbb, dbb, sy2b[k].x);
-                        sxya[k].x = __builtin_fmaf(daa.x, dba.x, sxya[k].x); sxya[k].y = __builtin_fmaf(daa.y, dba.y, sxya[k].y);
-                        sxyb[k].x = __builtin_fmaf(dab, dbb, sxyb[k].x);
+                        if constexpr (PRED) {
+                            sx2a[k].x = __builtin_fmaf(daa.x, daa.x, sx2a[k].x); sx2a[k].y = __builtin_fmaf(daa.y, daa.y, sx2a[k].y);
+                            sx2b[k].x = __builtin_fmaf(dab, dab, sx2b[k].x);
+                        }
+                        if constexpr (TARG) {
+                            sy2a[k].x = __builtin_fmaf(dba.x, dba.x, sy2a[k].x); sy2a[k].y = __builtin_fmaf(dba.y, dba.y, sy2a[k].y);
+                            sy2b[k].x = __builtin_fmaf(dbb, dbb, sy2b[k].x);
+                        }
+                        if constexpr (PRED) {
+                            sxya[k].x = __builtin_fmaf(daa.x, dba.x, sxya[k].x); sxya[k].y = __builtin_fmaf(daa.y, dba.y, sxya[k].y);
+                            sxyb[k].x = __builtin_fmaf(dab, dbb, sxyb[k].x);
+                        }
                     }
             }
 #pragma unroll
-            for (u32 k = 0; k < PPT; k++)
-                asm volatile("" : "+v"(sx2a[k].x), "+v"(sx2a[k].y), "+v"(sx2b[k].x), "+v"(sy2a[k].x), "+v"(sy2a[k].y), "+v"(sy2b[k].x), "+v"(sxya[k].x),
-                             "+v"(sxya[k].y), "+v"(sxyb[k].x));
+            for (u32 k = 0; k < PPT; k++) {
+                if constexpr (PRED) asm volatile("" : "+v"(sx2a[k].x), "+v"(sx2a[k].y), "+v"(sx2b[k].x), "+v"(sxya[k].x), "+v"(sxya[k].y), "+v"(sxyb[k].x));
+                if constexpr (TARG) asm volatile("" : "+v"(sy2a[k].x), "+v"(sy2a[k].y), "+v"(sy2b[k].x));
+            }
         }
 #pragma unroll
         for (u32 k = 0; k < PPT; k++) {
@@ -110,6 +135,11 @@
     for (u32 k = 0; k < PPT; k++) {
         const u32 y = y0 + k;
         if (y >= H) break;
+        if constexpr (MODE == LOSS_TARGET_STATS) {
+            stats_out_a[(size_t)y * W + x] = make_float4(my[k][0], my[k][1], my[k][2], wd_div_inrange(sy2[k][0], n));
+            stats_out_b[(size_t)y * W + x] = make_float2(wd_div_inrange(sy2[k][1], n), wd_div_inrange(sy2[k][2], n));
+            continue;
+        }
         const float4 p = sp[ly0 + k + 2u][lx + 2u];
         const float2 t = st[ly0 + k + 2u][lx + 2u];
         const float d[3] = {p.x - p.w, p.y - t.x, p.z - t.y};
@@ -117,7 +147,7 @@
         if (dssim) {
 #pragma unroll
             for (int c = 0; c < 3; c++) {
-                const float vx = wd_div_inrange(sx2[k][c], n), vy = wd_div_inrange(sy2[k][c], n), vxy = wd_div_inrange(sxy[k][c], n);
+                const float vx = wd_div_inrange(sx2[k][c], n), vy = MODE == LOSS_WITH_STATS ? vys[k][c] : wd_div_inrange(sy2[k][c], n), vxy = wd_div_inrange(sxy[k][c], n);
                 const float num1 = 2.0f * mx[k][c] * my[k][c] + cfg.c1;
                 const float num2 = 2.0f * vxy + cfg.c2;
                 const float den1 = mx[k][c] * mx[k][c] + my[k][c] * my[k][c] + cfg.c1;
@@ -136,16 +166,47 @@
     }
 }
 
+template <u32 PPT, u32 MODE>
+__global__ __launch_bounds__(256) void loss_grad_kernel(u32 W, u32 H, const u32* __restrict__ pred, const u32* __restrict__ targ, wdgs_training_config cfg,
+                                                         float4* __restrict__ out, int4* __restrict__ acc, u32 acc_quads, const u32* __restrict__ acc_dirty,
+                                                         const float4* __restrict__ stats_a, const float2* __restrict__ stats_b) {
+    loss_window<PPT, MODE>(W, H, pred, targ, cfg, out, acc, acc_quads, acc_dirty, stats_a, stats_b, nullptr, nullptr);
+}
+
+template <u32 PPT>
+__global__ __launch_bounds__(256) void loss_target_stats_kernel(u32 W, u32 H, const u32* __restrict__ targ, float4* __restrict__ stats_a, float2* __restrict__ stats_b) {
+    loss_window<PPT, LOSS_TARGET_STATS>(W, H, targ, targ, wdgs_training_config{}, nullptr, nullptr, 0u, nullptr, nullptr, nullptr, stats_a, stats_b);
+}
+
 }
 
 int launch_loss_grad(wdgs_device* dev, u32 W, u32 H, const void* pred, const void* targ, const wdgs_training_config& cfg, void* out, void* acc, u32 acc_rows,
-                     const void* acc_dirty) {
+                     const void* acc_dirty, const void* stats) {
     if (W == 0 || H == 0) return WDGS_OK;
-#define WDGS_LOSS_LAUNCH(PPT_)                                                                                                                                       \
-    WDGS_LAUNCH(dev, "loss_grad", loss_grad_kernel<PPT_>, dim3(ceil_div(W, LT), ceil_div(H, 8u * PPT_)), dim3(256), 0, W, H, (const u32*)pred, (const u32*)targ, cfg, \
-                (float4*)out, (int4*)acc, acc_rows * 3u , (const u32*)acc_dirty)
-    if ((size_t)W * H <= 640u * 480u) { WDGS_LOSS_LAUNCH(1u); } else { WDGS_LOSS_LAUNCH(2u); }
+    const float4* const sa = (const float4*)stats;
+    const float2* const sb = stats ? (const float2*)(sa + (size_t)W * H) : nullptr;
+#define WDGS_LOSS_LAUNCH(PPT_, MODE_)                                                                                                                          \
+    WDGS_LAUNCH(dev, "loss_grad", (loss_grad_kernel<PPT_, MODE_>), dim3(ceil_div(W, LT), ceil_div(H, 8u * PPT_)), dim3(256), 0, W, H, (const u32*)pred,         \
+                (const u32*)targ, cfg, (float4*)out, (int4*)acc, acc_rows * 3u , (const u32*)acc_dirty, sa, sb)
+    const bool small = (size_t)W * H <= 640u * 480u;
+    if (stats && cfg.lambda_dssim > 0.0f) {
+        if (small) { WDGS_LOSS_LAUNCH(1u, LOSS_WITH_STATS); } else { WDGS_LOSS_LAUNCH(2u, LOSS_WITH_STATS); }
+    } else {
+        if (small) { WDGS_LOSS_LAUNCH(1u, LOSS_FULL); } else { WDGS_LOSS_LAUNCH(2u, LOSS_FULL); }
+    }
 #undef WDGS_LOSS_LAUNCH
     WDGS_CHECK_HIP(hipGetLastError());
     return WDGS_OK;
 }
+
+int launch_loss_target_stats(wdgs_device* dev, u32 W, u32 H, const void* targ, void* stats) {
+    float4* const sa = (float4*)stats;
+    float2* const sb = (float2*)(sa + (size_t)W * H);
+    if ((size_t)W * H <= 640u * 480u) {
+        WDGS_LAUNCH(dev, "loss_target_stats", loss_target_stats_kernel<1u>, dim3(ceil_div(W, LT), ceil_div(H, 8u)), dim3(256), 0, W, H, (const u32*)targ, sa, sb);
+    } else {
+        WDGS_LAUNCH(dev, "loss_target_stats", loss_target_stats_kernel<2u>, dim3(ceil_div(W, LT), ceil_div(H, 16u)), dim3(256), 0, W, H, (const u32*)targ, sa, sb);
+    }
+    WDGS_CHECK_HIP(hipGetLastError());
+    return WDGS_OK;
+}
diff --git a/webdgs_amd/ops.py b/webdgs_amd/ops.py
--- a/webdgs_amd/ops.py
+++ b/webdgs_amd/ops.py
@@ -535,7 +535,7 @@
             b = res.get(k)
             return b.ptr if b is not None else None
         return _lib.TiledBackwardResources(p("splatBuffer"), p("tileOffsetsBuffer"), p("tileIndicesBuffer"), p("cameraBuffer"), p("alphaTexture"),
-                                           p("nContribTexture"))
+                                           p("nContribTexture"), p("targetStats"))
 
     def setPointCloud(self, pointCloud: PointCloud) -> bool:
         if pointCloud.sh_deg != self.pointCloud.sh_deg:
@@ -559,8 +559,13 @@
             into = C.byref(_lib.ViewAccumulate(a["sums"].ptr, a["visible"].ptr, a["tileCounts"].ptr, a["guard"].ptr, a["stats"].ptr + 8, 1 if a["first"] else 0))
         check(self.device.lib.wdgs_tiled_backward_encode_geometry(self.handle, cameraBuffer.ptr, self.pointCloud.gaussian_3d_buffer.ptr, into))
 
-    def computeLossOnly(self, encoder, predictedTexture: HipBuffer, targetTexture: HipBuffer) -> None:
-        check(self.device.lib.wdgs_tiled_backward_compute_loss_only(self.handle, predictedTexture.ptr, targetTexture.ptr))
+    def computeLossOnly(self, encoder, predictedTexture: HipBuffer, targetTexture: HipBuffer, targetStats: Optional[HipBuffer] = None) -> None:
+        if targetStats is None:
+            check(self.device.lib.wdgs_tiled_backward_compute_loss_only(self.handle, predictedTexture.ptr, targetTexture.ptr))
+            return
+        if targetStats.size < TARGET_STATS_BYTES_PER_PIXEL * self.viewportWidth * self.viewportHeight:
+            raise ValueError(f"computeLossOnly: target statistics of {targetStats.size} bytes are too small for {self.viewportWidth}x{self.viewportHeight}")
+        check(self.device.lib.wdgs_tiled_backward_compute_loss_only_with_stats(self.handle, predictedTexture.ptr, targetTexture.ptr, targetStats.ptr))
 
     def computeMetricMap(self, encoder, predictedTexture: HipBuffer, targetTexture: HipBuffer, options: Optional[dict] = None) -> None:
         thr = float((options or {}).get("threshold", 0.5))
@@ -625,6 +630,22 @@
 
 def downsampleRGBA8(device: HipDevice, src: HipBuffer, src_w: int, src_h: int, dst: HipBuffer, dst_w: int, dst_h: int) -> None:
     check(device.lib.wdgs_downsample_rgba8(device.handle, src.ptr, src_w, src_h, dst.ptr, dst_w, dst_h))
+
+
+TARGET_STATS_BYTES_PER_PIXEL = 24
+
+
+def lossTargetStats(device: HipDevice, target: HipBuffer, width: int, height: int, out: Optional[HipBuffer] = None) -> HipBuffer:
+    w, h = int(width), int(height)
+    need = TARGET_STATS_BYTES_PER_PIXEL * w * h
+    if w <= 0 or h <= 0 or target.size < 4 * w * h:
+        raise ValueError(f"lossTargetStats: a target of {target.size} bytes is not {w}x{h} rgba8")
+    if out is None:
+        out = device.createBuffer(need, "target statistics")
+    elif out.size < need:
+        raise ValueError(f"lossTargetStats: out holds {out.size} bytes, {w}x{h} needs {need}")
+    check(device.lib.wdgs_loss_target_stats(device.handle, w, h, target.ptr, out.ptr))
+    return out
 
 
 def depthToRGBA8(device: HipDevice, depth: HipBuffer, width: int, height: int, near: float, far: float, target: HipBuffer) -> None:
diff --git a/webdgs_amd/trainer.py b/webdgs_amd/trainer.py
--- a/webdgs_amd/trainer.py
+++ b/webdgs_amd/trainer.py
@@ -12,12 +12,19 @@
 from . import loaders, ops, parallel
 
 
+DEFAULT_TARGET_STATS_BUDGET = 4 << 30
+
+
 class Trainer:
     def __init__(self, device: ops.HipDevice, trainingConfig: Optional[dict] = None, seed: int = 0, world_size: int = 1, rank: int = 0,
                  views_per_rank: int = 1, maxTileEntries: int = 0, use_command_buffers: bool = True, exchange: Optional[parallel.Exchange] = None,
-                 overlap_views: Optional[bool] = None, pipeline_depth: int = 1, batch_views: Optional[bool] = None):
+                 overlap_views: Optional[bool] = None, pipeline_depth: int = 1, batch_views: Optional[bool] = None, target_stats: bool = True,
+                 target_stats_budget_bytes: int = DEFAULT_TARGET_STATS_BUDGET):
         ops.dssim_mode(trainingConfig)
         self.device = device
+        self.target_stats = bool(target_stats)
+        self.target_stats_budget_bytes = max(0, int(target_stats_budget_bytes))
+        self._target_stats: list = []
         self.trainingConfig = dict(trainingConfig or dict(lambda_l1=0.8, lambda_l2=0.0, lambda_dssim=0.2))
         self.optimizerHyperparameters = dict(ops.DEFAULT_ADAM_HYPERPARAMETERS)
         self.world_size, self.rank, self.views_per_rank = int(world_size), int(rank), max(1, int(views_per_rank))
@@ -186,7 +193,30 @@
     def setDataset(self, cameras: list, images: list) -> None:
         self.trainCameras, self.images = self._views(cameras, images)
         self._camera_buffers = [self.device.bufferFrom(np.asarray(c["camera"], np.float32)) for c in self.trainCameras]
-        self._invalidate_command_buffers()
+        self._target_stats = []
+        try:
+            self._invalidate_command_buffers()
+        finally:
+            self._build_target_stats()
+
+    def _build_target_stats(self) -> None:
+        self._target_stats += [None] * (len(self.images) - len(self._target_stats))
+        tc = self.trainingConfig
+        if not self.target_stats or ops.dssim_mode(tc) != ops.DSSIM_MODES["reference"] or not float(tc.get("lambda_dssim", 0.2)) > 0.0:
+            return
+        spent = sum(b.size for b in self._target_stats if b is not None)
+        built = False
+        for i, im in enumerate(self.images):
+            if self._target_stats[i] is not None:
+                continue
+            need = ops.TARGET_STATS_BYTES_PER_PIXEL * int(im["width"]) * int(im["height"])
+            if need <= 0 or spent + need > self.target_stats_budget_bytes:
+                continue
+            self._target_stats[i] = ops.lossTargetStats(self.device, im["texture"], im["width"], im["height"])
+            spent += need
+            built = True
+        if built:
+            self.device.torch_stream.synchronize()
 
     def _views(self, cameras: list, images: list) -> tuple:
         cameras, images = list(cameras), list(images)
@@ -203,6 +233,7 @@
         ops.dssim_mode(dict(self.trainingConfig, **{k: v for k, v in next_cfg.items() if v is not None}))
         self.trainingConfig.update({k: v for k, v in next_cfg.items() if v is not None})
         self._invalidate_command_buffers()
+        self._build_target_stats()
         for p in [self.backwardPass, self.metricsPass] + [more[2] for more in self._more_op_sets + self._more_metric_sets]:
             if p is not None:
                 p.setTrainingConfig(next_cfg)
@@ -395,7 +426,8 @@
         rasterizer.encode(encoder, image["width"], image["height"])
         res = dict(splatBuffer=forwardPass.getResources()["splatBuffer"], tileOffsetsBuffer=rasterizer.getTileOffsetsBuffer(),
                    tileIndicesBuffer=forwardPass.getSortedIndicesBuffer(), cameraBuffer=cam,
-                   alphaTexture=rasterizer.getAlphaTextureView(), nContribTexture=rasterizer.getNContribTextureView())
+                   alphaTexture=rasterizer.getAlphaTextureView(), nContribTexture=rasterizer.getNContribTextureView(),
+                   targetStats=self._target_stats[index] if self.target_stats and index < len(self._target_stats) else None)
         if geometry:
             backwardPass.encode(encoder, rasterizer.getOutputTextureView(), image["texture"], res)
         else:
@@ -748,6 +780,7 @@
         self._destroy_eval_sets()
         self._dp_grad = self._dp_visible = self._dp_rows = self._dp_flag = self.metricsTarget = None
         self._camera_buffers = []
+        self._target_stats = []
         self._eval_camera_buffers = []
         self.pointCloud = None
         self.isTraining = False
```
